# Tom94/practical-path-guiding

Hardware: AMD Instinct MI355X
Metric: Msamples/s (higher is better)
Workload: dtype f32; 1 GPU; room-720p (kitchen-class STAND-IN for the KITCHEN scene, 1397784 Lambertian triangles), 1280x720, 1 spp/pass, 614 passes, improved preset; headline_scene=False, parallelism=tiles1

## Files before the change

### include/ppg.h

```cpp
#ifndef PPG_H
#define PPG_H

#include <stddef.h>
#include <stdint.h>

#ifdef __cplusplus
extern "C" {
#endif

#define PPG_OK 0
#define PPG_ERR_INVALID (-1)
#define PPG_ERR_DEVICE (-2)
#define PPG_ERR_STATE (-3)
#define PPG_ERR_CANCELLED (-4)
#define PPG_ERR_NOMEM (-5)

typedef struct ppg_ctx ppg_ctx;

typedef struct ppg_config {
    const char *nee;
    const char *sampleCombination;
    const char *spatialFilter;
    const char *directionalFilter;
    const char *bsdfSamplingFractionLoss;
// ... 223 lines not shown
    uint32_t weight_texture;
    int32_t ensure_energy_conservation;
    uint32_t _reserved[4];
} ppg_blend;
int ppg_set_blends(ppg_ctx *ctx, const ppg_blend *b, uint32_t n_materials);

int ppg_render(ppg_ctx *ctx);

int ppg_begin_render(ppg_ctx *ctx);
int ppg_begin_iteration(ppg_ctx *ctx, int32_t is_final);
int ppg_set_final(ppg_ctx *ctx, int32_t is_final);
int ppg_set_do_nee(ppg_ctx *ctx, int32_t do_nee);
int ppg_render_passes(ppg_ctx *ctx, int32_t n_passes, ppg_pass_stats *stats);
int ppg_build_sdtree(ppg_ctx *ctx, ppg_tree_stats *stats);
int ppg_end_iteration(ppg_ctx *ctx);
int ppg_end_render(ppg_ctx *ctx);

int ppg_cancel(ppg_ctx *ctx);
int ppg_release_cached_memory(int32_t device);

int ppg_read_film(ppg_ctx *ctx, float *rgb);
int ppg_read_variance(ppg_ctx *ctx, float *rgb);

int ppg_dump_sdtree(ppg_ctx *ctx, const char *path);

typedef struct ppg_sdtree_info {
    uint32_t n_stree_nodes;
    uint32_t n_leaves;
    uint64_t n_sampling_nodes;
    uint64_t n_building_nodes;
    float aabb_min[3], aabb_max[3];
    int32_t iter;
    int32_t is_built;
} ppg_sdtree_info;

int ppg_sdtree_info_get(ppg_ctx *ctx, ppg_sdtree_info *info);

int ppg_sdtree_read_stree(ppg_ctx *ctx, int32_t *axis, uint32_t *children );

int ppg_sdtree_read_dtree_headers(ppg_ctx *ctx, int32_t which, uint64_t *offset, uint32_t *num_nodes,
                                  int32_t *max_depth, float *sum, double *stat_weight);

int ppg_sdtree_read_dtree_nodes(ppg_ctx *ctx, int32_t which, float *sums, uint16_t *children, uint64_t *fixed_sums);

int ppg_sdtree_read_adam(ppg_ctx *ctx, float *theta);

int ppg_sdtree_stat_buffers(ppg_ctx *ctx, void **dev_sums, uint64_t *n_sums, void **dev_weights, uint64_t *n_weights);
int ppg_film_buffers(ppg_ctx *ctx, void **dev_rgb_sum , void **dev_weight );
int ppg_image_buffers(ppg_ctx *ctx, void **dev_image , void **dev_sq_image ,
                      void **dev_weight );
int ppg_render_passes_nostat(ppg_ctx *ctx, int32_t n_passes);
int ppg_finish_passes(ppg_ctx *ctx, ppg_pass_stats *stats);

#define PPG_STOP_CANCELLED 2
typedef int (*ppg_stop_hook)(void *user, int local_stop);
int ppg_set_stop_hook(ppg_ctx *ctx, ppg_stop_hook hook, void *user);
int ppg_exchange_stream(ppg_ctx *ctx, void **hip_stream);
int32_t ppg_final_group_passes(int32_t n_passes);
int ppg_final_partials(ppg_ctx *ctx, void **dev , uint64_t *n_floats);
int ppg_final_partials_commit(ppg_ctx *ctx);

typedef int (*ppg_footprint_hook)(void *user, void *dev_halo , uint64_t n_floats, int32_t local_status);
int ppg_set_footprint_hook(ppg_ctx *ctx, ppg_footprint_hook hook, void *user);
uint64_t ppg_footprint_halo_floats(int32_t width, int32_t height, int32_t tile_size, int32_t world, int32_t border);

#define PPG_ADAM_ROUND_MAX_PASSES 16
#define PPG_ADAM_ROUND_MAX_PATHS (1u << 24)
#define PPG_ADAM_CODE_BITS 13
#define PPG_ADAM_PATH_BITS 27
#define PPG_ADAM_LEAF_SHIFT (PPG_ADAM_CODE_BITS + PPG_ADAM_PATH_BITS)
#define PPG_ADAM_CODE_VERTEX 4096
#define PPG_ADAM_DEFER_DEPTH 64
#define PPG_ADAM_DEFER_PATH_BIT (1u << (PPG_ADAM_PATH_BITS - 1))
int32_t ppg_adam_round_passes(int32_t spp_per_pass, int32_t width, int32_t height, int32_t n_passes);

#define PPG_ADAM_REGION_MAX_PASSES 16
int ppg_set_adam_regions(ppg_ctx *ctx, int32_t regions);

typedef struct ppg_adam_record {
    uint64_t key;
    float product, wo_pdf, bsdf_pdf, dtree_pdf, statistical_weight, _pad;
} ppg_adam_record;

typedef int (*ppg_pass_hook)(void *user);
int ppg_set_pass_hook(ppg_ctx *ctx, ppg_pass_hook hook, void *user);
int ppg_adam_records(ppg_ctx *ctx, void **dev_records , uint64_t *n);
int ppg_adam_records_replace(ppg_ctx *ctx, const void *dev_records, uint64_t n);

int ppg_hook_phase(ppg_ctx *ctx, int32_t *phase);
int ppg_adam_records_by_owner(ppg_ctx *ctx, int32_t world, void **dev_records , uint64_t *counts );
int ppg_adam_state(ppg_ctx *ctx, int32_t world, void **dev_state, uint64_t *segment);
int ppg_adam_state_commit(ppg_ctx *ctx);

int ppg_query_pdf(ppg_ctx *ctx, uint32_t n, const float *positions, const float *dirs, float *pdf_out);
int ppg_query_sample(ppg_ctx *ctx, uint32_t n, const float *positions, uint64_t seed, float *dirs_out);

typedef struct ppg_kernel_time { const char *name; double ms; uint64_t launches; uint64_t units; } ppg_kernel_time;
int ppg_kernel_times(ppg_ctx *ctx, ppg_kernel_time *out, uint32_t cap, uint32_t *n);
int ppg_enable_kernel_timing(ppg_ctx *ctx, int32_t enable);

#define PPG_FIXED_SHIFT 24

#ifdef __cplusplus
}
#endif
#endif
// ... 1 lines not shown
```

### include/ppg_testhooks.h

```cpp
#ifndef PPG_TESTHOOKS_H
#define PPG_TESTHOOKS_H

#include <stdint.h>

#ifdef __cplusplus
extern "C" {
#endif

int ppg_debug_build_bvh(const float *positions, const uint32_t *indices, uint32_t n_triangles, float pad_abs, int32_t max_leaf,
                        void *nodes_out, uint32_t nodes_cap, uint32_t *n_nodes, uint32_t *order_out);

struct ppg_bvh_stats {
    uint32_t n_nodes, n_leaves, depth, n_binary_nodes;
    uint32_t leaf_hist[9];
    uint32_t stack_need;
    double sa_interior, sa_leaf, sa_tris;
    double build_seconds;
};
int ppg_debug_bvh_stats(const float *positions, const uint32_t *indices, uint32_t n_triangles, float pad_abs, int32_t max_leaf,
                        struct ppg_bvh_stats *out);

int ppg_debug_bvh_trace(const float *positions, const uint32_t *indices, uint32_t n_triangles, float pad_abs, int32_t max_leaf,
                        const float *rays, uint32_t n_rays, float *t_out, int32_t *orig_out, uint32_t *steps_out, uint32_t *tests_out,
                        uint32_t *max_stack);

struct ppg_rfilter;
int ppg_debug_rfilter_table(const struct ppg_rfilter *f, float table[32], float *radius, int32_t *border);

struct ppg_ctx;
int ppg_debug_set_defer_depth(struct ppg_ctx *ctx, int32_t depth);

struct ppg_debug_hit {
    int32_t prim;
    float t;
    float p[3], geo_n[3], n[3], s[3], wi[3];
    int32_t material, emitter;
    int32_t _pad;
};
int ppg_debug_intersect(struct ppg_ctx *ctx, uint32_t n, const float *rays, struct ppg_debug_hit *out, int32_t any_hit);

enum {
    PPG_DEBUG_TRACE_LANE = 0, PPG_DEBUG_TRACE_LANE_ANY = 1, PPG_DEBUG_TRACE_LANE_VOTE = 2, PPG_DEBUG_TRACE_RESUME = 3, PPG_DEBUG_TRACE_WAVE = 4,
    PPG_DEBUG_TRACE_KTRACE = 5
};
int ppg_debug_intersect_mode(struct ppg_ctx *ctx, uint32_t n, const float *rays, struct ppg_debug_hit *out, int32_t mode, int32_t param, uint32_t *stats_out);

struct ppg_debug_direct {
    int32_t emitter;
    float d[3];
    float dist;
    float n[3];
    float pdf, em_pdf;
    float value[3];
    float _pad[3];
};
int ppg_debug_sample_direct(struct ppg_ctx *ctx, uint32_t n, const float *ref, const float *ref_n, const float *u, struct ppg_debug_direct *out);

struct ppg_debug_bsdf_item {
    int32_t material;
    float wi[3], wo[3];
    float sample[2];
    uint32_t key;
    float uv[2];
};
struct ppg_debug_bsdf_out {
    float eval[3];
    float pdf;
    float wo[3];
    float sampled_pdf;
    float weight[3];
    float eta;
    int32_t delta, is_null;
    int32_t _pad[2];
};
int ppg_debug_bsdf(struct ppg_ctx *ctx, uint32_t n, const struct ppg_debug_bsdf_item *items, struct ppg_debug_bsdf_out *out);

#ifdef __cplusplus
}
#endif
#endif
```

### practical-path-guiding_amd/csrc/ppg_batch_plan.h

```cpp
#pragma once

#include <algorithm>
#include <cstddef>
#include <cstdint>

namespace ppg_plan {

constexpr int kSpatialFilterBox = 2;
constexpr int kNeeKickstart = 1;
constexpr unsigned int kBlock = 256;
constexpr unsigned int kDenseChunk = 256;
constexpr unsigned int kAdamLeafShift = 40;

inline bool recordPositionsKnown(int spatialFilter, bool doNee, int nee) { return spatialFilter != kSpatialFilterBox && !(doNee && nee == kNeeKickstart); }

inline bool sideStreamsAllowed(bool timerOn, bool tuneNoOverlap) { return !timerOn && !tuneNoOverlap; }

inline unsigned int adamFlagShift(size_t streeNodes) {
    unsigned int leafBits = 1;
    while ((1u << leafBits) <= (unsigned int)streeNodes) ++leafBits;
    return kAdamLeafShift + leafBits;
}

struct BatchFacts {
// ... 58 lines not shown
    if (maxDepth >= 0) return maxDepth;
    int maxBounces;
    if (tuneBulkBounces >= 0) maxBounces = std::min(64, tuneBulkBounces);
    else {
        int need = 8;
        if (c.bounces > 0 && c.paths > 0) {
            const double scale = (double)paths / (double)c.paths;
            need = -1;
            for (int b = 0; b < c.bounces; ++b) if (c.live[b] * scale < stopBelow) { need = b + 1; break; }
            if (need < 0) {
                double live = c.live[c.bounces - 1] * scale;
                const double before = c.bounces > 1 ? c.live[c.bounces - 2] : (double)c.paths;
                const double ratio = std::min(0.97, std::max(0.5, before > 0 ? c.live[c.bounces - 1] / before : 0.9));
                need = c.bounces;
                while (live >= stopBelow && need < 64) { live *= ratio; ++need; }
            }
        }
        maxBounces = std::max(1, std::min(64, need + margin));
        if (paths < stopBelow) maxBounces = 1;
    }
    if (adamFast) maxBounces = std::min(maxBounces, std::max(1, deferDepthAdam));
    return maxBounces;
}

inline int observeBounces(SurvivalCurve &c, const unsigned int *live, int bouncesRun, unsigned int paths, unsigned int stopBelow) {
    int ran = bouncesRun;
    for (int b = 0; b < bouncesRun; ++b) if (live[b] < stopBelow) { ran = b + 1; break; }
    c.bounces = ran; c.paths = paths;
    for (int b = 0; b < ran; ++b) c.live[b] = live[b];
    return ran;
}

inline int wavefrontGrid(int nBlocks, int tuneBlocksSmall, size_t tuneSmallPaths, unsigned int paths, unsigned int queueCap) {
    if (tuneBlocksSmall > 0 && tuneBlocksSmall < nBlocks && (size_t)paths <= tuneSmallPaths) {
        const size_t chunks = ((size_t)paths + kDenseChunk - 1) / kDenseChunk;
        if (((chunks + (size_t)tuneBlocksSmall - 1) / (size_t)tuneBlocksSmall) * kDenseChunk <= (size_t)queueCap) return tuneBlocksSmall;
    }
    return nBlocks;
}

struct TailShape { int grid; unsigned int laneLimit; };

inline TailShape tailShape(int wavefrontGrid, int tuneTailBlocks, size_t handedPaths) {
    const int grid = std::min(wavefrontGrid, tuneTailBlocks ? tuneTailBlocks : 1024);
    const size_t waves = (size_t)grid * (kBlock / 64);
    return {grid, handedPaths ? (unsigned int)std::max<size_t>(1, std::min<size_t>(64, (handedPaths + waves - 1) / waves)) : 64u};
}
inline TailShape stragglerShape(unsigned int n) {
    const unsigned int waves = 1024u * (kBlock / 64u);
    const unsigned int laneLimit = std::max(1u, std::min(64u, (n + waves - 1u) / waves));
    return {(int)std::max(1u, std::min(1024u, (n + laneLimit * (kBlock / 64u) - 1u) / (laneLimit * (kBlock / 64u)))), laneLimit};
}

struct RoundReadback {
    unsigned int live[64];
    unsigned int slowCount, slowOverflow;
    unsigned int sumBase, lastNv;
    unsigned long long handed;
    unsigned long long stragglers;
};
static_assert(offsetof(RoundReadback, slowOverflow) == offsetof(RoundReadback, slowCount) + 4, "one 8-byte copy fills both");

enum class CommitSet {
    All,
    Ended,
    List
};

}
```

### practical-path-guiding_amd/csrc/ppg_hip.hip

```cpp
#include <hip/hip_runtime.h>

#include <cstring>
#include <map>
#include <mutex>
#include <set>

#include <rocprim/rocprim.hpp>

#include <algorithm>
#include <atomic>
#include <chrono>
#include <cmath>
#include <cstdio>
#include <cstdlib>
#include <cstring>
#include <functional>
#include <limits>
#include <map>
#include <memory>
#include <string>
#include <vector>

#include "../../include/ppg.h"
#include "../../include/ppg_testhooks.h"
// ... 138 lines not shown
        if (keep && p && cap && !g_ctxStream) (void)hipStreamSynchronize(nullptr);
        if (p) g_blockCache.give(p, bytes);
        p = np; bytes = got; cap = got / sizeof(T);
        return e;
    }
};

struct HostSNode {
    int axis = 0;
    uint32_t child[2] = {0, 0};
    bool isLeaf() const { return child[0] == 0; }
};

int parseEnum(const char *s, const char *dflt, std::initializer_list<const char *> names) {
    std::string v = s ? s : dflt;
    int i = 0;
    for (const char *n : names) {
        if (v == n) return i;
        ++i;
    }
    return -1;
}

struct KernelTimer {
    struct Rec { hipEvent_t a, b; int id; uint64_t units; };
    std::vector<std::string> names;
    std::vector<double> ms;
    std::vector<uint64_t> launches, units;
    std::vector<Rec> pending;
    std::vector<hipEvent_t> pool;
    bool enabled = false;
    int idOf(const char *n) {
        for (size_t i = 0; i < names.size(); ++i) if (names[i] == n) return (int)i;
        names.push_back(n); ms.push_back(0); launches.push_back(0); units.push_back(0);
        return (int)names.size() - 1;
    }
    hipEvent_t ev() { if (!pool.empty()) { hipEvent_t e = pool.back(); pool.pop_back(); return e; } hipEvent_t e; (void)hipEventCreate(&e); return e; }
    void resolve() {
        for (auto &r : pending) {
            (void)hipEventSynchronize(r.b);
            float t = 0; (void)hipEventElapsedTime(&t, r.a, r.b);
            ms[r.id] += t; launches[r.id]++; units[r.id] += r.units;
            pool.push_back(r.a); pool.push_back(r.b);
        }
        pending.clear();
    }
    void reset() { resolve(); for (size_t i = 0; i < ms.size(); ++i) { ms[i] = 0; launches[i] = 0; units[i] = 0; } }
};

}

struct GroupLaunch { unsigned int firstPass, groupPasses, stridePasses, slot0, slotStride; bool wholeFilm; unsigned int addCount; bool groupsDone = true; bool exchange = false; };

struct ppg_ctx {
    int nee = 0, sampleCombination = 1, spatialFilter = 0, directionalFilter = 0, loss = 0, budgetType = 1;
    int sdTreeMaxMemory = -1, sTreeThreshold = 12000, sppPerPass = 4, rrDepth = 5, maxDepth = -1;
    float dTreeThreshold = 0.01f, bsdfSamplingFraction = 0.5f, budget = 300.0f;
    bool dumpSDTree = false, strictNormals = false, hideEmitters = false;
    uint64_t seed = 0;
    int device = 0;
    std::string dumpPrefix, error;
    hipStream_t stream = nullptr;
    hipStream_t stream2 = nullptr;
    hipEvent_t evFork = nullptr, evJoin = nullptr;
    hipStream_t stream3 = nullptr;
    hipEvent_t evTreeFork = nullptr, evSplatDone = nullptr, evAdamDone = nullptr;
    bool treePending = false;
    void joinTree() {
        if (!treePending) return;
        (void)hipStreamWaitEvent(stream, evSplatDone, 0);
        (void)hipStreamWaitEvent(stream, evAdamDone, 0);
        treePending = false;
    }
    void quiesce() {
        joinTree();
        if (stream2) (void)hipStreamSynchronize(stream2);
        if (stream3) (void)hipStreamSynchronize(stream3);
        if (stream4) (void)hipStreamSynchronize(stream4);
        if (stream) (void)hipStreamSynchronize(stream);
        for (Stragglers &g : strag) { g.pending = false; g.aside = false; g.film = nullptr; }
    }
    hipStream_t stream4 = nullptr;
    hipEvent_t evStragFork = nullptr, evStragDone = nullptr;
    struct Stragglers {
        DevBuf<float4> rec, vert;
        DevBuf<unsigned int> orig, iota, ticket, base, origSorted, perm;
        DevBuf<unsigned long long> count;
        DevBuf<unsigned char> nv8;
        DevBuf<float> neeCos, theta;
        size_t iotaN = 0;
        PathState P{};
        unsigned int n = 0;
        bool pending = false;
        bool aside = false;
        bool commit = false, adam = false;
        std::function<void()> film;
    } strag[2];
    int stragCur = 0;
    DevBuf<float4> d_liKeep;
    Stragglers &stragPrev() { return strag[stragCur ^ 1]; }
    int tuneSplitDepth = PPG_ADAM_DEFER_DEPTH;
    bool tuneFinalHalves = false;
    int adamRegions = 0;
    DevBuf<unsigned int> d_regionPixels;
    std::vector<unsigned int> regionOffset;
    int regionsBuilt = 0;
    int deferDepthAdam = PPG_ADAM_DEFER_DEPTH;
    int joinStragglers() {
        int rc = 0;
        for (Stragglers &g : strag) if (g.pending && g.aside) { g.aside = false; rc = (int)hipStreamWaitEvent(stream, evStragDone, 0); }
        return rc;
    }
    DevBuf<unsigned char> d_straggler;
    DevBuf<unsigned char> d_nv8;

    bool haveScene = false;
    bool fullMaterials = false;
    DevBuf<float4> d_tris, d_accel, d_accelSmall, d_normals, d_materials, d_emitters, d_emTris, d_emNrm;
    DevBuf<float> d_rtrans;
    DevBuf<float4> d_spheres;
    DevBuf<float2> d_uvs;
    std::vector<DevBuf<float4>> d_texTexels;
    DevBuf<DevTex> d_textures;
    DevBuf<float4> d_emTexels;
    DevBuf<float> d_emCdfRows, d_emCdfCols, d_emRowWeights;
    DevBuf<float> d_emSel, d_emArea, d_neeCos;
    DevBuf<int4> d_emInfo;
    DevBuf<BvhNode> d_bvh;
    DevBuf<Bvh4QNode> d_bvh4;
    DevBuf<float4> d_bvhTop;
    DevScene scene{};
    float aabbMin[3], aabbMax[3];
// ... 80 lines not shown
    DevBuf<unsigned long long> d_adamKeys[2];
    DevBuf<unsigned int> d_adamIdx[2], d_adamNv, d_adamBase, d_adamCount;
    DevBuf<AdamRec> d_adamRecs, d_adamRecsOut;
    DevBuf<float4> d_splat;
    bool sortedCommit = false;
    unsigned int adamFlagShift = 0;
    DevBuf<unsigned char> d_sortTemp, d_orderTemp;
    DevBuf<unsigned int> d_adamLeafCount[2], d_adamLeafOrder[2];
    size_t adamIota = 0;
    bool adamFast = false;
    bool adamActive = false;
    bool inHook = false, hookReplaced = false;
    uint64_t hookCount = 0;
    int hookPhase = 0;
    bool ownerMode = false;
    DevBuf<unsigned int> d_adamState;
    DevBuf<unsigned long long> d_ownerBounds;
    DevBuf<unsigned int> d_bounceCounts, d_ticket;
    RoundReadback *h_round = nullptr;
    SurvivalCurve survival;
    int bounceMargin = 3;
    unsigned int tailThreshold = 0;
    unsigned int tailMin = 2097152, tailDiv = 12;
    size_t tuneBatchPaths = 0;
    int tuneBlocks = 0;
    bool tuneForceBvh = false;
    bool tuneNoSort = false;
    bool tuneNoSortFirst = false;
    bool tuneNoSplit = false;
    bool tuneNoOverlap = false;
    bool tuneNoSortedCommit = false;
    unsigned int tuneSplatLdsNodes = PPG_SPLAT_NODES;
    bool tuneNoAside = false;
    bool tuneAdamUnordered = false;
    int tuneBulkBounces = -1;
    bool debugBatch = false;
    int tuneFinalBatch = 0;
    int tuneTailBlocks = 0;
    int tunePathLayout = 0;
    int tuneBlocksSmall = 2048;
    size_t tuneSmallPaths = 13000000;
    int tuneBvhLeaf = 4;
    float tuneBvhPad = 2e-6f;
    bool tuneNoTopCut = false;
    DevBuf<unsigned int> d_leaves, d_counts, d_offsets, d_grid;
    DevBuf<unsigned int> d_dfs[2], d_refEv, d_refLv, d_refEvOff, d_refLvOff;
    int dfsCur = 0;
    unsigned int dfsCount = 0;
    int ldsNodes = 0, ldsTris = 0;
    float treeMin[3], treeMax[3], treeExt[3];
    bool isBuilt = false, isFinalIter = false, doNee = false;
    int iter = 0, passesRendered = 0, passesRenderedThisIter = 0, passesLocal = 0;
    std::chrono::steady_clock::time_point startTime, passStart;
    std::atomic<bool> cancelled{false};
    bool cancelSeen = false;
    bool seesCancel() { if (!cancelled.load()) return false; cancelSeen = true; return true; }
    float lastVariance = 0;
    ppg_pass_stats lastStats{};
    KernelTimer timer;
#define PPG_TAIL_LOG 256
    DevBuf<unsigned int> d_tailLongest;
    unsigned int tailLaunches = 0;
    uint64_t tailLongestSum = 0;
    uint64_t shadeCommonRays = 0;
    uint64_t bvhNodesVisited = 0, bvhTrisTested = 0;
    ppg_pass_hook passHook = nullptr;
    void *passHookUser = nullptr;
    ppg_stop_hook stopHook = nullptr;
    void *stopHookUser = nullptr;
#ifdef PPG_PROBE
    DevBuf<unsigned long long> d_probe;
#endif

    DevTree devTree() {
        DevTree T{};
        T.stree = d_stree.p; T.hdr = d_hdr.p; T.snodes = d_snodes[cur].p; T.bchild = d_bchild.p; T.bacc = d_bacc.p;
        T.bweight = d_bweight.p;
        T.bweight_rep = d_bweightRep.p;
        T.adam_keys = adamActive ? d_adamKeys[0].p : nullptr; T.adam_recs = adamActive ? d_adamRecs.p : nullptr;
        T.adam_count = d_adamCount.p; T.adam_base = (adamActive && adamFast) ? d_adamBase.p : nullptr;
        T.adam_cap = adamActive ? (unsigned int)std::min<size_t>(std::min(d_adamRecs.cap, d_adamKeys[0].cap), 0xfffffff0u) : 0u;
        for (int a = 0; a < 3; ++a) { T.aabb_min[a] = treeMin[a]; T.aabb_ext[a] = treeExt[a]; T.aabb_max[a] = treeMax[a]; }
        T.is_built = isBuilt ? 1 : 0;
        T.grid = d_grid.p;
        return T;
    }
    RenderParams params() const {
        RenderParams R{};
        R.nee = nee; R.spatial_filter = spatialFilter; R.directional_filter = directionalFilter; R.loss = loss;
        R.bsdf_sampling_fraction = bsdfSamplingFraction; R.rr_depth = rrDepth; R.max_depth = maxDepth;
        R.strict_normals = strictNormals; R.hide_emitters = hideEmitters; R.spp = sppPerPass;
        R.is_final_iter = isFinalIter; R.do_nee = doNee; R.seed = seed; R.pass_index = (unsigned int)passesRendered;
        R.max_vertices = maxVertices; R.img_pixels = (unsigned int)W * (unsigned int)H;
#ifdef PPG_PROBE
        R.probe = d_probe.p;
#endif
        return R;
    }
};

PathKernels ppg_path_kernels[PPG_FAMILIES];

static int sceneFamily(const DevScene &S) {
    if (S.blend) return PPG_FAMILY_BLEND;
    if (S.coat) return PPG_FAMILY_COAT;
    if (S.mfd) return PPG_FAMILY_EXT;
    if (S.n_shapes) return PPG_FAMILY_SHAPES;
    return PPG_FAMILY_BASE;
}
template <typename F> static F launcher(F f) {
    if (!f) { fprintf(stderr, "libppg_hip: no unit of this library holds the kernel asked for\n"); abort(); }
    return f;
}
static void ppg_launch_shade(int variant, const ShadeLaunch &a) { launcher(ppg_path_kernels[sceneFamily(a.S)].shade[variant >> 1])(variant, a); }
static void ppg_launch_tail(int variant, const TailLaunch &a) { launcher(ppg_path_kernels[sceneFamily(a.S)].tail[variant >> 1])(variant, a); }
static bool isSmallScene(const ppg_ctx *ctx) {
    return ctx->scene.n_tris <= 64 && ctx->ldsTris == ctx->scene.n_tris && ctx->scene.n_spheres == 0 && sceneFamily(ctx->scene) == PPG_FAMILY_BASE && !ctx->tuneForceBvh;
}
namespace {

template <typename F> void timedLaunch(ppg_ctx *ctx, const char *name, uint64_t units, F &&launch) {
    if (!ctx->timer.enabled) { launch(); return; }
    KernelTimer::Rec r; r.a = ctx->timer.ev(); r.b = ctx->timer.ev(); r.id = ctx->timer.idOf(name); r.units = units;
    (void)hipEventRecord(r.a, ctx->stream);
    launch();
    (void)hipEventRecord(r.b, ctx->stream);
    ctx->timer.pending.push_back(r);
}

bool sideStreamsAllowed(const ppg_ctx *ctx) { return ppg_plan::sideStreamsAllowed(ctx->timer.enabled, ctx->tuneNoOverlap); }

int gridFor(size_t n, int block = PPG_BLOCK, int maxBlocks = 256 * 8) {
    size_t b = (n + block - 1) / block;
    return (int)std::max<size_t>(1, std::min<size_t>(b, (size_t)maxBlocks));
}

float elapsedSeconds(std::chrono::steady_clock::time_point start) {
    auto ms = std::chrono::duration_cast<std::chrono::milliseconds>(std::chrono::steady_clock::now() - start);
    return (float)ms.count() / 1000;
}

int uploadTree(ppg_ctx *ctx, bool nodes) {
    size_t n = ctx->snodes.size();
    std::vector<int4> st(nodes ? n : 0);
    if (nodes) {
        for (size_t i = 0; i < n; ++i) st[i] = make_int4(ctx->snodes[i].axis, (int)ctx->snodes[i].child[0], (int)ctx->snodes[i].child[1], 0);
        HIP_CHECK(ctx->d_stree.reserve(n));
        HIP_CHECK(ctx->d_hdr.reserve(n));
        HIP_CHECK(hipMemcpyAsync(ctx->d_stree.p, st.data(), n * sizeof(int4), hipMemcpyHostToDevice, ctx->stream));
        HIP_CHECK(hipMemcpyAsync(ctx->d_hdr.p, ctx->hdr.data(), n * sizeof(LeafHdr), hipMemcpyHostToDevice, ctx->stream));
    }
    ctx->leaves.clear();
    for (size_t i = 0; i < n; ++i) if (ctx->snodes[i].isLeaf()) ctx->leaves.push_back((unsigned int)i);
    HIP_CHECK(ctx->d_leaves.reserve(ctx->leaves.size()));
    HIP_CHECK(ctx->d_counts.reserve(ctx->leaves.size()));
    HIP_CHECK(ctx->d_offsets.reserve(ctx->leaves.size()));
    HIP_CHECK(hipMemcpyAsync(ctx->d_leaves.p, ctx->leaves.data(), ctx->leaves.size() * 4, hipMemcpyHostToDevice, ctx->stream));
    HIP_CHECK(ctx->d_bweight.reserve(n));
    HIP_CHECK(hipMemsetAsync(ctx->d_bweight.p, 0, n * 8, ctx->stream));
    HIP_CHECK(ctx->d_bweightRep.reserve(n * PPG_REPLICAS));
    HIP_CHECK(hipMemsetAsync(ctx->d_bweightRep.p, 0, n * PPG_REPLICAS * 8, ctx->stream));
    if (n >= (1u << 27)) { ctx->error = "S-tree exceeds 2^27 nodes"; return PPG_ERR_NOMEM; }
    const unsigned int cells = PPG_GRID_DIM * PPG_GRID_DIM * PPG_GRID_DIM;
    HIP_CHECK(ctx->d_grid.reserve(cells));
    hipLaunchKernelGGL(k_build_grid, dim3((cells + 255) / 256), dim3(256), 0, ctx->stream, ctx->d_stree.p, ctx->d_grid.p);
    HIP_CHECK(hipStreamSynchronize(ctx->stream));
    return PPG_OK;
}

int refineDevice(ppg_ctx *ctx, size_t sTreeThreshold, int maxMB) {
    auto &nodes = ctx->snodes;
    auto &hdr = ctx->hdr;
    if (maxMB >= 0) {
        size_t foot = 0;
        for (size_t i = 0; i < nodes.size(); ++i) foot += nodes[i].isLeaf() ? ((size_t)hdr[i].b_num * 24 + 40) + ((size_t)hdr[i].s_num * 24 + 40) : 2 * (24 + 40);
        if (foot / 1000000 >= (size_t)maxMB) return PPG_OK;
    }
    const unsigned int nl = ctx->dfsCount, nOld = (unsigned int)nodes.size();
    hipStream_t s = ctx->stream;
    HIP_CHECK(ctx->d_refEv.reserve(nl)); HIP_CHECK(ctx->d_refLv.reserve(nl)); HIP_CHECK(ctx->d_refEvOff.reserve(nl)); HIP_CHECK(ctx->d_refLvOff.reserve(nl));
    HIP_CHECK(ctx->d_total.reserve(2));
    hipLaunchKernelGGL(k_refine_count, dim3((nl + 255) / 256), dim3(256), 0, s, ctx->d_hdr.p, ctx->d_dfs[ctx->dfsCur].p, nl, (float)sTreeThreshold,
                       ctx->d_refEv.p, ctx->d_refLv.p);
// ... 114 lines not shown
        st->min_stat_weight = minSW; st->avg_stat_weight = avgSW; st->max_stat_weight = maxSW;
        st->n_leaves = (uint32_t)nPoints; st->n_stree_nodes = (uint32_t)ctx->snodes.size(); st->n_dtree_nodes = totalNodes;
    }
    ctx->isBuilt = true;
    return PPG_OK;
}

int allocPaths(ppg_ctx *ctx) {
    std::vector<unsigned int> pix;
    int tilesX = (ctx->W + ctx->tileSize - 1) / ctx->tileSize;
    for (int y = 0; y < ctx->H; ++y)
        for (int x = 0; x < ctx->W; ++x) {
            int t = (y / ctx->tileSize) * tilesX + (x / ctx->tileSize);
            if (ctx->shardWorld <= 1 || t % ctx->shardWorld == ctx->shardRank) pix.push_back((unsigned int)(y * ctx->W + x));
        }
    ctx->nPix = (unsigned int)pix.size();
    ctx->regionsBuilt = 0;
    HIP_CHECK(ctx->d_pixels.reserve(std::max<size_t>(1, pix.size())));
    if (!pix.empty()) HIP_CHECK(hipMemcpy(ctx->d_pixels.p, pix.data(), pix.size() * 4, hipMemcpyHostToDevice));
    ctx->nPixAll = (unsigned int)((size_t)ctx->W * ctx->H);
    if (ctx->shardWorld > 1) {
        std::vector<unsigned int> all(ctx->nPixAll);
        for (unsigned int k = 0; k < ctx->nPixAll; ++k) all[k] = k;
        HIP_CHECK(ctx->d_pixelsAll.reserve(std::max<size_t>(1, all.size())));
        if (!all.empty()) HIP_CHECK(hipMemcpy(ctx->d_pixelsAll.p, all.data(), all.size() * 4, hipMemcpyHostToDevice));
    }
    {
        const size_t perPass = std::max<size_t>(1, (size_t)ctx->nPix * ctx->sppPerPass);
        size_t target = 16u << 20;
        {
            int slots = PPG_MAX_VERTICES;
            if (ctx->maxDepth > 0) slots = std::max(1, std::min(PPG_MAX_VERTICES, ctx->maxDepth - 1));
            const size_t perPath = (size_t)slots * (ctx->spatialFilter != SF_NEAREST ? 96 : 64) + 96;
            target = std::min<size_t>(target, (size_t)24e9 / perPath);
        }
        if (ctx->tuneBatchPaths) target = ctx->tuneBatchPaths;
        ctx->maxBatch = ctx->budgetType == 1 ? 1 : (int)std::max<size_t>(1, std::min<size_t>(64, target / perPass));
        if (ctx->loss != LOSS_NONE) {
            if ((uint64_t)ctx->W * ctx->H * ctx->sppPerPass > (uint64_t)PPG_ADAM_DEFER_PATH_BIT) { ctx->error = "width * height * sppPerPass exceeds 2^26 = 67108864 with a bsdfSamplingFractionLoss"; return PPG_ERR_INVALID; }
            ctx->maxBatch = std::max(ctx->maxBatch, (int)ppg_adam_round_passes(ctx->sppPerPass, ctx->W, ctx->H, 1 << 30));
        }
    }
    {
        const size_t perPass = std::max<size_t>(1, (size_t)(ctx->shardWorld > 1 ? ctx->nPixAll : ctx->nPix) * ctx->sppPerPass);
        const size_t capPasses = ctx->tuneFinalBatch ? (size_t)ctx->tuneFinalBatch : 64, capPaths = (size_t)1 << (capPasses > 64 ? 28 : 26);
        ctx->maxBatchFinal = ctx->budgetType == 1 ? 1 : (int)std::max<size_t>((size_t)ctx->maxBatch, std::min<size_t>(capPasses, capPaths / perPass));
        if (ctx->tuneBatchPaths) ctx->maxBatchFinal = ctx->maxBatch;
    }
    size_t n = (size_t)ctx->nPix * ctx->sppPerPass * (size_t)ctx->maxBatch;
    const size_t nFinal = (size_t)(ctx->shardWorld > 1 ? ctx->nPixAll : ctx->nPix) * ctx->sppPerPass * (size_t)ctx->maxBatchFinal;
    if (n > 0xfffffff0ull || nFinal > 0xfffffff0ull) { ctx->error = "too many paths per pass"; return PPG_ERR_INVALID; }
    const size_t nTrain = std::max<size_t>(1, n);
    size_t nn = std::max<size_t>(1, std::max(n, nFinal));
    ctx->maxVertices = PPG_MAX_VERTICES;
    if (ctx->maxDepth > 0) ctx->maxVertices = std::max(1, std::min(PPG_MAX_VERTICES, ctx->maxDepth - 1));
    ctx->aosPaths = ctx->tunePathLayout ? ctx->tunePathLayout == 2 : (ctx->maxDepth < 0 && ctx->scene.n_tris > 64);
    if (ctx->aosPaths) { HIP_CHECK(ctx->d_pathRec.reserve(nn * 8)); HIP_CHECK(ctx->d_miscCompact.reserve(nn)); }
    else {
        HIP_CHECK(ctx->d_ray_o.reserve(nn)); HIP_CHECK(ctx->d_ray_d.reserve(nn)); HIP_CHECK(ctx->d_thr.reserve(nn));
        HIP_CHECK(ctx->d_li.reserve(nn)); HIP_CHECK(ctx->d_hit.reserve(nn)); HIP_CHECK(ctx->d_misc.reserve(nn));
    }
    if (ctx->tuneBlocks) ctx->nBlocks = ctx->tuneBlocks;
    const size_t nb = (size_t)ctx->nBlocks;
    const size_t chunks = (nn + PPG_DCHUNK - 1) / PPG_DCHUNK;
    const size_t cap = ((chunks + nb - 1) / nb) * PPG_DCHUNK;
    for (int k = 0; k < 2; ++k) { HIP_CHECK(ctx->d_queue[k].reserve(cap * nb)); HIP_CHECK(ctx->d_qcount[k].reserve(nb)); }
    HIP_CHECK(ctx->d_stats.reserve(nb)); HIP_CHECK(ctx->d_qtotal.reserve(1));
    HIP_CHECK(ctx->d_offsets.reserve(nb)); HIP_CHECK(ctx->d_total.reserve(2));
    HIP_CHECK(ctx->d_bounceCounts.reserve(72)); HIP_CHECK(ctx->d_ticket.reserve(1));
    HIP_CHECK(ctx->d_adamCount.reserve(2));
    if (!ctx->h_round) HIP_CHECK(hipHostMalloc((void **)&ctx->h_round, sizeof(RoundReadback), hipHostMallocDefault));
    ctx->queues.items[0] = ctx->d_queue[0].p; ctx->queues.items[1] = ctx->d_queue[1].p;
    ctx->queues.count[0] = ctx->d_qcount[0].p; ctx->queues.count[1] = ctx->d_qcount[1].p;
    ctx->queues.cap = (unsigned int)cap; ctx->queues.stats = ctx->d_stats.p; ctx->queues.n_blocks = (unsigned int)nb;
    ctx->queues.n_common = nullptr;
    if (ctx->fullMaterials && !ctx->tuneNoSort) {
        HIP_CHECK(ctx->d_queueSorted.reserve(cap * nb)); HIP_CHECK(ctx->d_sortKeys.reserve(cap * nb));
        if (!ctx->tuneNoSplit) { HIP_CHECK(ctx->d_qcommon.reserve(nb)); ctx->queues.n_common = ctx->d_qcommon.p; }
    }
    size_t nv = nTrain * (size_t)ctx->maxVertices;
    const bool filtered = ctx->spatialFilter != SF_NEAREST;
    PathState &P = ctx->paths;
    P.n_paths = (unsigned int)n; P.n_pix = ctx->nPix; P.pixels = ctx->d_pixels.p;
    if (ctx->aosPaths) {
        const unsigned int vs = filtered ? 6u : 4u;
        HIP_CHECK(ctx->d_vertexRec.reserve(nv * vs));
        float4 *r = ctx->d_pathRec.p, *v = ctx->d_vertexRec.p;
        P.ray_o = {r, 8}; P.ray_d = {r + 1, 8}; P.thr = {r + 2, 8}; P.li = {r + 3, 8}; P.hit = {r + 4, 8}; P.misc = {reinterpret_cast<uint4 *>(r + 5), 8};
        P.v_d = {v, vs}; P.v_thr = {v + 1, vs}; P.v_bsdf = {v + 2, vs}; P.v_rad = {v + 3, vs};
        P.v_o = {filtered ? v + 4 : nullptr, vs}; P.v_vox = {filtered ? v + 5 : nullptr, vs};
    } else {
        HIP_CHECK(ctx->d_vd.reserve(nv)); HIP_CHECK(ctx->d_vthr.reserve(nv)); HIP_CHECK(ctx->d_vbsdf.reserve(nv)); HIP_CHECK(ctx->d_vrad.reserve(nv));
        if (filtered) { HIP_CHECK(ctx->d_vo.reserve(nv)); HIP_CHECK(ctx->d_vvox.reserve(nv)); }
        P.ray_o = {ctx->d_ray_o.p, 1}; P.ray_d = {ctx->d_ray_d.p, 1}; P.thr = {ctx->d_thr.p, 1}; P.li = {ctx->d_li.p, 1}; P.hit = {ctx->d_hit.p, 1};
        P.misc = {ctx->d_misc.p, 1};
        P.v_d = {ctx->d_vd.p, 1}; P.v_thr = {ctx->d_vthr.p, 1}; P.v_bsdf = {ctx->d_vbsdf.p, 1}; P.v_rad = {ctx->d_vrad.p, 1};
        P.v_o = {filtered ? ctx->d_vo.p : nullptr, 1}; P.v_vox = {filtered ? ctx->d_vvox.p : nullptr, 1};
    }
    P.nee_cos = nullptr;
    if (ctx->scene.env.w != 0 && ctx->nee != NEE_NEVER) { HIP_CHECK(ctx->d_neeCos.reserve(nn)); P.nee_cos = ctx->d_neeCos.p; }
    return PPG_OK;
}

int presizeRounds(ppg_ctx *ctx) {
    g_blockCache.prewarm();
    if (ctx->loss == LOSS_NONE || ctx->budgetType != 0 || !recordPositionsKnown(ctx->spatialFilter, false, ctx->nee)) return PPG_OK;
    const int nPasses = (int)std::ceil((size_t)ctx->budget / (float)ctx->sppPerPass);
    int rendered = 0, largest = 0;
    for (int it = 0; rendered < nPasses; ++it) {
        const int remaining = nPasses - rendered;
        int n = std::min(remaining, 1 << std::min(it, 30));
        if (remaining - n < 2 * n) n = remaining;
        if (n < remaining && it > 0) largest = std::max(largest, n);
        rendered += n;
    }
    if (largest == 0) return PPG_OK;
    const size_t roundPaths = (size_t)ppg_adam_round_passes(ctx->sppPerPass, ctx->W, ctx->H, largest) * ctx->nPix * ctx->sppPerPass;
    const size_t handed = ctx->maxDepth < 0 ? std::min(roundPaths, std::max<size_t>(ctx->tailMin, roundPaths / ctx->tailDiv)) : 0;
    const size_t positions = std::min<size_t>(roundPaths * 7 + handed * (size_t)ctx->maxVertices, 0xfffffff0u);
    for (int k = 0; k < 2; ++k) { HIP_CHECK(ctx->d_adamKeys[k].reserve(positions)); HIP_CHECK(ctx->d_adamIdx[k].reserve(positions)); }
// ... 406 lines not shown
                           ctx->d_foot.p, ctx->d_halo.p);
    });
    { int rc = callFootprintHook(ctx, 0); if (rc) return rc; }
    if (ctx->haloUnpackN) timedLaunch(ctx, "k_halo_unpack", ctx->haloUnpackN, [&] {
        hipLaunchKernelGGL(k_halo_unpack, dim3((ctx->haloUnpackN + 255) / 256), dim3(256), 0, s, ctx->d_haloUnpack.p, ctx->haloUnpackN, ctx->d_haloSrc.p, ctx->d_haloTap.p, M, n,
                           ctx->d_foot.p, ctx->d_halo.p);
    });
    launchFilmResolveOwned(ctx, im, sq, w, film, film_w);
    HIP_CHECK(hipGetLastError());
    return PPG_OK;
}


int prepareBatch(ppg_ctx *ctx, Batch &B, int batch, bool adamRound, const GroupLaunch *gl, bool last) {
    const PathState &P = B.P;
    hipStream_t s = ctx->stream;
    const ppg_ctx::Stragglers &prev = ctx->stragPrev();
    BatchFacts f;
    f.paths = P.n_paths; f.maxDepth = ctx->maxDepth; f.isFinalIter = ctx->isFinalIter; f.adamRound = adamRound; f.last = last;
    f.spatialFilter = ctx->spatialFilter; f.nee = ctx->nee; f.doNee = ctx->doNee;
    f.timerOn = ctx->timer.enabled; f.tuneNoOverlap = ctx->tuneNoOverlap; f.tuneNoSortedCommit = ctx->tuneNoSortedCommit; f.tuneSplitDepth = ctx->tuneSplitDepth;
    f.tailThreshold = ctx->tailThreshold; f.tailMin = ctx->tailMin; f.tailDiv = ctx->tailDiv;
    f.deferDepthAdam = ctx->deferDepthAdam; f.streeNodes = ctx->snodes.size();
    f.prevPendingWithRecords = prev.pending && prev.adam; f.prevStragglers = prev.n; f.maxVertices = ctx->maxVertices;
    B.plan = planBatch(f);
    ctx->adamActive = adamRound; ctx->adamFast = B.plan.adamFast; ctx->sortedCommit = B.plan.sortedCommit; ctx->adamFlagShift = B.plan.adamFlagShift;
    if (adamRound && !B.plan.adamFast) {
        const size_t cap = std::max<size_t>((size_t)1 << 16, std::min<size_t>((size_t)48 * P.n_paths, 0xfffffff0u));
        HIP_CHECK(ctx->d_adamKeys[0].reserve(cap)); HIP_CHECK(ctx->d_adamRecs.reserve(cap));
        HIP_CHECK(hipMemsetAsync(ctx->d_adamCount.p, 0, 8, s));
    }
    B.S = ctx->scene;
    B.T = ctx->devTree();
    RenderParams &R = B.R;
    R = ctx->params();
    R.spp = ctx->sppPerPass * batch;
    R.pass_index_spp = (unsigned int)ctx->passesRendered * (unsigned int)ctx->sppPerPass;
    if (gl) {
        R.pass_index_spp = gl->firstPass * (unsigned int)ctx->sppPerPass;
        R.group_samples = gl->groupPasses * (unsigned int)ctx->sppPerPass;
        R.group_stride = gl->stridePasses * (unsigned int)ctx->sppPerPass;
    }
    B.Q = ctx->queues;
    B.dense = B.Q.items[1];
    B.grid = wavefrontGrid(ctx->nBlocks, ctx->tuneBlocksSmall, ctx->tuneSmallPaths, P.n_paths, ctx->queues.cap);
    B.gridAll = gridFor(P.n_paths);
    B.smallScene = isSmallScene(ctx);
    B.ldsBytes = B.smallScene ? (size_t)ctx->ldsTris * 48 : (size_t)PPG_LDS_STACK * PPG_BLOCK * 4;
    B.hostCount = P.n_paths;
    B.Pc = P;
    return PPG_OK;
}

int runWavefront(ppg_ctx *ctx, Batch &B) {
    const PathState &P = B.P;
    const DevScene &S = B.S;
    Queues &Q = B.Q;
    hipStream_t s = ctx->stream;
    const int grid = B.grid;
    const bool smallScene = B.smallScene;
    const bool neeOn = ctx->doNee;
    const bool fullMats = ctx->fullMaterials;
    const size_t triBytes = (size_t)ctx->scene.n_tris * 48;
    const size_t traceLds = smallScene ? B.ldsBytes : (size_t)PPG_TRACE_STACK * PPG_BLOCK * 4 + (PPG_BLOCK / 64) * sizeof(PairLds);
    const unsigned int stopBelow = B.plan.stopBelow;
    int qin = QIN_FIRST;
    timedLaunch(ctx, "k_generate", P.n_paths, [&] { hipLaunchKernelGGL(k_generate, dim3(B.gridAll), dim3(PPG_BLOCK), 0, s, P, S, B.R, Q); });
    const int maxBounces = planBounces(ctx->survival, P.n_paths, stopBelow, ctx->maxDepth, ctx->tuneBulkBounces, ctx->bounceMargin, B.plan.adamFast, ctx->deferDepthAdam);
    const bool liveCount = ctx->timer.enabled;
    unsigned int *counts = ctx->d_bounceCounts.p;
    HIP_CHECK(hipMemsetAsync(counts, 0, 72 * 4, s));
    Q.stop = counts + 64;
    Q.dense_n = ctx->d_total.p;
    for (int b = 0; b < maxBounces; ++b) {
        const bool sortSlices = fullMats && (qin == QIN_DENSE || (Q.n_common && !neeOn && !ctx->tuneNoSortFirst)) && ctx->d_queueSorted.p;
        unsigned int *const trSorted = sortSlices ? ctx->d_queueSorted.p : nullptr;
        unsigned char *const trKeys = sortSlices ? ctx->d_sortKeys.p : nullptr;
        timedLaunch(ctx, "k_trace", B.hostCount, [&] {
            TraceLaunch a{grid, traceLds, s, P, S, Q, qin, smallScene ? 0 : ctx->ldsNodes, ctx->ldsTris, trSorted, trKeys, smallScene, ctx->timer.enabled};
            launcher(ppg_path_kernels[sceneFamily(S)].trace)(a);
        });
        int shadeIn = sortSlices ? QIN_SORTED : qin;
        ctx->joinTree();
        const bool split = shadeIn == QIN_SORTED && Q.n_common && !neeOn;
        if (split) {
            timedLaunch(ctx, "k_shade<common>", B.hostCount, [&] {
                ShadeLaunch a{grid, 0, s, P, S, B.T, B.R, Q, QIN_SORTED_COMMON, smallScene ? 1 : 0, ctx->d_queueSorted.p};
                ppg_launch_shade_common(a);
            });
            shadeIn = QIN_SORTED_REST;
        }
        timedLaunch(ctx, neeOn ? "k_shade<nee>" : (fullMats ? (split ? "k_shade<rest>" : "k_shade<full>") : "k_shade"), B.hostCount, [&] {
            const int small = smallScene ? 1 : 0;
            const size_t neeBytes = smallScene ? triBytes : (size_t)PPG_LDS_STACK * PPG_BLOCK * 4;
            const size_t lds = (neeOn || ctx->scene.has_null) ? neeBytes : 0;
            const int variant = (neeOn ? 2 : 0) | (fullMats ? 1 : 0);
            ShadeLaunch a{grid, lds, s, P, S, B.T, B.R, Q, shadeIn, small, ctx->d_queueSorted.p};
            ppg_launch_shade(variant, a);
        });
        qin = QIN_DENSE;
        ++B.bouncesRun;
        hipLaunchKernelGGL(k_scan_counts, dim3(1), dim3(1024), 0, s, Q.count[0], ctx->d_offsets.p, (unsigned int)grid, ctx->d_total.p,
                           counts + std::min(b, 63), counts + 64, stopBelow);
        hipLaunchKernelGGL(k_gather_slices, dim3(grid), dim3(PPG_BLOCK), 0, s, Q.items[0], Q.count[0], ctx->d_offsets.p, Q.cap, Q.items[1]);
        if (liveCount) {
            HIP_CHECK(hipMemcpyAsync(&B.hostCount, ctx->d_total.p, 4, hipMemcpyDeviceToHost, s));
            HIP_CHECK(hipStreamSynchronize(s));
            if (B.hostCount == 0 || (ctx->maxDepth < 0 && B.hostCount < stopBelow)) break;
        }
    }
    return PPG_OK;
}

int launchTail(ppg_ctx *ctx, Batch &B, unsigned int depth, size_t handedPaths) {
    hipStream_t s = ctx->stream;
    ppg_ctx::Stragglers &G = ctx->strag[ctx->stragCur];
    HIP_CHECK(hipMemsetAsync(ctx->d_ticket.p, 0, 4, s));
    const TailShape shape = tailShape(B.grid, ctx->tuneTailBlocks, handedPaths);
    timedLaunch(ctx, "k_tail", B.hostCount, [&] {
        RenderParams Rt = B.R;
        Rt.defer_depth = depth;
        TailLaunch a{shape.grid, B.ldsBytes, s, B.P, B.S, B.T, Rt, B.dense, ctx->d_total.p, ctx->d_ticket.p, B.Q.stats, ctx->ldsTris,
                     ctx->d_tailLongest.p + (depth ? PPG_TAIL_LOG : (ctx->tailLaunches++ % PPG_TAIL_LOG)), StragOut{G.rec.p, G.orig.p, G.count.p}, shape.laneLimit};
        ppg_launch_tail(tailVariant(ctx), a);
    });
    return PPG_OK;
}

int copyMisc(ppg_ctx *ctx, Batch &B) {
    const PathState &P = B.P;
    if (B.miscCopied || P.n_paths == 0) return PPG_OK;
    HIP_CHECK(ctx->d_nv8.reserve(P.n_paths));
    hipLaunchKernelGGL(k_commit_prepare, dim3((P.n_paths + 255) / 256), dim3(256), 0, ctx->stream, P, ctx->aosPaths ? ctx->d_miscCompact.p : (uint4 *)nullptr, ctx->d_nv8.p,
                       B.plan.overlap ? (const unsigned char *)ctx->d_straggler.p : (const unsigned char *)nullptr);
// ... 8 lines not shown
    CommitLaunch a{B.grid, st, list ? B.P : B.Pc, B.T, B.R, B.Q, ctx->d_nv8.p, list ? B.dense : nullptr, list ? ctx->d_total.p : nullptr, ctx->d_splat.p, ctx->adamFlagShift};
    launchCommitKernels(ctx, a, ctx->sortedCommit);
}
void launchCommitTimed(ppg_ctx *ctx, const Batch &B, CommitSet set, uint64_t units) {
    timedLaunch(ctx, commitName(ctx->sortedCommit), units, [&] { launchCommit(ctx, B, ctx->stream, set); });
}

int launchTailAndEndedCommit(ppg_ctx *ctx, Batch &B, unsigned int depth, size_t handedPaths) {
    hipStream_t s = ctx->stream;
    if (B.plan.overlap) HIP_CHECK(hipEventRecord(ctx->evFork, s));
    { int rc = launchTail(ctx, B, depth, handedPaths); if (rc) return rc; }
    if (!B.plan.overlap) return PPG_OK;
    if (B.plan.beside) {
        HIP_CHECK(hipStreamWaitEvent(ctx->stream2, ctx->evFork, 0));
        launchCommit(ctx, B, ctx->stream2, CommitSet::Ended);
        HIP_CHECK(hipEventRecord(ctx->evJoin, ctx->stream2));
        HIP_CHECK(hipStreamWaitEvent(s, ctx->evJoin, 0));
    } else launchCommitTimed(ctx, B, CommitSet::Ended, B.P.n_paths);
    return PPG_OK;
}

int finishPaths(ppg_ctx *ctx, Batch &B) {
    const PathState &P = B.P;
    const BatchPlan &plan = B.plan;
    hipStream_t s = ctx->stream;
    RoundReadback *const h = ctx->h_round;
    ctx->joinTree();
    if (plan.tail) {
        if (B.bouncesRun == 0)
            hipLaunchKernelGGL(k_iota_total, dim3(B.gridAll), dim3(PPG_BLOCK), 0, s, B.dense, P.n_paths, ctx->d_total.p);
        if (plan.overlap) {
            HIP_CHECK(ctx->d_straggler.reserve(P.n_paths));
            HIP_CHECK(hipMemsetAsync(ctx->d_straggler.p, 0, P.n_paths, s));
            hipLaunchKernelGGL(k_mark_list, dim3(B.grid), dim3(PPG_BLOCK), 0, s, B.dense, ctx->d_total.p, ctx->d_straggler.p);
        } else if (!plan.splitTail) {
            int rc = launchTail(ctx, B, 0u, 0);
            if (rc) return rc;
        }
    }
    if (plan.fastRound) {
        HIP_CHECK(ctx->d_adamNv.reserve(P.n_paths)); HIP_CHECK(ctx->d_adamBase.reserve(P.n_paths));
        { int rc = copyMisc(ctx, B); if (rc) return rc; }
        hipLaunchKernelGGL(k_path_nv, dim3((P.n_paths + 255) / 256), dim3(256), 0, s, B.Pc, ctx->d_adamNv.p, plan.overlap ? ctx->d_straggler.p : nullptr, (unsigned int)ctx->maxVertices);
        size_t bytes = 0;
        HIP_CHECK(rocprim::exclusive_scan(nullptr, bytes, ctx->d_adamNv.p, ctx->d_adamBase.p, 0u, (size_t)P.n_paths, rocprim::plus<unsigned int>(), s));
        HIP_CHECK(ctx->d_sortTemp.reserve(std::max<size_t>(bytes, 16)));
        HIP_CHECK(rocprim::exclusive_scan((void *)ctx->d_sortTemp.p, bytes, ctx->d_adamNv.p, ctx->d_adamBase.p, 0u, (size_t)P.n_paths, rocprim::plus<unsigned int>(), s));
        HIP_CHECK(hipMemcpyAsync(&h->sumBase, ctx->d_adamBase.p + (P.n_paths - 1), 4, hipMemcpyDeviceToHost, s));
        HIP_CHECK(hipMemcpyAsync(&h->lastNv, ctx->d_adamNv.p + (P.n_paths - 1), 4, hipMemcpyDeviceToHost, s));
    }
    if (plan.tail || plan.fastRound) {
        if (plan.tail) HIP_CHECK(hipMemcpyAsync(h->live, ctx->d_bounceCounts.p, sizeof h->live, hipMemcpyDeviceToHost, s));
        if (plan.splitTail) HIP_CHECK(hipMemcpyAsync(&h->handed, ctx->d_total.p, 8, hipMemcpyDeviceToHost, s));
        HIP_CHECK(hipStreamSynchronize(s));
        if (plan.tail) {
            const int ran = observeBounces(ctx->survival, h->live, B.bouncesRun, P.n_paths, plan.stopBelow);
            if (ctx->debugBatch) {
                fprintf(stderr, "[ppg batch] iter %d paths %u built %d final %d launched %d ran %d stop<%u live:", ctx->iter, P.n_paths, (int)ctx->isBuilt, (int)ctx->isFinalIter, B.bouncesRun, ran, plan.stopBelow);
                for (int b = 0; b < ran; ++b) fprintf(stderr, " %u", h->live[b]);
                fprintf(stderr, "\n");
            }
        }
        if (plan.fastRound) {
            B.nRecordsOwn = (size_t)h->sumBase + h->lastNv;
            if (B.nRecordsOwn + plan.nDeferredIn > 0xfffffff0ull) { ctx->error = "too many Adam records in one round"; return PPG_ERR_NOMEM; }
        }
    }
    if (plan.fastRound || (plan.adamFast && plan.nDeferredIn)) {
        B.nRecords = B.nRecordsOwn + plan.nDeferredIn;
        int rc = reserveRoundRecords(ctx, B.nRecords);
        if (rc) return rc;
        B.T = ctx->devTree();
    }
    if (plan.commit) { int rc = copyMisc(ctx, B); if (rc) return rc; }
    if (plan.splitTail) {
        ppg_ctx::Stragglers &G = ctx->strag[ctx->stragCur];
        const size_t handed = (size_t)h->handed;
        HIP_CHECK(G.rec.reserve(std::max<size_t>(1, handed) * 8)); HIP_CHECK(G.orig.reserve(std::max<size_t>(1, handed)));
        HIP_CHECK(G.count.reserve(2)); HIP_CHECK(G.ticket.reserve(1));
        HIP_CHECK(hipMemsetAsync(G.count.p, 0, 16, s));
        { int rc = launchTailAndEndedCommit(ctx, B, plan.deferDepth, handed); if (rc) return rc; }
        HIP_CHECK(hipMemcpyAsync(&h->stragglers, G.count.p, 8, hipMemcpyDeviceToHost, s));
        HIP_CHECK(hipStreamSynchronize(s));
        B.nStrag = (unsigned int)h->stragglers;
        if (ctx->debugBatch) fprintf(stderr, "[ppg batch] iter %d stragglers %u of %zu handed over at depth %u\n", ctx->iter, B.nStrag, handed, plan.deferDepth);
        if (B.nStrag) {
            int rc = drainStragglers(ctx, B.nRecordsOwn);
            if (!rc) rc = launchStragglers(ctx, B);
            if (rc) return rc;
        }
        if (plan.overlap) launchCommitTimed(ctx, B, CommitSet::List, 0);
    } else if (plan.overlap) {
        int rc = launchTailAndEndedCommit(ctx, B, 0u, 0);
        if (rc) return rc;
        launchCommitTimed(ctx, B, CommitSet::List, 0);
    } else if (plan.commit) launchCommitTimed(ctx, B, CommitSet::All, P.n_paths);
    if (!B.nStrag) return drainStragglers(ctx, B.nRecordsOwn);
    return PPG_OK;
}

int optimiserRound(ppg_ctx *ctx, Batch &B) {
    if (!ctx->adamFast) {
        RoundReadback *const h = ctx->h_round;
        HIP_CHECK(hipMemcpyAsync(&h->slowCount, ctx->d_adamCount.p, 8, hipMemcpyDeviceToHost, ctx->stream));
        HIP_CHECK(hipStreamSynchronize(ctx->stream));
        if (h->slowOverflow) { ctx->error = "Adam record buffer overflow (box spatial filter / next-event estimation with a bsdfSamplingFractionLoss)"; return PPG_ERR_NOMEM; }
        B.nRecords = h->slowCount;
    }
    const int rc = applyAdamRound(ctx, B.nRecords);
    ctx->adamActive = false;
    return rc;
}

void filmOrDefer(ppg_ctx *ctx, const Batch &B, int batch, const GroupLaunch *gl) {
    PathState Pf = B.P;
    const bool defer = B.nStrag > 0;
    if (defer) Pf.li = {ctx->d_liKeep.p, 1};
    const int sppBatch = ctx->sppPerPass * batch;
    const bool hasGl = gl != nullptr;
    const GroupLaunch glv = gl ? *gl : GroupLaunch{};
    const unsigned long long seed = B.R.seed;
    const unsigned int base = B.R.pass_index_spp, gs = B.R.group_samples, gstride = B.R.group_stride;
    auto film = [ctx, Pf, sppBatch, hasGl, glv, seed, base, gs, gstride] {
        hipStream_t st = ctx->stream;
        if (ctx->filtered) {
            if (!hasGl) launchFilmFilter(ctx, Pf, seed, base, 0u, 0u, 0, sppBatch);
            else {
                const size_t n = ctx->nPixAll;
                for (int j0 = 0, k = 0; j0 < sppBatch; j0 += (int)gs, ++k) {
                    launchFilmFilter(ctx, Pf, seed, base, gs, gstride, j0, std::min(sppBatch, j0 + (int)gs));
                    if (!glv.groupsDone || glv.exchange) continue;
                    float *slot = ctx->d_partials.p + (ctx->shardWorld > 1 ? 4 * n : 0) + (size_t)(glv.slot0 + (unsigned int)k * glv.slotStride) * 7u * n;
                    launchFilmResolve(ctx, slot, slot + 3 * n, slot + 6 * n, nullptr, nullptr);
                }
            }
            if (hasGl && glv.addCount) (void)addGroups(ctx, 0, glv.addCount);
            return;
        }
        timedLaunch(ctx, "k_film", Pf.n_pix, [&] {
            if (hasGl) hipLaunchKernelGGL(k_film_groups, dim3((Pf.n_pix + 255) / 256), dim3(256), 0, st, Pf, sppBatch, glv.groupPasses * (unsigned int)ctx->sppPerPass,
                                          ctx->d_partials.p + (ctx->shardWorld > 1 ? 4 * (size_t)ctx->nPixAll : 0), glv.slot0, glv.slotStride, ctx->nPixAll);
            else hipLaunchKernelGGL(k_film, dim3((Pf.n_pix + 255) / 256), dim3(256), 0, st, Pf, sppBatch, ctx->d_image.p, ctx->d_sq.p, ctx->d_imageW.p,
                                    ctx->d_film.p, ctx->d_filmW.p);
        });
        if (hasGl && glv.addCount) (void)addGroups(ctx, 0, glv.addCount);
    };
    if (defer) ctx->stragPrev().film = film; else film();
}


int renderBatch(ppg_ctx *ctx, int batch, bool adamRound, const GroupLaunch *gl = nullptr, bool last = true, const unsigned int *regionPixels = nullptr,
                unsigned int regionCount = 0) {
    Batch B{};
    PathState &P = B.P;
    P = ctx->paths;
    if (regionPixels) { P.n_pix = regionCount; P.pixels = regionPixels; }
    if (gl && gl->wholeFilm && ctx->shardWorld > 1) { P.n_pix = ctx->nPixAll; P.pixels = ctx->d_pixelsAll.p; }
    P.n_paths = (unsigned int)((size_t)P.n_pix * ctx->sppPerPass * (size_t)batch);
    if (P.n_paths == 0 && !(adamRound && ctx->passHook)) return PPG_OK;
    int rc = prepareBatch(ctx, B, batch, adamRound, gl, last);
    if (!rc && P.n_paths > 0) rc = runWavefront(ctx, B);
    if (!rc) rc = finishPaths(ctx, B);
    if (!rc && adamRound) rc = optimiserRound(ctx, B);
    if (rc) return rc;
    if (P.n_paths > 0) filmOrDefer(ctx, B, batch, gl);
    HIP_CHECK(hipGetLastError());
    return PPG_OK;
}


int addGroups(ppg_ctx *ctx, unsigned int first, unsigned int count) {
    const unsigned int n = ctx->nPixAll;
    hipLaunchKernelGGL(k_add_groups, dim3((n + 255) / 256), dim3(256), 0, ctx->stream, n, ctx->d_partials.p + (ctx->shardWorld > 1 ? 4 * (size_t)n : 0), first, count,
                       ctx->d_image.p, ctx->d_sq.p, ctx->d_imageW.p, ctx->d_film.p, ctx->d_filmW.p);
    return PPG_OK;
}
static bool finalGroupsByRank(unsigned int nGroups, unsigned int world) { return world > 1 && nGroups >= 2u * world; }

int renderFinalGroups(ppg_ctx *ctx, int numPasses) {
    const unsigned int G = (unsigned int)ppg_final_group_passes(numPasses), nGroups = ((unsigned int)numPasses + G - 1) / G;
    const unsigned int world = (unsigned int)ctx->shardWorld, rank = (unsigned int)ctx->shardRank;
    const bool byRank = finalGroupsByRank(nGroups, world);
    const size_t n = ctx->nPixAll;
    std::vector<unsigned int> mine;
    for (unsigned int g = byRank ? rank : 0u; g < nGroups; g += byRank ? world : 1u) mine.push_back(g);
    auto passesOf = [&](unsigned int g) { return std::min(G, (unsigned int)numPasses - g * G); };
    unsigned int launchPasses = (unsigned int)ctx->maxBatchFinal;
    {
        unsigned int minePasses = 0;
        for (unsigned int g : mine) minePasses += passesOf(g);
        const size_t pixels = byRank || world == 1 ? n : (size_t)ctx->nPix;
        if (ctx->tuneFinalHalves && ctx->maxDepth < 0 && ctx->tuneSplitDepth > 0 && sideStreamsAllowed(ctx) && minePasses >= 2 && minePasses <= launchPasses &&
            pixels * (size_t)ctx->sppPerPass * (size_t)(minePasses / 2) >= ((size_t)1 << 21)) {
            launchPasses = (minePasses + 1) / 2;
            if (G < launchPasses) launchPasses = std::max(G, launchPasses / G * G);
        }
    }
    const bool exch = ctx->exchangesFootprints() && !byRank;
    auto exchangeGroup = [&](unsigned int g) -> int {
        int rc = flushStragglers(ctx, false);
        if (rc) return rc;
        float *slot = ctx->d_partials.p + 4 * n + (size_t)g * 7u * n;
        return exchangeFootprint(ctx, slot, slot + 3 * n, slot + 6 * n, nullptr, nullptr);
    };
    const unsigned int perLaunch = exch ? 1u : std::max(1u, launchPasses / G);
    const unsigned int slots = world > 1 ? nGroups : std::max(perLaunch, std::max(1u, (unsigned int)ctx->maxBatchFinal / G));
    const size_t floats = (world > 1 ? 4 * n : 0) + (size_t)slots * 7 * n;
    if (ctx->d_partials.cap < floats || ctx->partialSlots != slots) {
        HIP_CHECK(ctx->d_partials.reserve(floats));
        ctx->partialSlots = slots;
    }
    HIP_CHECK(hipMemsetAsync(ctx->d_partials.p, 0, floats * 4, ctx->stream));
    const unsigned int firstPassAbs = (unsigned int)ctx->passesRendered;
    const unsigned int step = byRank ? world : 1u;
    const uint64_t pixelsMine = byRank || world == 1 ? (uint64_t)n : (uint64_t)ctx->nPix;
    bool stop = false;
    for (size_t m = 0; m < mine.size() && !stop;) {
        if (ctx->seesCancel()) break;
        if (G <= launchPasses) {
            const size_t cnt = std::min<size_t>(perLaunch, mine.size() - m);
            unsigned int batch = 0;
            for (size_t q = 0; q < cnt; ++q) batch += passesOf(mine[m + q]);
            GroupLaunch gl{firstPassAbs + mine[m] * G, G, step * G, world > 1 ? mine[m] : 0u, world > 1 ? step : 1u, byRank, world == 1 ? (unsigned int)cnt : 0u};
            gl.exchange = exch;
            int rc = renderBatch(ctx, (int)batch, false, &gl, m + cnt >= mine.size());
            if (rc) return rc;
            ctx->samplesLocal += pixelsMine * batch * ctx->sppPerPass;
            if (exch && (rc = exchangeGroup(mine[m]))) return rc;
            m += cnt;
        } else {
            const unsigned int g = mine[m], total = passesOf(g);
            for (unsigned int done = 0; done < total;) {
                if (ctx->seesCancel()) { stop = true; break; }
                const unsigned int batch = std::min(launchPasses, total - done);
                const bool lastPart = done + batch >= total;
                GroupLaunch gl{firstPassAbs + g * G + done, batch, batch, world > 1 ? g : 0u, 1u, byRank, (world == 1 && lastPart) ? 1u : 0u, lastPart};
                gl.exchange = exch;
                int rc = renderBatch(ctx, (int)batch, false, &gl, lastPart && m + 1 >= mine.size());
                if (rc) return rc;
                ctx->samplesLocal += pixelsMine * batch * ctx->sppPerPass;
                done += batch;
            }
            if (exch && !stop) { int rc = exchangeGroup(g); if (rc) return rc; }
            ++m;
        }
        HIP_CHECK(hipStreamSynchronize(ctx->stream));
    }
    { int rc = flushStragglers(ctx, false); if (rc) return rc; }
    ctx->passesRendered += numPasses; ctx->passesRenderedThisIter += numPasses; ctx->passesLocal += numPasses;
    if (world > 1) { ctx->partialsPending = true; ctx->pendingGroups = nGroups; }
    return ctx->seesCancel() ? PPG_ERR_CANCELLED : PPG_OK;
}

int buildRegionLists(ppg_ctx *ctx, int regions) {
    if (ctx->regionsBuilt == regions) return PPG_OK;
    const int bs = 32, bx = (ctx->W + bs - 1) / bs, by = (ctx->H + bs - 1) / bs;
    std::vector<int> rank((size_t)bx * by);
    ppg_spiral_block_ranks(bx, by, rank.data());
    std::vector<unsigned int> own(ctx->nPix);
    if (ctx->nPix) HIP_CHECK(hipMemcpy(own.data(), ctx->d_pixels.p, (size_t)ctx->nPix * 4, hipMemcpyDeviceToHost));
    std::vector<std::vector<unsigned int>> lists((size_t)regions);
    for (unsigned int p : own) {
        const int x = (int)(p % (unsigned int)ctx->W), y = (int)(p / (unsigned int)ctx->W);
        const int r = (int)((long long)rank[(size_t)(y / bs) * bx + (x / bs)] * regions / (bx * by));
        lists[(size_t)r].push_back(p);
    }
    ctx->regionOffset.assign((size_t)regions + 1, 0u);
    std::vector<unsigned int> flat;
    flat.reserve(own.size());
    for (int r = 0; r < regions; ++r) { ctx->regionOffset[(size_t)r] = (unsigned int)flat.size(); flat.insert(flat.end(), lists[(size_t)r].begin(), lists[(size_t)r].end()); }
    ctx->regionOffset[(size_t)regions] = (unsigned int)flat.size();
    HIP_CHECK(ctx->d_regionPixels.reserve(std::max<size_t>(1, flat.size())));
    if (!flat.empty()) HIP_CHECK(hipMemcpyAsync(ctx->d_regionPixels.p, flat.data(), flat.size() * 4, hipMemcpyHostToDevice, ctx->stream));
    HIP_CHECK(hipStreamSynchronize(ctx->stream));
    ctx->regionsBuilt = regions;
    return PPG_OK;
}

int renderPassesBody(ppg_ctx *ctx, int numPasses) {
    size_t n = (size_t)ctx->W * ctx->H;
    HIP_CHECK(hipMemsetAsync(ctx->d_image.p, 0, 3 * n * 4, ctx->stream));
    HIP_CHECK(hipMemsetAsync(ctx->d_sq.p, 0, 3 * n * 4, ctx->stream));
    HIP_CHECK(hipMemsetAsync(ctx->d_imageW.p, 0, n * 4, ctx->stream));
    HIP_CHECK(hipMemsetAsync(ctx->d_stats.p, 0, sizeof(BlockStats) * (size_t)ctx->nBlocks, ctx->stream));
    HIP_CHECK(ctx->d_tailLongest.reserve(PPG_TAIL_LOG + 1));
    HIP_CHECK(hipMemsetAsync(ctx->d_tailLongest.p, 0, (PPG_TAIL_LOG + 1) * 4, ctx->stream));
    ctx->tailLaunches = 0;
    ctx->passStart = std::chrono::steady_clock::now();
    ctx->passesLocal = 0;
    const bool rounds = ctx->loss != LOSS_NONE && ctx->isBuilt && !ctx->isFinalIter;
    const int roundPasses = rounds ? (int)ppg_adam_round_passes(ctx->sppPerPass, ctx->W, ctx->H, numPasses) : (ctx->isFinalIter ? ctx->maxBatchFinal : ctx->maxBatch);
    ctx->samplesLocal = 0;
    ctx->partialsPending = false; ctx->partialsExported = false;
    if (ctx->filtered) { int rc = prepareFootprint(ctx); if (rc) return rc; }
    if (ctx->isFinalIter && ctx->budgetType == 0 && numPasses > 0) return renderFinalGroups(ctx, numPasses);
    int regions = 0;
    if (rounds && ctx->adamRegions > 1 && numPasses <= PPG_ADAM_REGION_MAX_PASSES) {
        regions = std::min(ctx->adamRegions, ((ctx->W + 31) / 32) * ((ctx->H + 31) / 32));
        int rc = buildRegionLists(ctx, regions);
        if (rc) return rc;
    }
    bool drain = false;
    for (int i = 0; i < numPasses;) {
        if (ctx->seesCancel()) {
            if (rounds && ctx->passHook) drain = true;
            else {
                if (ctx->budgetType == 1 && ctx->stopHook) (void)ctx->stopHook(ctx->stopHookUser, PPG_STOP_CANCELLED);
                break;
            }
        }
        const int batch = regions ? 1 : std::min(roundPasses, numPasses - i);
        int rc = PPG_OK;
        if (regions) {
            for (int r = 0; r < regions && !rc; ++r) {
                const unsigned int first = ctx->regionOffset[(size_t)r], count = ctx->regionOffset[(size_t)r + 1] - first;
                rc = renderBatch(ctx, drain ? 0 : 1, true, nullptr, i + 1 >= numPasses && r + 1 == regions, ctx->d_regionPixels.p + first, drain ? 0u : count);
            }
        } else rc = renderBatch(ctx, drain ? 0 : batch, rounds, nullptr, i + batch >= numPasses);
        if (rc) return rc;
        ctx->passesRendered += batch; ctx->passesRenderedThisIter += batch; ctx->passesLocal += batch;
        ctx->samplesLocal += (uint64_t)ctx->nPix * batch * ctx->sppPerPass;
        i += batch;
        if (ctx->budgetType == 1) {
            HIP_CHECK(hipStreamSynchronize(ctx->stream));
            int stop = (int)elapsedSeconds(ctx->startTime) > ctx->budget ? 1 : 0;
            if (ctx->stopHook) stop = ctx->stopHook(ctx->stopHookUser, stop);
            if (stop) break;
        } else if ((i & 63) < batch) {
            HIP_CHECK(hipStreamSynchronize(ctx->stream));
        }
    }
    {
        const bool deferRounds = rounds && ctx->maxDepth < 0 && recordPositionsKnown(ctx->spatialFilter, ctx->doNee, ctx->nee);
        int rc = flushStragglers(ctx, deferRounds && ctx->passHook != nullptr);
        if (rc) return rc;
    }
    if (ctx->exchangesFootprints()) { int rc = exchangeFootprint(ctx, ctx->d_image.p, ctx->d_sq.p, ctx->d_imageW.p, ctx->d_film.p, ctx->d_filmW.p); if (rc) return rc; }
    else if (ctx->filtered) launchFilmResolve(ctx, ctx->d_image.p, ctx->d_sq.p, ctx->d_imageW.p, ctx->d_film.p, ctx->d_filmW.p);
    return ctx->seesCancel() ? PPG_ERR_CANCELLED : PPG_OK;
}

int renderPassesNoStat(ppg_ctx *ctx, int numPasses) {
    ctx->footDue = 0; ctx->footDone = 0; ctx->footFailed = false;
    if (ctx->exchangesFootprints()) {
        if (!ctx->footHook) { ctx->error = kShardedFilter; return PPG_ERR_STATE; }
        if (ctx->isFinalIter && ctx->budgetType == 0 && numPasses > 0) {
            const unsigned int G = (unsigned int)ppg_final_group_passes(numPasses), nGroups = ((unsigned int)numPasses + G - 1) / G;
            ctx->footDue = finalGroupsByRank(nGroups, (unsigned int)ctx->shardWorld) ? 0u : nGroups;
        } else ctx->footDue = 1;
    }
    int rc = renderPassesBody(ctx, numPasses);
    if (ctx->footDone < ctx->footDue && !ctx->footFailed) {
        const std::string why = ctx->error;
        const uint64_t floats = ppg_footprint_halo_floats(ctx->W, ctx->H, ctx->tileSize, ctx->shardWorld, ctx->rfBorder);
        void *buf = nullptr;
        if (ctx->d_halo.reserve(std::max<size_t>(1, (size_t)floats)) == hipSuccess && hipMemsetAsync(ctx->d_halo.p, 0, std::max<size_t>(1, (size_t)floats) * 4, ctx->stream) == hipSuccess &&
            hipStreamSynchronize(ctx->stream) == hipSuccess) buf = ctx->d_halo.p;
        else (void)hipGetLastError();
        ++ctx->footDone;
        (void)ctx->footHook(ctx->footHookUser, buf, floats, 1);
        ctx->footFailed = true;
        ctx->error = why.empty() ? "footprint hook failed" : why;
        if (rc == PPG_OK) rc = PPG_ERR_INVALID;
    }
    return rc;
}

int finishPasses(ppg_ctx *ctx, ppg_pass_stats *st) {
    if (ctx->partialsPending) { ctx->error = "the groups of this final iteration were not exchanged: ppg_final_partials / ppg_final_partials_commit before ppg_finish_passes"; return PPG_ERR_STATE; }
    const int n = ctx->W * ctx->H;
    const int N = ctx->passesLocal * ctx->sppPerPass;
    if (ctx->sampleCombination == 2) {
        ctx->images.emplace_back();
        HIP_CHECK(ctx->images.back().reserve(3 * (size_t)n));
        hipLaunchKernelGGL(k_normalise, dim3((n + 255) / 256), dim3(256), 0, ctx->stream, n, ctx->d_image.p, ctx->d_imageW.p, ctx->images.back().p);
    }
    hipLaunchKernelGGL(k_variance, dim3((n + 255) / 256), dim3(256), 0, ctx->stream, n, ctx->W, N, ctx->d_image.p, ctx->d_sq.p, ctx->d_imageW.p, ctx->d_var.p, ctx->d_lum.p);
    float *lum = ctx->h_lum;
    if (ctx->h_statsCap < (size_t)ctx->nBlocks) {
        if (ctx->h_stats) (void)hipHostFree(ctx->h_stats);
        ctx->h_stats = nullptr; ctx->h_statsCap = 0;
        HIP_CHECK(hipHostMalloc((void **)&ctx->h_stats, (size_t)ctx->nBlocks * sizeof(BlockStats), hipHostMallocDefault));
        ctx->h_statsCap = (size_t)ctx->nBlocks;
    }
    BlockStats *bs = ctx->h_stats;
    HIP_CHECK(hipMemcpyAsync(lum, ctx->d_lum.p, (size_t)n * 4, hipMemcpyDeviceToHost, ctx->stream));
    HIP_CHECK(hipMemcpyAsync(bs, ctx->d_stats.p, (size_t)ctx->nBlocks * sizeof(BlockStats), hipMemcpyDeviceToHost, ctx->stream));
    unsigned int tailLongest[PPG_TAIL_LOG];
    const unsigned int nTails = std::min<unsigned int>(ctx->tailLaunches, PPG_TAIL_LOG);
    if (nTails) HIP_CHECK(hipMemcpyAsync(tailLongest, ctx->d_tailLongest.p, nTails * 4, hipMemcpyDeviceToHost, ctx->stream));
    HIP_CHECK(hipStreamSynchronize(ctx->stream));
    BlockStats c{};
    for (int k = 0; k < ctx->nBlocks; ++k) { const BlockStats &x = bs[k]; c.rays += x.rays; c.path_len += x.path_len; c.committed += x.committed; c.bvh_nodes += x.bvh_nodes; c.bvh_tris += x.bvh_tris; c.max_len = std::max(c.max_len, x.max_len); c.shade_common += x.shade_common; }
    if (ctx->debugBatch) fprintf(stderr, "[ppg passes] iter %d passes %d rays %llu path_len_sum %llu longest path finished by k_tail %llu\n", ctx->iter, ctx->passesLocal, (unsigned long long)c.rays, (unsigned long long)c.path_len, (unsigned long long)c.max_len);
    ctx->bvhNodesVisited += c.bvh_nodes; ctx->bvhTrisTested += c.bvh_tris; ctx->shadeCommonRays += c.shade_common;
    for (unsigned int k = 0; k < nTails; ++k) ctx->tailLongestSum += tailLongest[k];
    float variance = 0;
    for (int k = 0; k < n; ++k) variance += lum[k];
    variance /= (float)ctx->W * ctx->H * (N - 1);
    if (ctx->sampleCombination == 2) ctx->variances.push_back(variance);
    ctx->lastVariance = variance;
    ppg_pass_stats s{};
    s.seconds = elapsedSeconds(ctx->passStart);
    s.passes_rendered_total = ctx->passesRendered; s.passes_rendered_local = ctx->passesLocal; s.variance = variance;
    s.samples = ctx->samplesLocal;
    s.rays = c.rays; s.path_length_sum = c.path_len; s.vertices_committed = c.committed;
    ctx->lastStats = s;
    if (st) *st = s;
    ctx->timer.resolve();
    return PPG_OK;
}

int allocFilm(ppg_ctx *ctx) {
    size_t n = (size_t)ctx->W * ctx->H;
    HIP_CHECK(ctx->d_image.reserve(3 * n)); HIP_CHECK(ctx->d_sq.reserve(3 * n)); HIP_CHECK(ctx->d_imageW.reserve(n));
    HIP_CHECK(ctx->d_film.reserve(3 * n)); HIP_CHECK(ctx->d_filmW.reserve(n)); HIP_CHECK(ctx->d_var.reserve(3 * n));
    HIP_CHECK(ctx->d_lum.reserve(n)); HIP_CHECK(ctx->d_tmp.reserve(3 * n));
    if (ctx->h_lumCap < n) {
        if (ctx->h_lum) (void)hipHostFree(ctx->h_lum);
        ctx->h_lum = nullptr; ctx->h_lumCap = 0;
        HIP_CHECK(hipHostMalloc((void **)&ctx->h_lum, n * sizeof(float), hipHostMallocDefault));
        ctx->h_lumCap = n;
    }
    return PPG_OK;
}

int beginRender(ppg_ctx *ctx) {
    HIP_CHECK(hipSetDevice(ctx->device));
    ctx->quiesce();
    if (!ctx->pathsReady) {
        int rc = allocPaths(ctx);
        if (rc) return rc;
        if ((rc = allocFilm(ctx))) return rc;
        ctx->pathsReady = true;
    }
    float maxSize = 0;
    for (int a = 0; a < 3; ++a) maxSize = ppg_max(maxSize, ctx->aabbMax[a] - ctx->aabbMin[a]);
    {
        float sx = ctx->aabbMax[0] - ctx->aabbMin[0], sy = ctx->aabbMax[1] - ctx->aabbMin[1], sz = ctx->aabbMax[2] - ctx->aabbMin[2];
        maxSize = ppg_max(ppg_max(sx, sy), sz);
    }
    for (int a = 0; a < 3; ++a) {
        ctx->treeMin[a] = ctx->aabbMin[a];
        ctx->treeMax[a] = ctx->aabbMin[a] + maxSize;
        ctx->treeExt[a] = ctx->treeMax[a] - ctx->treeMin[a];
    }
    ctx->snodes.assign(1, HostSNode());
    ctx->hdr.assign(1, LeafHdr{});
    HIP_CHECK(ctx->d_snodes[0].reserve(1));
    HIP_CHECK(hipMemsetAsync(ctx->d_snodes[0].p, 0, sizeof(SNode), ctx->stream));
    ctx->cur = 0;
    ctx->hdr[0].s_base = 0; ctx->hdr[0].s_num = 1;
    {
        int rc = uploadTree(ctx, true);
        if (rc) return rc;
        const unsigned int root = 0;
        HIP_CHECK(ctx->d_dfs[0].reserve(1));
        HIP_CHECK(hipMemcpy(ctx->d_dfs[0].p, &root, 4, hipMemcpyHostToDevice));
        ctx->dfsCur = 0; ctx->dfsCount = 1;
    }
    ctx->nSamplingNodes = 1; ctx->nBuildingNodes = 0;
    ctx->iter = 0; ctx->isFinalIter = false; ctx->isBuilt = false;
    size_t n = (size_t)ctx->W * ctx->H;
    HIP_CHECK(hipMemsetAsync(ctx->d_film.p, 0, 3 * n * 4, ctx->stream));
    HIP_CHECK(hipMemsetAsync(ctx->d_filmW.p, 0, n * 4, ctx->stream));
    HIP_CHECK(hipMemsetAsync(ctx->d_var.p, 0, 3 * n * 4, ctx->stream));
    HIP_CHECK(hipMemsetAsync(ctx->d_image.p, 0, 3 * n * 4, ctx->stream));
    HIP_CHECK(hipMemsetAsync(ctx->d_sq.p, 0, 3 * n * 4, ctx->stream));
    HIP_CHECK(hipMemsetAsync(ctx->d_imageW.p, 0, n * 4, ctx->stream));
    ctx->images.clear(); ctx->variances.clear();
#ifdef PPG_PROBE
    HIP_CHECK(ctx->d_probe.reserve(PPG_PROBE_SLOTS));
    HIP_CHECK(hipMemsetAsync(ctx->d_probe.p, 0, PPG_PROBE_SLOTS * 8, ctx->stream));
#endif
    ctx->startTime = std::chrono::steady_clock::now();
    ctx->passesRendered = 0; ctx->passesRenderedThisIter = 0;
    ctx->treeAlive = true;
    ctx->renderOpen = true;
    {
        const bool pending = ctx->cancelled.exchange(false), spent = ctx->cancelSeen;
        ctx->cancelSeen = false;
        if (pending && !spent) { ctx->error = "cancelled before the render began"; return PPG_ERR_CANCELLED; }
    }
    return PPG_OK;
}

int beginIteration(ppg_ctx *ctx, bool isFinal) {
    ctx->isFinalIter = isFinal;
    size_t n = (size_t)ctx->W * ctx->H;
    HIP_CHECK(hipMemsetAsync(ctx->d_film.p, 0, 3 * n * 4, ctx->stream));
    HIP_CHECK(hipMemsetAsync(ctx->d_filmW.p, 0, n * 4, ctx->stream));
    return resetSDTree(ctx);
}

int dumpSDTreeFile(ppg_ctx *ctx, const char *path);

int endIteration(ppg_ctx *ctx) {
    if (ctx->dumpSDTree && !ctx->isFinalIter && !ctx->dumpPrefix.empty()) {
        char buf[1024];
        snprintf(buf, sizeof buf, "%s-%02d.sdt", ctx->dumpPrefix.c_str(), ctx->iter);
        int rc = dumpSDTreeFile(ctx, buf);
        if (rc) return rc;
    }
    ++ctx->iter;
    ctx->passesRenderedThisIter = 0;
    return PPG_OK;
}

int endRender(ppg_ctx *ctx) {
    ctx->joinTree();
    ctx->renderOpen = false;
#ifdef PPG_PROBE
    if (ctx->d_probe.p) {
        unsigned long long h[PPG_PROBE_SLOTS];
        HIP_CHECK(hipStreamSynchronize(ctx->stream));
        HIP_CHECK(hipMemcpy(h, ctx->d_probe.p, sizeof h, hipMemcpyDeviceToHost));
        fprintf(stderr, "[ppg probe] lone_bounces %llu coop_rays %llu coop_steps %llu cycles:", h[20], h[22], h[21]);
        for (int k = 0; k <= 11; ++k) fprintf(stderr, " s%d=%llu", k, h[k]);
        fprintf(stderr, "\n");
    }
#endif
    if (ctx->sampleCombination == 2 && !ctx->images.empty()) {
        const int n = ctx->W * ctx->H;
        HIP_CHECK(hipMemsetAsync(ctx->d_film.p, 0, 3 * (size_t)n * 4, ctx->stream));
        std::vector<float> ones((size_t)n, 1.0f);
        HIP_CHECK(hipMemcpyAsync(ctx->d_filmW.p, ones.data(), (size_t)n * 4, hipMemcpyHostToDevice, ctx->stream));
        size_t begin = ctx->images.size() - std::min(ctx->images.size(), (size_t)4);
        float totalWeight = 0;
        for (size_t i = begin; i < ctx->variances.size(); ++i) totalWeight += 1.0f / ctx->variances[i];
        for (size_t i = begin; i < ctx->images.size(); ++i) {
            float mult = 1.0f / ctx->variances[i] / totalWeight;
            hipLaunchKernelGGL(k_axpy, dim3((3 * n + 255) / 256), dim3(256), 0, ctx->stream, 3 * n, mult, ctx->images[i].p, ctx->d_film.p);
        }
        HIP_CHECK(hipStreamSynchronize(ctx->stream));
    }
    return PPG_OK;
}

bool doNeeWithSpp(const ppg_ctx *ctx, int spp) {
    switch (ctx->nee) {
        case NEE_NEVER: return false;
        case NEE_KICKSTART: return spp < 128;
        default: return true;
    }
}

int renderSPP(ppg_ctx *ctx) {
    size_t sampleCount = (size_t)ctx->budget;
    int nPasses = (int)std::ceil(sampleCount / (float)ctx->sppPerPass);
    float currentVarAtEnd = std::numeric_limits<float>::infinity();
    while (ctx->passesRendered < nPasses) {
        const int sppRendered = ctx->passesRendered * ctx->sppPerPass;
        ctx->doNee = doNeeWithSpp(ctx, sppRendered);
        int remainingPasses = nPasses - ctx->passesRendered;
        int passesThisIteration = std::min(remainingPasses, 1 << ctx->iter);
        if (remainingPasses - passesThisIteration < 2 * passesThisIteration) passesThisIteration = remainingPasses;
        int rc = beginIteration(ctx, passesThisIteration >= remainingPasses);
        if (rc) return rc;
        ppg_pass_stats st;
        if ((rc = renderPassesNoStat(ctx, passesThisIteration))) return rc;
        if ((rc = finishPasses(ctx, &st))) return rc;
        float variance = st.variance;
        const float lastVarAtEnd = currentVarAtEnd;
        currentVarAtEnd = passesThisIteration * variance / remainingPasses;
        remainingPasses -= passesThisIteration;
        if (ctx->sampleCombination == 1 && remainingPasses > 0 &&
            (remainingPasses < passesThisIteration || (sppRendered > 256 && currentVarAtEnd > lastVarAtEnd))) {
            ctx->isFinalIter = true;
            if ((rc = renderPassesNoStat(ctx, remainingPasses))) return rc;
            if ((rc = finishPasses(ctx, &st))) return rc;
        }
        if ((rc = buildSDTree(ctx, nullptr))) return rc;
        if ((rc = endIteration(ctx))) return rc;
    }
    return PPG_OK;
}

int renderTime(ppg_ctx *ctx) {
    float nSeconds = ctx->budget;
    float currentVarAtEnd = std::numeric_limits<float>::infinity();
    float elapsed = 0;
    while (elapsed < nSeconds) {
        const int sppRendered = ctx->passesRendered * ctx->sppPerPass;
        ctx->doNee = doNeeWithSpp(ctx, sppRendered);
        float remainingTime = nSeconds - elapsed;
        const int passesThisIteration = 1 << ctx->iter;
        const auto startIter = std::chrono::steady_clock::now();
        int rc = beginIteration(ctx, false);
        if (rc) return rc;
        ppg_pass_stats st;
        if ((rc = renderPassesNoStat(ctx, passesThisIteration))) return rc;
        if ((rc = finishPasses(ctx, &st))) return rc;
        float variance = st.variance;
        const float secondsIter = elapsedSeconds(startIter);
        const float lastVarAtEnd = currentVarAtEnd;
        currentVarAtEnd = secondsIter * variance / remainingTime;
        remainingTime -= secondsIter;
        if (ctx->sampleCombination == 1 && remainingTime > 0 &&
            (remainingTime < secondsIter || (sppRendered > 256 && currentVarAtEnd > lastVarAtEnd))) {
            ctx->isFinalIter = true;
            do {
                if ((rc = renderPassesNoStat(ctx, passesThisIteration))) return rc;
                if ((rc = finishPasses(ctx, &st))) return rc;
                elapsed = elapsedSeconds(ctx->startTime);
            } while (elapsed < nSeconds);
        }
        if ((rc = buildSDTree(ctx, nullptr))) return rc;
        if ((rc = endIteration(ctx))) return rc;
        elapsed = elapsedSeconds(ctx->startTime);
    }
    return PPG_OK;
}

int gatherDTrees(ppg_ctx *ctx, int which, std::vector<float> &sums, std::vector<uint16_t> &children, std::vector<uint64_t> *fixed) {
// ... 142 lines not shown
int32_t ppg_adam_round_passes(int32_t spp_per_pass, int32_t width, int32_t height, int32_t n_passes) {
    const uint64_t perPass = (uint64_t)std::max(1, spp_per_pass) * (uint64_t)std::max(1, width) * (uint64_t)std::max(1, height);
    int32_t r = 1;
    while (r * 2 <= PPG_ADAM_ROUND_MAX_PASSES && r * 4 <= n_passes && (uint64_t)(r * 2) * perPass <= PPG_ADAM_ROUND_MAX_PATHS) r *= 2;
    return r;
}

int ppg_create(const ppg_config *cfg, ppg_ctx **out) {
    if (!cfg || !out) { g_createError = "null argument"; return PPG_ERR_INVALID; }
    std::unique_ptr<ppg_ctx> c(new ppg_ctx());
#define PARSE(field, dflt, target, ...)                                                                                  \
    c->target = parseEnum(cfg->field, dflt, {__VA_ARGS__});                                                              \
    if (c->target < 0) { g_createError = std::string("invalid value for '" #field "': ") + (cfg->field ? cfg->field : ""); return PPG_ERR_INVALID; }
    PARSE(nee, "never", nee, "never", "kickstart", "always")
    PARSE(sampleCombination, "automatic", sampleCombination, "discard", "automatic", "inversevar")
    PARSE(spatialFilter, "nearest", spatialFilter, "nearest", "stochastic", "box")
    PARSE(directionalFilter, "nearest", directionalFilter, "nearest", "box")
    PARSE(bsdfSamplingFractionLoss, "none", loss, "none", "kl", "var")
    PARSE(budgetType, "seconds", budgetType, "spp", "seconds")
#undef PARSE
    c->sdTreeMaxMemory = cfg->sdTreeMaxMemory; c->sTreeThreshold = cfg->sTreeThreshold; c->dTreeThreshold = cfg->dTreeThreshold;
    c->bsdfSamplingFraction = cfg->bsdfSamplingFraction; c->sppPerPass = cfg->sppPerPass; c->budget = cfg->budget;
    c->dumpSDTree = cfg->dumpSDTree != 0; c->rrDepth = cfg->rrDepth; c->maxDepth = cfg->maxDepth;
    c->strictNormals = cfg->strictNormals != 0; c->hideEmitters = cfg->hideEmitters != 0; c->seed = cfg->seed; c->device = cfg->device;
    if (cfg->dumpPrefix) c->dumpPrefix = cfg->dumpPrefix;
    {
        if (const char *e = getenv("PPG_TAIL_THRESHOLD")) c->tailThreshold = (unsigned int)std::max(0ll, atoll(e));
        if (const char *e = getenv("PPG_TAIL_MIN")) c->tailMin = (unsigned int)std::max(1ll, atoll(e));
        if (const char *e = getenv("PPG_TAIL_DIV")) c->tailDiv = (unsigned int)std::max(1ll, atoll(e));
        if (const char *e = getenv("PPG_BATCH_PATHS")) c->tuneBatchPaths = (size_t)std::max(1ll, atoll(e));
        if (const char *e = getenv("PPG_BLOCKS")) c->tuneBlocks = std::max(1, atoi(e));
        c->tuneForceBvh = getenv("PPG_FORCE_BVH") != nullptr;
        c->tuneNoSort = getenv("PPG_NO_SORT") != nullptr;
        c->tuneNoSplit = getenv("PPG_NO_SPLIT") != nullptr;
        c->tuneNoSortFirst = getenv("PPG_NO_SORT_FIRST") != nullptr;
        c->tuneNoOverlap = getenv("PPG_NO_OVERLAP") != nullptr;
        c->tuneNoSortedCommit = getenv("PPG_NO_SORTED_COMMIT") != nullptr;
        c->tuneAdamUnordered = getenv("PPG_ADAM_UNORDERED") != nullptr;
        c->tuneNoAside = getenv("PPG_NO_ASIDE") != nullptr;
        if (const char *e = getenv("PPG_SPLAT_LDS_NODES")) c->tuneSplatLdsNodes = (unsigned int)std::max(0, std::min((int)PPG_SPLAT_NODES, atoi(e)));
        if (const char *e = getenv("PPG_BULK_BOUNCES")) c->tuneBulkBounces = std::max(0, atoi(e));
        if (const char *e = getenv("PPG_BOUNCE_MARGIN")) c->bounceMargin = std::max(0, atoi(e));
        c->debugBatch = getenv("PPG_DEBUG_BATCH") != nullptr;
        if (const char *e = getenv("PPG_TAIL_BLOCKS")) c->tuneTailBlocks = std::max(1, atoi(e));
        if (const char *e = getenv("PPG_FINAL_BATCH")) c->tuneFinalBatch = std::max(1, atoi(e));
        if (const char *e = getenv("PPG_PATH_LAYOUT")) c->tunePathLayout = !strcmp(e, "aos") ? 2 : (!strcmp(e, "soa") ? 1 : 0);
        if (const char *e = getenv("PPG_BLOCKS_SMALL")) c->tuneBlocksSmall = std::max(0, atoi(e));
        if (const char *e = getenv("PPG_SMALL_PATHS")) c->tuneSmallPaths = (size_t)std::max(0ll, atoll(e));
        if (const char *e = getenv("PPG_BVH_LEAF")) c->tuneBvhLeaf = std::max(1, std::min(8, atoi(e)));
        if (const char *e = getenv("PPG_BVH_PAD")) c->tuneBvhPad = (float)atof(e);
        if (const char *e = getenv("PPG_SPLIT_DEPTH")) c->tuneSplitDepth = std::max(0, atoi(e));
        c->tuneFinalHalves = getenv("PPG_FINAL_HALVES") != nullptr;
        c->tuneNoTopCut = getenv("PPG_NO_TOPCUT") != nullptr;
    }
    if (c->sppPerPass <= 0) { g_createError = "sppPerPass must be > 0"; return PPG_ERR_INVALID; }
    int ndev = 0;
    hipError_t e = hipGetDeviceCount(&ndev);
    if (e != hipSuccess || ndev <= 0) { g_createError = std::string("no HIP device available: ") + hipGetErrorString(e); return PPG_ERR_DEVICE; }
    if (c->device < 0 || c->device >= ndev) { g_createError = "device ordinal out of range"; return PPG_ERR_INVALID; }
    if ((e = hipSetDevice(c->device)) != hipSuccess || (e = hipStreamCreate(&c->stream)) != hipSuccess || (e = hipStreamCreate(&c->stream2)) != hipSuccess ||
        (e = hipEventCreateWithFlags(&c->evFork, hipEventDisableTiming)) != hipSuccess || (e = hipEventCreateWithFlags(&c->evJoin, hipEventDisableTiming)) != hipSuccess ||
        (e = hipStreamCreate(&c->stream3)) != hipSuccess || (e = hipEventCreateWithFlags(&c->evTreeFork, hipEventDisableTiming)) != hipSuccess ||
        (e = hipStreamCreate(&c->stream4)) != hipSuccess || (e = hipEventCreateWithFlags(&c->evStragFork, hipEventDisableTiming)) != hipSuccess ||
        (e = hipEventCreateWithFlags(&c->evStragDone, hipEventDisableTiming)) != hipSuccess ||
        (e = hipEventCreateWithFlags(&c->evSplatDone, hipEventDisableTiming)) != hipSuccess || (e = hipEventCreateWithFlags(&c->evAdamDone, hipEventDisableTiming)) != hipSuccess) {
        g_createError = std::string("HIP init failed: ") + hipGetErrorString(e);
        return PPG_ERR_DEVICE;
    }
    *out = c.release();
    return PPG_OK;
}

void ppg_destroy(ppg_ctx *ctx) {
    if (!ctx) return;
    (void)hipSetDevice(ctx->device);
    if (ctx->stream) { (void)hipStreamSynchronize(ctx->stream); }
    g_blockCache.settle();
    if (ctx->stream2) (void)hipStreamSynchronize(ctx->stream2);
    if (ctx->stream3) (void)hipStreamSynchronize(ctx->stream3);
    if (ctx->stream4) (void)hipStreamSynchronize(ctx->stream4);
    g_blockCache.settle();
    if (ctx->stream2) (void)hipStreamDestroy(ctx->stream2);
    if (ctx->stream3) (void)hipStreamDestroy(ctx->stream3);
    if (ctx->stream4) (void)hipStreamDestroy(ctx->stream4);
    for (hipEvent_t ev : {ctx->evStragFork, ctx->evStragDone}) if (ev) (void)hipEventDestroy(ev);
    for (hipEvent_t ev : {ctx->evTreeFork, ctx->evSplatDone, ctx->evAdamDone}) if (ev) (void)hipEventDestroy(ev);
    if (ctx->evFork) (void)hipEventDestroy(ctx->evFork);
    if (ctx->evJoin) (void)hipEventDestroy(ctx->evJoin);
    ctx->timer.resolve();
    for (auto e : ctx->timer.pool) (void)hipEventDestroy(e);
    if (ctx->h_lum) (void)hipHostFree(ctx->h_lum);
    if (ctx->h_stats) (void)hipHostFree(ctx->h_stats);
    if (ctx->h_round) (void)hipHostFree(ctx->h_round);
    hipStream_t s = ctx->stream;
    delete ctx;
    if (s) (void)hipStreamDestroy(s);
}

const char *ppg_last_error(const ppg_ctx *ctx) { return ctx ? ctx->error.c_str() : g_createError.c_str(); }

int ppg_set_scene(ppg_ctx *ctx, const ppg_scene *s) {
    const SceneInputs in{s, ctx->materialTextures, ctx->microfacet, ctx->coatings, ctx->blends, ctx->deltaEmitters, ctx->shapes,
                         ctx->lensOn ? &ctx->lens : nullptr, ctx->tuneBvhPad, ctx->tuneBvhLeaf, ctx->tuneNoTopCut};
    if (!sceneComplete(in)) { ctx->error = "incomplete scene"; return PPG_ERR_INVALID; }
    HIP_CHECK(hipSetDevice(ctx->device));
    ctx->quiesce();
    HostScene H;
    if (int rc = buildScene(in, H, ctx->error)) return rc;
    ctx->haveScene = false; ctx->treeAlive = false; ctx->renderOpen = false; ctx->pathsReady = false;
    DevScene S;
    if (int rc = uploadScene(ctx, H, S)) return rc;
    ctx->scene = S;
    for (int a = 0; a < 3; ++a) { ctx->geomMin[a] = H.geomMin[a]; ctx->geomMax[a] = H.geomMax[a]; ctx->aabbMin[a] = H.aabbMin[a]; ctx->aabbMax[a] = H.aabbMax[a]; }
    ctx->sceneDelta = std::move(H.deltaEmitters);
    ctx->fullMaterials = H.fullMaterials; ctx->nMaterials = H.nMaterials;
    ctx->ldsNodes = H.ldsNodes; ctx->ldsTris = H.ldsTris;
    ctx->W = H.W; ctx->H = H.H;
    ctx->haveScene = true;
    return sizeBuffers(ctx);
}

int ppg_set_shard(ppg_ctx *ctx, int32_t rank, int32_t world, int32_t tile_size) {
    (void)hipSetDevice(ctx->device);
    ctx->quiesce();
    if (world < 1 || rank < 0 || rank >= world || tile_size < 1) { ctx->error = "bad shard"; return PPG_ERR_INVALID; }
    if (world > 1 && ctx->filtered && !ctx->footHook) { ctx->error = kShardedFilter; return PPG_ERR_INVALID; }
    ctx->shardRank = rank; ctx->shardWorld = world; ctx->tileSize = tile_size;
    return sizeBuffers(ctx);
}

#define NEED_SCENE (void)hipSetDevice(ctx->device); StreamScope scope_(ctx->stream); if (!ctx->haveScene) { ctx->error = "no scene"; return PPG_ERR_STATE; }
#define NEED_TREE (void)hipSetDevice(ctx->device); StreamScope scope_(ctx->stream); if (!ctx->treeAlive) { ctx->error = "render not begun"; return PPG_ERR_STATE; } ctx->joinTree();

int ppg_begin_render(ppg_ctx *ctx) { NEED_SCENE return beginRender(ctx); }
int ppg_begin_iteration(ppg_ctx *ctx, int32_t is_final) { NEED_TREE return beginIteration(ctx, is_final != 0); }
int ppg_set_final(ppg_ctx *ctx, int32_t is_final) { ctx->isFinalIter = is_final != 0; return PPG_OK; }
int ppg_set_do_nee(ppg_ctx *ctx, int32_t do_nee) { ctx->doNee = do_nee != 0; return PPG_OK; }
int ppg_render_passes_nostat(ppg_ctx *ctx, int32_t n) { NEED_TREE return renderPassesNoStat(ctx, n); }
int ppg_finish_passes(ppg_ctx *ctx, ppg_pass_stats *st) { NEED_TREE return finishPasses(ctx, st); }
int ppg_render_passes(ppg_ctx *ctx, int32_t n, ppg_pass_stats *st) {
    NEED_TREE
    int rc = renderPassesNoStat(ctx, n);
    if (rc && rc != PPG_ERR_CANCELLED) return rc;
    int rc2 = finishPasses(ctx, st);
    return rc ? rc : rc2;
}
int ppg_build_sdtree(ppg_ctx *ctx, ppg_tree_stats *st) { NEED_TREE return buildSDTree(ctx, st); }
int ppg_end_iteration(ppg_ctx *ctx) { NEED_TREE return endIteration(ctx); }
int ppg_end_render(ppg_ctx *ctx) { NEED_TREE return endRender(ctx); }
int ppg_cancel(ppg_ctx *ctx) { ctx->cancelled.store(true); return PPG_OK; }
int ppg_debug_build_bvh(const float *positions, const uint32_t *indices, uint32_t n_triangles, float pad_abs, int32_t max_leaf,
                        void *nodes_out, uint32_t nodes_cap, uint32_t *n_nodes, uint32_t *order_out) {
    if (!positions || !indices || !n_nodes || n_triangles == 0) return PPG_ERR_INVALID;
    BvhBuilder bb;
    bb.maxLeaf = std::max(1, std::min(8, (int)max_leaf));
    bb.run(positions, indices, n_triangles, pad_abs);
    *n_nodes = (uint32_t)bb.nodes4q.size();
    if (nodes_out) memcpy(nodes_out, bb.nodes4q.data(), std::min<size_t>(nodes_cap, bb.nodes4q.size()) * sizeof(Bvh4QNode));
    if (order_out) memcpy(order_out, bb.order.data(), (size_t)n_triangles * sizeof(uint32_t));
    return PPG_OK;
}
static void decodeChildBox(const Bvh4QNode &q, int k, float lo[3], float hi[3]) {
    const float s[3] = {BvhBuilder::scaleOf(q.exps & 255u), BvhBuilder::scaleOf((q.exps >> 8) & 255u), BvhBuilder::scaleOf((q.exps >> 16) & 255u)};
    const float org[3] = {q.ox, q.oy, q.oz};
    const unsigned int ql[3] = {q.qlox, q.qloy, q.qloz}, qh[3] = {q.qhix, q.qhiy, q.qhiz};
    for (int a = 0; a < 3; ++a) {
        lo[a] = org[a] + (float)((ql[a] >> (8 * k)) & 255u) * s[a];
        hi[a] = org[a] + (float)((qh[a] >> (8 * k)) & 255u) * s[a];
    }
}
int ppg_debug_bvh_stats(const float *positions, const uint32_t *indices, uint32_t n_triangles, float pad_abs, int32_t max_leaf, ppg_bvh_stats *out) {
    if (!positions || !indices || !out || n_triangles == 0) return PPG_ERR_INVALID;
    BvhBuilder bb;
    bb.maxLeaf = std::max(1, std::min(8, (int)max_leaf));
    const auto t0 = std::chrono::steady_clock::now();
    bb.run(positions, indices, n_triangles, pad_abs);
    const auto t1 = std::chrono::steady_clock::now();
    memset(out, 0, sizeof(*out));
    out->build_seconds = std::chrono::duration<double>(t1 - t0).count();
    out->n_nodes = (uint32_t)bb.nodes4q.size();
    out->n_binary_nodes = (uint32_t)bb.nodes.size();
    out->stack_need = (uint32_t)BvhBuilder::stackNeedOf(bb.nodes4);
    auto areaOf = [](const float lo[3], const float hi[3]) {
        const double d[3] = {(double)hi[0] - lo[0], (double)hi[1] - lo[1], (double)hi[2] - lo[2]};
        return d[0] < 0 || d[1] < 0 || d[2] < 0 ? 0.0 : 2 * (d[0] * d[1] + d[1] * d[2] + d[2] * d[0]);
    };
    double rootArea = 0;
    {
        float lo[3] = {INFINITY, INFINITY, INFINITY}, hi[3] = {-INFINITY, -INFINITY, -INFINITY};
        for (int k = 0; k < 4; ++k) {
            if (bb.nodes4q[0].child[k] == PPG_BVH4_EMPTY) continue;
            float l[3], h[3];
// ... 353 lines not shown
    for (uint32_t i = 0; i < n; ++i)
        if (items[i].material < 0 || (uint32_t)items[i].material >= ctx->nMaterials) { ctx->error = "ppg_debug_bsdf: item " + std::to_string(i) + ": material out of range"; return PPG_ERR_INVALID; }
    if (n == 0) return PPG_OK;
    HIP_CHECK(hipSetDevice(ctx->device));
    ctx->quiesce();
    DebugBuf dItems, dOut;
    HIP_CHECK(dItems.fill(items, (size_t)n * sizeof(ppg_debug_bsdf_item)));
    HIP_CHECK(dOut.fill(nullptr, (size_t)n * sizeof(ppg_debug_bsdf_out)));
    const unsigned int block = 64;
    const int family = std::max(sceneFamily(ctx->scene), PPG_FAMILY_EXT);
    launcher(ppg_path_kernels[family].debug_bsdf)((int)((n + block - 1) / block), (int)block, ctx->stream, ctx->scene, n, (const ppg_debug_bsdf_item *)dItems.p, (ppg_debug_bsdf_out *)dOut.p);
    HIP_CHECK(hipGetLastError());
    HIP_CHECK(hipStreamSynchronize(ctx->stream));
    HIP_CHECK(hipMemcpy(out, dOut.p, (size_t)n * sizeof(ppg_debug_bsdf_out), hipMemcpyDeviceToHost));
    return PPG_OK;
}

int ppg_debug_rfilter_table(const ppg_rfilter *f, float table[32], float *radius, int32_t *border) {
    if (!f || !table || !radius || !border) return PPG_ERR_INVALID;
    std::string err;
    return rfilterTable(f, table, radius, border, err);
}

int ppg_release_cached_memory(int32_t device) {
    int prev = 0;
    (void)hipGetDevice(&prev);
    if (hipSetDevice(device) != hipSuccess) return PPG_ERR_DEVICE;
    g_blockCache.trim();
    (void)hipSetDevice(prev);
    return PPG_OK;
}

int ppg_render(ppg_ctx *ctx) {
    NEED_SCENE
    int rc = beginRender(ctx);
    if (rc) return rc;
    rc = ctx->budgetType == 0 ? renderSPP(ctx) : renderTime(ctx);
    if (rc) { ctx->renderOpen = false; return rc; }
    return endRender(ctx);
}

int ppg_read_film(ppg_ctx *ctx, float *rgb) {
    NEED_SCENE
    const int n = ctx->W * ctx->H;
    if (!ctx->d_film.p || !ctx->d_tmp.p) { ctx->error = "nothing rendered"; return PPG_ERR_STATE; }
    hipLaunchKernelGGL(k_normalise, dim3((n + 255) / 256), dim3(256), 0, ctx->stream, n, ctx->d_film.p, ctx->d_filmW.p, ctx->d_tmp.p);
    HIP_CHECK(hipMemcpyAsync(rgb, ctx->d_tmp.p, 3 * (size_t)n * 4, hipMemcpyDeviceToHost, ctx->stream));
    HIP_CHECK(hipStreamSynchronize(ctx->stream));
    return PPG_OK;
}
int ppg_read_variance(ppg_ctx *ctx, float *rgb) {
    NEED_SCENE
    if (!ctx->d_var.p) { ctx->error = "nothing rendered"; return PPG_ERR_STATE; }
    HIP_CHECK(hipMemcpy(rgb, ctx->d_var.p, 3 * (size_t)ctx->W * ctx->H * 4, hipMemcpyDeviceToHost));
    return PPG_OK;
}
int ppg_dump_sdtree(ppg_ctx *ctx, const char *path) { NEED_TREE return dumpSDTreeFile(ctx, path); }

int ppg_sdtree_info_get(ppg_ctx *ctx, ppg_sdtree_info *info) {
    NEED_TREE
    memset(info, 0, sizeof *info);
    info->n_stree_nodes = (uint32_t)ctx->snodes.size();
    std::vector<LeafHdr> dh(ctx->hdr);
    if (ctx->d_hdr.p && ctx->d_hdr.cap >= dh.size()) HIP_CHECK(hipMemcpy(dh.data(), ctx->d_hdr.p, dh.size() * sizeof(LeafHdr), hipMemcpyDeviceToHost));
    for (size_t i = 0; i < ctx->snodes.size(); ++i)
        if (ctx->snodes[i].isLeaf()) { info->n_leaves++; info->n_sampling_nodes += ctx->hdr[i].s_num; info->n_building_nodes += dh[i].b_num; }
    for (int a = 0; a < 3; ++a) { info->aabb_min[a] = ctx->treeMin[a]; info->aabb_max[a] = ctx->treeMax[a]; }
    info->iter = ctx->iter; info->is_built = ctx->isBuilt;
    return PPG_OK;
}

int ppg_sdtree_read_stree(ppg_ctx *ctx, int32_t *axis, uint32_t *children) {
    NEED_TREE
    for (size_t i = 0; i < ctx->snodes.size(); ++i) { axis[i] = ctx->snodes[i].axis; children[2 * i] = ctx->snodes[i].child[0]; children[2 * i + 1] = ctx->snodes[i].child[1]; }
    return PPG_OK;
}

int ppg_sdtree_read_dtree_headers(ppg_ctx *ctx, int32_t which, uint64_t *offset, uint32_t *num_nodes, int32_t *max_depth, float *sum, double *stat_weight) {
    NEED_TREE
    std::vector<LeafHdr> dh(ctx->hdr.size());
    std::vector<unsigned long long> bw(ctx->hdr.size(), 0);
    { int rc = foldWeights(ctx); if (rc) return rc; }
    if (ctx->d_hdr.p) {
        HIP_CHECK(hipMemcpy(dh.data(), ctx->d_hdr.p, dh.size() * sizeof(LeafHdr), hipMemcpyDeviceToHost));
        HIP_CHECK(hipMemcpy(bw.data(), ctx->d_bweight.p, bw.size() * 8, hipMemcpyDeviceToHost));
    } else dh = ctx->hdr;
    uint64_t off = 0;
    for (size_t i = 0; i < ctx->snodes.size(); ++i) {
        if (!ctx->snodes[i].isLeaf()) { offset[i] = 0; num_nodes[i] = 0; max_depth[i] = 0; sum[i] = 0; stat_weight[i] = 0; continue; }
        const LeafHdr &h = dh[i];
        offset[i] = off;
        if (which == 0) { num_nodes[i] = h.s_num; max_depth[i] = h.s_depth; sum[i] = h.s_sum; stat_weight[i] = h.s_statw; off += h.s_num; }
        else {
            num_nodes[i] = h.b_num; max_depth[i] = h.b_depth; sum[i] = 0.0f;
            stat_weight[i] = (double)bw[i] / 16777216.0;
            off += h.b_num;
        }
    }
    return PPG_OK;
}

int ppg_sdtree_read_dtree_nodes(ppg_ctx *ctx, int32_t which, float *sums, uint16_t *children, uint64_t *fixed_sums) {
    NEED_TREE
    std::vector<float> s; std::vector<uint16_t> c; std::vector<uint64_t> f;
    int rc = gatherDTrees(ctx, which, s, c, fixed_sums ? &f : nullptr);
    if (rc) return rc;
// ... 132 lines not shown
    hipLaunchKernelGGL((k_adam_state<true>), dim3((nNodes + 255u) / 256u), dim3(256), 0, ctx->stream, ctx->d_hdr.p, nNodes, ctx->d_adamState.p);
    HIP_CHECK(hipStreamSynchronize(ctx->stream));
    return PPG_OK;
}
int ppg_adam_records_replace(ppg_ctx *ctx, const void *dev_records, uint64_t n) {
    NEED_TREE
    if (!ctx->inHook) { ctx->error = "ppg_adam_records_replace: only valid inside the round hook"; return PPG_ERR_STATE; }
    if (n > 0xfffffff0ull) { ctx->error = "too many Adam records in one round"; return PPG_ERR_NOMEM; }
    if (n && dev_records == (const void *)ctx->d_adamRecs.p) { ctx->error = "ppg_adam_records_replace: source aliases the destination"; return PPG_ERR_INVALID; }
    HIP_CHECK(ctx->d_adamRecs.reserve(std::max<size_t>(1, (size_t)n)));
    if (n) HIP_CHECK(hipMemcpyAsync(ctx->d_adamRecs.p, dev_records, (size_t)n * sizeof(AdamRec), hipMemcpyDeviceToDevice, ctx->stream));
    HIP_CHECK(hipStreamSynchronize(ctx->stream));
    ctx->hookReplaced = true; ctx->hookCount = n;
    return PPG_OK;
}

int ppg_query_pdf(ppg_ctx *ctx, uint32_t n, const float *positions, const float *dirs, float *pdf_out) {
    NEED_TREE
    if (n == 0) return PPG_OK;
    DevBuf<float> dp, dd, dout;
    HIP_CHECK(dp.reserve(3 * (size_t)n)); HIP_CHECK(dd.reserve(3 * (size_t)n)); HIP_CHECK(dout.reserve(n));
    HIP_CHECK(hipMemcpy(dp.p, positions, 12 * (size_t)n, hipMemcpyHostToDevice));
    HIP_CHECK(hipMemcpy(dd.p, dirs, 12 * (size_t)n, hipMemcpyHostToDevice));
    hipLaunchKernelGGL(k_query_pdf, dim3((n + 255) / 256), dim3(256), 0, ctx->stream, ctx->devTree(), n, dp.p, dd.p, dout.p);
    HIP_CHECK(hipStreamSynchronize(ctx->stream));
    HIP_CHECK(hipMemcpy(pdf_out, dout.p, 4 * (size_t)n, hipMemcpyDeviceToHost));
    return PPG_OK;
}
int ppg_query_sample(ppg_ctx *ctx, uint32_t n, const float *positions, uint64_t seed, float *dirs_out) {
    NEED_TREE
    if (n == 0) return PPG_OK;
    DevBuf<float> dp, dout;
    HIP_CHECK(dp.reserve(3 * (size_t)n)); HIP_CHECK(dout.reserve(3 * (size_t)n));
    HIP_CHECK(hipMemcpy(dp.p, positions, 12 * (size_t)n, hipMemcpyHostToDevice));
    hipLaunchKernelGGL(k_query_sample, dim3((n + 255) / 256), dim3(256), 0, ctx->stream, ctx->devTree(), n, dp.p, (unsigned long long)seed, dout.p);
    HIP_CHECK(hipStreamSynchronize(ctx->stream));
    HIP_CHECK(hipMemcpy(dirs_out, dout.p, 12 * (size_t)n, hipMemcpyDeviceToHost));
    return PPG_OK;
}

int ppg_set_adam_regions(ppg_ctx *ctx, int32_t regions) {
    if (!ctx || regions < 0 || regions > 4096) { if (ctx) ctx->error = "ppg_set_adam_regions: 0 .. 4096"; return PPG_ERR_INVALID; }
    ctx->adamRegions = regions >= 2 ? regions : 0;
    return PPG_OK;
}

int ppg_debug_set_defer_depth(ppg_ctx *ctx, int32_t depth) {
    if (!ctx || depth < 1 || depth > 64) return PPG_ERR_INVALID;
    ctx->deferDepthAdam = depth;
    return PPG_OK;
}

int ppg_enable_kernel_timing(ppg_ctx *ctx, int32_t enable) {
    ctx->timer.reset();
    ctx->bvhNodesVisited = ctx->bvhTrisTested = 0; ctx->tailLongestSum = 0; ctx->shadeCommonRays = 0;
    ctx->timer.enabled = enable != 0;
    return PPG_OK;
}
int ppg_kernel_times(ppg_ctx *ctx, ppg_kernel_time *out, uint32_t cap, uint32_t *n) {
    ctx->timer.resolve();
    uint32_t k = 0;
    for (size_t i = 0; i < ctx->timer.names.size() && k < cap; ++i, ++k) {
        out[k].name = ctx->timer.names[i].c_str(); out[k].ms = ctx->timer.ms[i]; out[k].launches = ctx->timer.launches[i]; out[k].units = ctx->timer.units[i];
        if (ctx->timer.names[i] == "k_shade<common>") out[k].units = ctx->shadeCommonRays;
        else if (ctx->timer.names[i] == "k_shade<rest>") out[k].units = ctx->timer.units[i] > ctx->shadeCommonRays ? ctx->timer.units[i] - ctx->shadeCommonRays : 0;
    }
    if (k + 2 <= cap && ctx->bvhNodesVisited) {
        out[k].name = "bvh_nodes_visited"; out[k].ms = 0; out[k].launches = 0; out[k].units = ctx->bvhNodesVisited; ++k;
        out[k].name = "bvh_triangles_tested"; out[k].ms = 0; out[k].launches = 0; out[k].units = ctx->bvhTrisTested; ++k;
    }
    if (k + 1 <= cap && ctx->tailLongestSum) { out[k].name = "tail_longest_paths_sum"; out[k].ms = 0; out[k].launches = 0; out[k].units = ctx->tailLongestSum; ++k; }
    *n = k;
    return PPG_OK;
}

}
```

### practical-path-guiding_amd/csrc/ppg_host_kernels.h

```cpp
#ifndef PPG_HOST_KERNELS_H
#define PPG_HOST_KERNELS_H

#include "ppg_kernels.h"

static __global__ __launch_bounds__(PPG_BLOCK) void k_generate(PathState P, DevScene S, RenderParams R, Queues Q) {
    for (unsigned int i = blockIdx.x * blockDim.x + threadIdx.x; i < P.n_paths; i += gridDim.x * blockDim.x) {
        unsigned int k = i % P.n_pix, j = i / P.n_pix;
        unsigned int pixel = P.pixels[k];
        const unsigned int sample = R.group_samples ? R.pass_index_spp + (j / R.group_samples) * R.group_stride + (j % R.group_samples) : R.pass_index_spp + j;
        unsigned int key = ppg_path_key(R.seed, pixel, sample);
        unsigned int dim = 0;
        float u1 = ppg_rand(key, dim++);
        float u2 = ppg_rand(key, dim++);
        int px = (int)(pixel % (unsigned int)S.cam.width), py = (int)(pixel / (unsigned int)S.cam.width);
        float sx = (float)px + u1, sy = (float)py + u2;
        F3 nearP = xf_point(S.cam.s2c, f3(sx * S.cam.inv_w, sy * S.cam.inv_h, 0.0f));
        F3 dl, o;
        if (S.cam.lens) {
            const float u3 = ppg_rand(key, dim++);
            const float u4 = ppg_rand(key, dim++);
            float ax, ay;
            disk_concentric(u3, u4, ax, ay);
            ax = ax * S.cam.aperture; ay = ay * S.cam.aperture;
            const float fDist = S.cam.focus / nearP.z;
// ... 17 lines not shown

static __global__ void k_build_grid(const int4 *stree, unsigned int *grid) {
    unsigned int c = blockIdx.x * blockDim.x + threadIdx.x;
    if (c >= PPG_GRID_DIM * PPG_GRID_DIM * PPG_GRID_DIM) return;
    unsigned int coord[3] = {c % PPG_GRID_DIM, (c / PPG_GRID_DIM) % PPG_GRID_DIM, c / (PPG_GRID_DIM * PPG_GRID_DIM)};
    int used[3] = {0, 0, 0};
    int idx = 0, depth = 0;
    for (; depth < PPG_GRID_LEVELS; ++depth) {
        int4 n = stree[idx];
        if (n.y == 0) break;
        int a = n.x;
        unsigned int bit = (coord[a] >> (PPG_GRID_BITS - 1 - used[a])) & 1u;
        ++used[a];
        idx = bit ? n.z : n.y;
    }
    grid[c] = (unsigned int)idx | ((unsigned int)depth << 27);
}

static __global__ void k_gather_slices(const unsigned int *items, const unsigned int *count, const unsigned int *offsets, unsigned int cap,
                                unsigned int *dense) {
    const unsigned int b = blockIdx.x, n = count[b], off = offsets[b];
    for (unsigned int k = threadIdx.x; k < n; k += blockDim.x) dense[off + k] = items[(size_t)b * cap + k];
}

static __global__ __launch_bounds__(1024) void k_scan_counts(const unsigned int *counts, unsigned int *offsets, unsigned int n, unsigned long long *total_out,
                                                      unsigned int *bounce_count, unsigned int *stop, unsigned int stop_below) {
    __shared__ unsigned long long part[1024];
    __shared__ unsigned long long carry;
    const bool stopped = stop && *stop;
    if (threadIdx.x == 0) carry = 0;
    __syncthreads();
    if (stopped) return;
    for (unsigned int start = 0; start < n; start += 1024) {
        unsigned int i = start + threadIdx.x;
        unsigned long long v = i < n ? counts[i] : 0;
        part[threadIdx.x] = v;
        __syncthreads();
        for (unsigned int off = 1; off < 1024; off <<= 1) {
            unsigned long long t = threadIdx.x >= off ? part[threadIdx.x - off] : 0;
            __syncthreads();
            part[threadIdx.x] += t;
            __syncthreads();
        }
        if (i < n) offsets[i] = (unsigned int)(carry + part[threadIdx.x] - v);
        __syncthreads();
        if (threadIdx.x == 1023) carry += part[1023];
        __syncthreads();
    }
    if (threadIdx.x == 0) {
        *total_out = carry;
        if (bounce_count) *bounce_count = (unsigned int)carry;
        if (stop && carry < (unsigned long long)stop_below) *stop = 1u;
    }
}

static __global__ void k_fold_replicas(unsigned long long *compact, unsigned long long *rep, unsigned int n_nodes) {
    unsigned int i = blockIdx.x * blockDim.x + threadIdx.x;
    if (i >= n_nodes) return;
    unsigned long long s = 0;
    for (int r = 0; r < PPG_REPLICAS; ++r) {
        unsigned long long v = rep[(size_t)i * PPG_REPLICAS + r];
        if (v) { s += v; rep[(size_t)i * PPG_REPLICAS + r] = 0; }
    }
    if (s) compact[i] += s;
}

static __global__ void k_path_nv(PathState P, unsigned int *nv, const unsigned char *straggler, unsigned int max_vertices) {
    unsigned int i = blockIdx.x * blockDim.x + threadIdx.x;
    if (i < P.n_paths) nv[i] = (straggler && straggler[i]) ? max_vertices : (P.misc[i].z & FL_NV_MASK) >> FL_NV_SHIFT;
}
static __global__ void k_commit_prepare(PathState P, uint4 *misc_out, unsigned char *nv8, const unsigned char *straggler) {
    unsigned int i = blockIdx.x * blockDim.x + threadIdx.x;
    if (i >= P.n_paths) return;
    const uint4 m = P.misc[i];
    if (misc_out) misc_out[i] = m;
    nv8[i] = (straggler && straggler[i]) ? (unsigned char)0 : (unsigned char)((m.z & FL_NV_MASK) >> FL_NV_SHIFT);
}
static __global__ void k_commit_prepare_list(PathState P, const unsigned int *list, const unsigned long long *list_n, unsigned char *nv8) {
    const unsigned int n = (unsigned int)*list_n;
    for (unsigned int k = blockIdx.x * blockDim.x + threadIdx.x; k < n; k += gridDim.x * blockDim.x)
        nv8[k] = (unsigned char)((P.misc[list[k]].z & FL_NV_MASK) >> FL_NV_SHIFT);
}
static __global__ void k_mark_list(const unsigned int *list, const unsigned long long *list_n, unsigned char *flag) {
    const unsigned int n = (unsigned int)*list_n;
    for (unsigned int k = blockIdx.x * blockDim.x + threadIdx.x; k < n; k += gridDim.x * blockDim.x) flag[list[k]] = 1;
}
static __global__ void k_iota_total(unsigned int *a, unsigned int n, unsigned long long *total) {
    for (unsigned int i = blockIdx.x * blockDim.x + threadIdx.x; i < n; i += gridDim.x * blockDim.x) a[i] = i;
    if (blockIdx.x == 0 && threadIdx.x == 0) *total = n;
}
static __global__ void k_iota(unsigned int *a, unsigned int n) {
    unsigned int i = blockIdx.x * blockDim.x + threadIdx.x;
    if (i < n) a[i] = i;
}
static __global__ void k_extract_vertices(PathState P, PathState Ps, unsigned int n, unsigned int max_vertices) {
    const unsigned int q = threadIdx.x & 3u;
    for (unsigned int j = (blockIdx.x * blockDim.x + threadIdx.x) >> 2; j < n; j += (gridDim.x * blockDim.x) >> 2) {
        const unsigned int i = Ps.orig[j];
        unsigned int nv = ((Ps.misc[j].z & FL_NV_MASK) >> FL_NV_SHIFT) + 1u;
        if (nv > max_vertices) nv = max_vertices;
        for (unsigned int v = q; v < nv; v += 4u) {
            const size_t a = (size_t)v * P.n_paths + i, b = (size_t)v * Ps.n_paths + j;
            Ps.v_d[b] = P.v_d[a]; Ps.v_thr[b] = P.v_thr[a]; Ps.v_bsdf[b] = P.v_bsdf[a]; Ps.v_rad[b] = P.v_rad[a];
            if (P.v_o) { Ps.v_o[b] = P.v_o[a]; Ps.v_vox[b] = P.v_vox[a]; }
        }
        if (q == 0 && P.nee_cos) Ps.nee_cos[j] = P.nee_cos[i];
// ... 573 lines not shown
```

### practical-path-guiding_amd/host/guided_path_hip.h

```cpp
#ifndef GUIDED_PATH_HIP_H
#define GUIDED_PATH_HIP_H

#include <algorithm>
#include <atomic>
#include <chrono>
#include <cstdarg>
#include <cmath>
#include <cstdio>
#include <functional>
#include <limits>
#include <map>
#include <stdexcept>
#include <string>
#include <vector>

#include "../../include/ppg.h"

namespace ppg {

struct SceneData {
    std::vector<float> positions, normals;
    std::vector<uint32_t> indices, triMaterial;
    std::vector<int32_t> triEmitter;
    std::vector<ppg_material> materials;
// ... 120 lines not shown
        check(ppg_set_shapes(m_ctx, scene.shapes.data(), (uint32_t)scene.shapes.size()), "ppg_set_shapes");
        check(ppg_set_microfacet(m_ctx, scene.microfacet.data(), (uint32_t)scene.microfacet.size()), "ppg_set_microfacet");
        check(ppg_set_coatings(m_ctx, scene.coatings.data(), (uint32_t)scene.coatings.size()), "ppg_set_coatings");
        check(ppg_set_blends(m_ctx, scene.blends.data(), (uint32_t)scene.blends.size()), "ppg_set_blends");
        check(ppg_set_scene(m_ctx, &sv), "ppg_set_scene");
        check(ppg_set_rfilter(m_ctx, scene.hasRFilter ? &scene.rfilter : nullptr), "ppg_set_rfilter");
        check(ppg_set_lens(m_ctx, scene.hasLens ? &scene.lens : nullptr), "ppg_set_lens");
        if (reducer) check(ppg_set_shard(m_ctx, reducer->rank(), reducer->world(), 32), "ppg_set_shard");
        m_w = scene.camera.width; m_h = scene.camera.height;
        {
            const int rc = ppg_begin_render(m_ctx);
            if (reducer) {
                if (rc != PPG_OK) reducer->setLocalStatus(1);
                const int bad = reducer->stopDecision(0);
                if (rc == PPG_ERR_CANCELLED) return false;
                check(rc, "ppg_begin_render");
                if (bad) throw std::runtime_error("render aborted: a rank could not start (cancelled or failed before its first exchange)");
            } else {
                if (rc == PPG_ERR_CANCELLED) return false;
                check(rc, "ppg_begin_render");
            }
        }
        if (reducer && std::string(m_cfg.bsdfSamplingFractionLoss) != "none") check(ppg_set_pass_hook(m_ctx, &GuidedPathTracerHIP::roundHook, this), "ppg_set_pass_hook");
        check(ppg_set_stop_hook(m_ctx, (reducer && !spp) ? &GuidedPathTracerHIP::stopHook : nullptr, this), "ppg_set_stop_hook");
        say(log, fmt("Starting render job (%ix%i, MI355X%s) ..", m_w, m_h, reducer ? fmt(", rank %d of %d", reducer->rank(), reducer->world()).c_str() : ""));
        bool ok = spp ? renderSPP(log) : renderTime(log);
        if (ok && reducer && !m_filmComplete && std::string(m_cfg.sampleCombination) != "inversevar") reducer->reduceFilm(m_ctx, m_w, m_h);
        if (ok) check(ppg_end_render(m_ctx), "ppg_end_render");
        return ok;
    }

    std::vector<float> film() {
        std::vector<float> rgb((size_t)m_w * m_h * 3);
        check(ppg_read_film(m_ctx, rgb.data()), "ppg_read_film");
        return rgb;
    }
    ppg_ctx *context() { return m_ctx; }

private:
    static std::string fmt(const char *f, ...) __attribute__((format(printf, 1, 2))) {
        char buf[1024];
        va_list ap; va_start(ap, f); vsnprintf(buf, sizeof buf, f, ap); va_end(ap);
        return buf;
    }
    static void say(const LogFn &log, const std::string &s) { if (log) log(s); }
    void check(int rc, const char *what) {
        rethrowHookError();
        if (rc != PPG_OK && rc != PPG_ERR_CANCELLED) throw std::runtime_error(std::string(what) + ": " + ppg_last_error(m_ctx));
    }

    bool passes(int n, ppg_pass_stats &st, const LogFn &log, bool finalGroups = false) {
        say(log, fmt("Rendering %d render passes.", n));
        int rc;
        if (!m_reducer) {
            rc = ppg_render_passes(m_ctx, n, &st);
            check(rc, "ppg_render_passes");
        } else {
            rc = ppg_render_passes_nostat(m_ctx, n);
            if (rc != PPG_OK || m_hookError) m_reducer->setLocalStatus(1);
            try {
                if (finalGroups && m_reducer->world() > 1) {
                    const uint64_t px = (uint64_t)m_w * m_h, G = (uint64_t)ppg_final_group_passes(n);
                    const uint64_t expect = 4 * px + (((uint64_t)n + G - 1) / G) * 7 * px;
                    void *dev = nullptr;
                    uint64_t nFloats = 0;
                    if (ppg_final_partials(m_ctx, &dev, &nFloats) != PPG_OK || nFloats != expect) { m_reducer->setLocalStatus(1); dev = nullptr; }
                    m_reducer->reduceFinalPartials(m_ctx, dev, expect);
                    m_filmComplete = true;
                } else m_reducer->reduceImages(m_ctx, m_w, m_h);
            } catch (...) { if (!m_hookError) m_hookError = std::current_exception(); }
            if (rc == PPG_ERR_CANCELLED || m_cancelled.load()) { m_hookError = nullptr; return false; }
            check(rc, "ppg_render_passes_nostat");
            rethrowHookError();
            check(ppg_finish_passes(m_ctx, &st), "ppg_finish_passes");
        }
        const float ttuv = (float)st.seconds * st.variance, stuv = st.passes_rendered_local * m_cfg.sppPerPass * st.variance;
        say(log, fmt("%.2f seconds, Total passes: %d, Var: %f, TTUV: %f, STUV: %f.", st.seconds, st.passes_rendered_total, st.variance, ttuv, stuv));
        m_passesRendered = st.passes_rendered_total;
        return rc == PPG_OK;
    }
    void build(const LogFn &log, bool nothingRecorded = false) {
        if (m_reducer && !nothingRecorded) m_reducer->reduceSDTree(m_ctx);
        say(log, "Building distributions for sampling.");
        ppg_tree_stats t;
        check(ppg_build_sdtree(m_ctx, &t), "ppg_build_sdtree");
        say(log, fmt("Distribution statistics:\n  Depth         = [%d, %f, %d]\n  Mean radiance = [%f, %f, %f]\n  Node count    = [%llu, %f, %llu]\n"
                     "  Stat. weight  = [%f, %f, %f]\n",
                     t.min_depth, t.avg_depth, t.max_depth, t.min_mean_radiance, t.avg_mean_radiance, t.max_mean_radiance,
                     (unsigned long long)t.min_nodes, t.avg_nodes, (unsigned long long)t.max_nodes, t.min_stat_weight, t.avg_stat_weight,
                     t.max_stat_weight));
    }
    bool doNeeWithSpp(int spp) const {
        const std::string nee = m_cfg.nee;
        return nee == "never" ? false : (nee == "kickstart" ? spp < 128 : true);
    }

    bool renderSPP(const LogFn &log) {
        const size_t sampleCount = (size_t)m_cfg.budget;
        const int nPasses = (int)std::ceil(sampleCount / (float)m_cfg.sppPerPass);
        float currentVarAtEnd = std::numeric_limits<float>::infinity();
        const bool automatic = std::string(m_cfg.sampleCombination) == "automatic";
        int iter = 0;
        m_passesRendered = 0;
        while (m_passesRendered < nPasses) {
            const int sppRendered = m_passesRendered * m_cfg.sppPerPass;
            ppg_set_do_nee(m_ctx, doNeeWithSpp(sppRendered));
            int remainingPasses = nPasses - m_passesRendered;
            int passesThisIteration = std::min(remainingPasses, 1 << iter);
            if (remainingPasses - passesThisIteration < 2 * passesThisIteration) passesThisIteration = remainingPasses;
            say(log, fmt("ITERATION %d, %d passes", iter, passesThisIteration));
            say(log, "Resetting distributions for sampling.");
            bool isFinal = passesThisIteration >= remainingPasses;
            const bool recorded = !isFinal;
            check(ppg_begin_iteration(m_ctx, isFinal), "ppg_begin_iteration");
            m_filmComplete = false;
            ppg_pass_stats st;
            if (!passes(passesThisIteration, st, log, isFinal)) return false;
            const float lastVarAtEnd = currentVarAtEnd;
            currentVarAtEnd = passesThisIteration * st.variance / remainingPasses;
            say(log, fmt("Extrapolated var:\n  Last:    %f\n  Current: %f\n", lastVarAtEnd, currentVarAtEnd));
            remainingPasses -= passesThisIteration;
            if (automatic && remainingPasses > 0 && (remainingPasses < passesThisIteration || (sppRendered > 256 && currentVarAtEnd > lastVarAtEnd))) {
                say(log, fmt("FINAL %d passes", remainingPasses));
                ppg_set_final(m_ctx, 1);
                isFinal = true;
                if (!passes(remainingPasses, st, log, true)) return false;
            }
            build(log, !recorded);
            check(ppg_end_iteration(m_ctx), "ppg_end_iteration");
            ++iter;
        }
        return true;
    }

    bool renderTime(const LogFn &log) {
        const float nSeconds = m_cfg.budget;
        float currentVarAtEnd = std::numeric_limits<float>::infinity();
        const bool automatic = std::string(m_cfg.sampleCombination) == "automatic";
        const auto start = std::chrono::steady_clock::now();
        auto elapsed = [&](std::chrono::steady_clock::time_point t0) {
            const float local = (float)std::chrono::duration_cast<std::chrono::milliseconds>(std::chrono::steady_clock::now() - t0).count() / 1000;
            return m_reducer ? (float)m_reducer->broadcast(local) : local;
        };
        float elapsedSeconds = 0;
        int iter = 0;
        m_passesRendered = 0;
        while (elapsedSeconds < nSeconds) {
            const int sppRendered = m_passesRendered * m_cfg.sppPerPass;
            ppg_set_do_nee(m_ctx, doNeeWithSpp(sppRendered));
            float remainingTime = nSeconds - elapsedSeconds;
            const int passesThisIteration = 1 << iter;
            say(log, fmt("ITERATION %d, %d passes", iter, passesThisIteration));
            const auto startIter = std::chrono::steady_clock::now();
            check(ppg_begin_iteration(m_ctx, 0), "ppg_begin_iteration");
            ppg_pass_stats st;
            if (!passes(passesThisIteration, st, log)) return false;
            const float secondsIter = elapsed(startIter);
            const float lastVarAtEnd = currentVarAtEnd;
            currentVarAtEnd = secondsIter * st.variance / remainingTime;
            remainingTime -= secondsIter;
            if (automatic && remainingTime > 0 && (remainingTime < secondsIter || (sppRendered > 256 && currentVarAtEnd > lastVarAtEnd))) {
                say(log, fmt("FINAL %f seconds", remainingTime));
                ppg_set_final(m_ctx, 1);
                do {
                    if (!passes(passesThisIteration, st, log)) return false;
                    elapsedSeconds = elapsed(start);
                } while (elapsedSeconds < nSeconds);
            }
            build(log);
            check(ppg_end_iteration(m_ctx), "ppg_end_iteration");
            ++iter;
            elapsedSeconds = elapsed(start);
        }
        return true;
    }

    static int stopHook(void *self, int localStop) {
        GuidedPathTracerHIP *g = static_cast<GuidedPathTracerHIP *>(self);
        if (g->m_cancelled.load() || localStop == PPG_STOP_CANCELLED) g->m_reducer->setLocalStatus(1);
        try { return g->m_reducer->stopDecision(localStop); } catch (...) { if (!g->m_hookError) g->m_hookError = std::current_exception(); return 1; }
    }
    static int footprintHook(void *self, void *dev, uint64_t nFloats, int32_t localStatus) {
        GuidedPathTracerHIP *g = static_cast<GuidedPathTracerHIP *>(self);
        if (!g->m_reducer) return 1;
        if (localStatus != 0 || g->m_cancelled.load()) g->m_reducer->setLocalStatus(1);
        try { g->m_reducer->reduceFootprint(dev, nFloats); return 0; } catch (...) { if (!g->m_hookError) g->m_hookError = std::current_exception(); return 1; }
    }
    static int roundHook(void *self) {
        GuidedPathTracerHIP *g = static_cast<GuidedPathTracerHIP *>(self);
        if (g->m_cancelled.load()) g->m_reducer->setLocalStatus(1);
        try { g->m_reducer->reduceAdamRecords(g->m_ctx); return 0; } catch (...) { if (!g->m_hookError) g->m_hookError = std::current_exception(); return 1; }
    }
    void rethrowHookError() { if (m_hookError) { std::exception_ptr e = m_hookError; m_hookError = nullptr; std::rethrow_exception(e); } }

    Reducer *m_reducer = nullptr;
    std::atomic<bool> m_cancelled{false};
    bool m_filmComplete = false;
    std::exception_ptr m_hookError;
    ppg_config m_cfg;
    ppg_ctx *m_ctx = nullptr;
    std::string m_str[7];
    int m_w = 0, m_h = 0, m_passesRendered = 0;
};

}
#endif
```

### practical-path-guiding_amd/ppg_host/bindings.py

```python
import ctypes as C
import os

import numpy as np

_HERE = os.path.dirname(os.path.abspath(__file__))
_PKG = os.path.dirname(_HERE)


def hip_library_path():
    return os.environ.get("PPG_HIP_LIB") or os.path.join(_PKG, "lib", "libppg_hip.so")


class PPGError(RuntimeError):
    def __init__(self, code, msg):
        super().__init__("ppg error %d: %s" % (code, msg))
        self.code = code


class Config(C.Structure):
    _fields_ = [
        ("nee", C.c_char_p), ("sampleCombination", C.c_char_p), ("spatialFilter", C.c_char_p),
        ("directionalFilter", C.c_char_p), ("bsdfSamplingFractionLoss", C.c_char_p),
        ("sdTreeMaxMemory", C.c_int32), ("sTreeThreshold", C.c_int32), ("dTreeThreshold", C.c_float),
        ("bsdfSamplingFraction", C.c_float), ("sppPerPass", C.c_int32), ("budgetType", C.c_char_p),
# ... 701 lines not shown
        items["material"] = material
        items["wi"] = np.broadcast_to(np.asarray(wi, np.float32), (n, 3))
        items["wo"] = wo
        items["sample"] = np.broadcast_to(np.asarray(sample, np.float32), (n, 2))
        items["key"] = 0 if key is None else key
        items["uv"] = 0.0 if uv is None else np.broadcast_to(np.asarray(uv, np.float32), (n, 2))
        out = np.zeros(n, DEBUG_BSDF_OUT_DTYPE)
        assert items.itemsize == C.sizeof(DebugBsdfItem) and out.itemsize == C.sizeof(DebugBsdfOut)
        self._call("debug_bsdf", C.c_uint32(n), items.ctypes.data_as(C.POINTER(DebugBsdfItem)), out.ctypes.data_as(C.POINTER(DebugBsdfOut)))
        return out

    def set_lens(self, lens):
        self._lens = None if lens is None else Lens.from_dict(lens)
        self._call("set_lens", None if self._lens is None else C.byref(self._lens))

    def set_rfilter(self, rfilter):
        self._rfilter = RFilter.from_dict(rfilter)
        self._call("set_rfilter", C.byref(self._rfilter))

    def set_shard(self, rank, world, tile_size=32):
        self._call("set_shard", C.c_int32(rank), C.c_int32(world), C.c_int32(tile_size))

    def render(self):
        self._call("render")

    def begin_render(self):
        self._call("begin_render")

    def begin_iteration(self, is_final):
        self._call("begin_iteration", C.c_int32(int(is_final)))

    def set_final(self, is_final):
        self._call("set_final", C.c_int32(int(is_final)))

    def set_adam_regions(self, regions):
        self._call("set_adam_regions", C.c_int32(int(regions)))

    def set_do_nee(self, v):
        self._call("set_do_nee", C.c_int32(int(v)))

    def render_passes(self, n):
        st = PassStats()
        self._call("render_passes", C.c_int32(n), C.byref(st))
        return st

    def render_passes_nostat(self, n):
        self._call("render_passes_nostat", C.c_int32(n))

    def finish_passes(self):
        st = PassStats()
        self._call("finish_passes", C.byref(st))
        return st

    def build_sdtree(self):
        st = TreeStats()
        self._call("build_sdtree", C.byref(st))
        return st

    def end_iteration(self):
        self._call("end_iteration")

    def end_render(self):
        self._call("end_render")

    def cancel(self):
        self._call("cancel")

    def read_film(self):
        out = np.empty((self.height, self.width, 3), np.float32)
        self._call("read_film", _fp(out))
        return out

    def read_variance(self):
        out = np.empty((self.height, self.width, 3), np.float32)
        self._call("read_variance", _fp(out))
        return out

    def dump_sdtree(self, path):
        self._call("dump_sdtree", path.encode())

    def sdtree_info(self):
        info = SDTreeInfo()
        self._call("sdtree_info_get", C.byref(info))
        return info

    def read_sdtree(self):
        info = self.sdtree_info()
        n = info.n_stree_nodes
        axis = np.zeros(n, np.int32)
        children = np.zeros((n, 2), np.uint32)
        self._call("sdtree_read_stree", _p(axis, C.c_int32), _p(children, C.c_uint32))
        out = {"axis": axis, "children": children, "n_leaves": info.n_leaves, "iter": info.iter,
               "aabb_min": np.array(info.aabb_min[:], np.float32), "aabb_max": np.array(info.aabb_max[:], np.float32)}
        for which, name, total in ((0, "sampling", info.n_sampling_nodes), (1, "building", info.n_building_nodes)):
            off = np.zeros(n, np.uint64)
            nn = np.zeros(n, np.uint32)
            md = np.zeros(n, np.int32)
            sm = np.zeros(n, np.float32)
            sw = np.zeros(n, np.float64)
            self._call("sdtree_read_dtree_headers", C.c_int32(which), _p(off, C.c_uint64), _p(nn, C.c_uint32),
                       _p(md, C.c_int32), _fp(sm), _p(sw, C.c_double))
            total = int(total)
            sums = np.zeros((total, 4), np.float32)
            ch = np.zeros((total, 4), np.uint16)
            fx = np.zeros((total, 4), np.uint64)
            self._call("sdtree_read_dtree_nodes", C.c_int32(which), _fp(sums), _p(ch, C.c_uint16), _p(fx, C.c_uint64))
# ... 139 lines not shown
```

### practical-path-guiding_amd/ppg_host/integrator.py

```python
import math
import time

from .bindings import Engine


class GuidedPathTracer:
    def __init__(self, engine=None, reducer=None, log=None, **props):
        self.engine = engine if engine is not None else Engine.hip(**props)
        self.props = self.engine.props
        self.reducer = reducer
        self.log = log
        self.iterations = []

    def _passes(self, n):
        e = self.engine
        if self.reducer is None:
            return e.render_passes(n)
        failure = None
        try:
            e.render_passes_nostat(n)
        except Exception as ex:
            failure = ex
            self.reducer.status = 1
        try:
            if self._final and self.props["budgetType"] == "spp" and self.reducer.world > 1:
                expect = e.final_partials_expected(n)
                ptr, count = None, 0
                if failure is None:
                    try:
                        ptr, count = e.final_partials()
                    except Exception as ex:
                        failure = ex
                if count != expect:
                    self.reducer.status, ptr = 1, None
                self.reducer.reduce_final_partials(e, ptr, expect)
                self._film_complete = True
            else:
                self.reducer.reduce_images(e)
        except Exception:
            if failure is None:
                raise
        if failure is not None:
            raise failure
        return e.finish_passes()

    def _build(self):
        if self.reducer is not None and self._recorded:
            self.reducer.reduce_sdtree(self.engine)
        return self.engine.build_sdtree()

    def cancel(self):
        self._cancelled = True
        self.engine.cancel()

    def _do_nee(self, spp):
        nee = self.props["nee"]
        return False if nee == "never" else (spp < 128 if nee == "kickstart" else True)

    def render(self, scene=None):
        e, p = self.engine, self.props
        if scene is not None:
            if self.reducer is not None:
                from .distributed import check_shardable
                check_shardable(scene, self.reducer)
                self.reducer.install(e)
            e.set_scene(scene)
        self._cancelled = False
        if self.reducer is not None:
            self.reducer.begin_render()
        try:
            e.begin_render()
        except Exception:
            if self.reducer is None:
                raise
            self.reducer.status = 1
            self.reducer.stop_decision(0)
            raise
        if self.reducer is not None and self.reducer.stop_decision(0):
            from .distributed import RenderAborted
            raise RenderAborted("render aborted: a rank could not start (cancelled or failed before its first exchange)")
        clock = (lambda v: self.reducer.broadcast(v)) if self.reducer is not None else (lambda v: v)
        def stop_hook(local):
            if self._cancelled or local == 2:
                self.reducer.status = 1
            return self.reducer.stop_decision(local)
        e.set_stop_hook(stop_hook if (self.reducer is not None and p["budgetType"] != "spp") else None)
        e.set_pass_hook(None)
        if self.reducer is not None and p["bsdfSamplingFractionLoss"] != "none":
            def round_hook():
                if self._cancelled:
                    self.reducer.status = 1
                self.reducer.reduce_adam(e)
            e.set_pass_hook(round_hook)
        self.iterations = []
        self._film_complete = False
        spp = p["sppPerPass"]
        automatic = p["sampleCombination"] == "automatic"
        it, passes_rendered = 0, 0
        current_var_at_end = float("inf")
        t_start = time.monotonic()
        if p["budgetType"] == "spp":
            n_passes = int(math.ceil(int(p["budget"]) / float(spp)))
            while passes_rendered < n_passes:
                spp_rendered = passes_rendered * spp
                e.set_do_nee(self._do_nee(spp_rendered))
                remaining = n_passes - passes_rendered
                this_iter = min(remaining, 1 << it)
                if remaining - this_iter < 2 * this_iter:
                    this_iter = remaining
                self._final = this_iter >= remaining
                self._recorded = not self._final
                self._film_complete = False
                e.begin_iteration(self._final)
                st = self._passes(this_iter)
                rec = dict(iter=it, passes=this_iter, stats=[st.as_dict()])
                passes_rendered += st.passes_rendered_local
                last_var_at_end = current_var_at_end
                current_var_at_end = this_iter * st.variance / remaining
                remaining -= this_iter
                if automatic and remaining > 0 and (remaining < this_iter or (spp_rendered > 256 and current_var_at_end > last_var_at_end)):
                    self._final = True
                    e.set_final(True)
                    st = self._passes(remaining)
                    rec["final_passes"] = remaining
                    rec["stats"].append(st.as_dict())
                    passes_rendered += st.passes_rendered_local
                rec["tree"] = self._build().as_dict()
                e.end_iteration()
                self.iterations.append(rec)
                if self.log:
                    self.log(rec)
                it += 1
        else:
            n_seconds = float(p["budget"])
            elapsed = 0.0
            while elapsed < n_seconds:
                spp_rendered = passes_rendered * spp
                e.set_do_nee(self._do_nee(spp_rendered))
                remaining_time = n_seconds - elapsed
                this_iter = 1 << it
                t_iter = time.monotonic()
                self._final = False
                self._recorded = True
                e.begin_iteration(False)
                st = self._passes(this_iter)
                rec = dict(iter=it, passes=this_iter, stats=[st.as_dict()])
                passes_rendered += st.passes_rendered_local
                seconds_iter = clock(time.monotonic() - t_iter)
                last_var_at_end = current_var_at_end
                current_var_at_end = seconds_iter * st.variance / remaining_time
                remaining_time -= seconds_iter
                if automatic and remaining_time > 0 and (remaining_time < seconds_iter or (spp_rendered > 256 and current_var_at_end > last_var_at_end)):
                    self._final = True
                    e.set_final(True)
                    while True:
                        st = self._passes(this_iter)
                        rec["stats"].append(st.as_dict())
                        passes_rendered += st.passes_rendered_local
                        elapsed = clock(time.monotonic() - t_start)
                        if elapsed >= n_seconds:
                            break
                rec["tree"] = self._build().as_dict()
                e.end_iteration()
                self.iterations.append(rec)
                if self.log:
                    self.log(rec)
                it += 1
                elapsed = clock(time.monotonic() - t_start)
        if self.reducer is not None and not self._film_complete:
            self.reducer.reduce_film(e, inverse_variance=(p["sampleCombination"] == "inversevar"))
        e.end_render()
        return e.read_film()
```

Baseline: 253.6 Msamples/s.

## Defer pass-stat readback and launch next iteration's first bounce early

Pass statistics are no longer read back synchronously at the end of each iteration. They are owed and resolved later, when the next iteration starts or when they are queried. The host also tells the context how many passes come next, so the first bounce of the next iteration (generate plus first trace) can be launched early, while the SD-tree build runs on the host. The runner checks that this early bounce exactly matches the parameters of the real launch before reusing it, and otherwise discards it. This removes host-device sync bubbles between iterations, at the cost of extra state, a second stats buffer and the chance of wasted work when the early bounce is discarded.

Result: no change. 254.2 Msamples/s (median of 3 runs) (+0.2%).

```diff
diff --git a/include/ppg.h b/include/ppg.h
--- a/include/ppg.h
+++ b/include/ppg.h
@@ -299,6 +299,11 @@
 int ppg_render_passes_nostat(ppg_ctx *ctx, int32_t n_passes);
 int ppg_finish_passes(ppg_ctx *ctx, ppg_pass_stats *stats);
 
+int ppg_finish_passes_deferred(ppg_ctx *ctx);
+int ppg_pass_stats_resolve(ppg_ctx *ctx, ppg_pass_stats *stats);
+
+int ppg_hint_next_passes(ppg_ctx *ctx, int32_t n_passes, int32_t is_final, int32_t do_nee);
+
 #define PPG_STOP_CANCELLED 2
 typedef int (*ppg_stop_hook)(void *user, int local_stop);
 int ppg_set_stop_hook(ppg_ctx *ctx, ppg_stop_hook hook, void *user);
diff --git a/include/ppg_testhooks.h b/include/ppg_testhooks.h
--- a/include/ppg_testhooks.h
+++ b/include/ppg_testhooks.h
@@ -29,6 +29,8 @@
 
 struct ppg_ctx;
 int ppg_debug_set_defer_depth(struct ppg_ctx *ctx, int32_t depth);
+
+int ppg_schedule_counters(struct ppg_ctx *ctx, uint64_t *out, uint32_t cap);
 
 struct ppg_debug_hit {
     int32_t prim;
diff --git a/practical-path-guiding_amd/csrc/ppg_batch_plan.h b/practical-path-guiding_amd/csrc/ppg_batch_plan.h
--- a/practical-path-guiding_amd/csrc/ppg_batch_plan.h
+++ b/practical-path-guiding_amd/csrc/ppg_batch_plan.h
@@ -134,6 +134,94 @@
     return {(int)std::max(1u, std::min(1024u, (n + laneLimit * (kBlock / 64u) - 1u) / (laneLimit * (kBlock / 64u)))), laneLimit};
 }
 
+struct FirstBounce {
+    bool launched = false;
+    unsigned int n_paths = 0, n_pix = 0;
+    const unsigned int *pixels = nullptr;
+    unsigned int pass_index_spp = 0, group_samples = 0, group_stride = 0;
+    unsigned long long seed = 0;
+    int grid = 0, gridAll = 0;
+    bool sorted = false;
+    bool do_nee = false;
+    bool small = false;
+};
+
+inline bool sameFirstBounce(const FirstBounce &early, const FirstBounce &own) {
+    return early.launched && early.n_paths == own.n_paths && early.n_pix == own.n_pix && early.pixels == own.pixels &&
+           early.pass_index_spp == own.pass_index_spp && early.group_samples == own.group_samples && early.group_stride == own.group_stride &&
+           early.seed == own.seed && early.grid == own.grid && early.gridAll == own.gridAll && early.sorted == own.sorted &&
+           early.do_nee == own.do_nee && early.small == own.small;
+}
+
+inline bool sortFirstBounce(bool fullMaterials, bool commonSplit, bool doNee, bool tuneNoSortFirst, bool haveSortBuffers) {
+    return fullMaterials && commonSplit && !doNee && !tuneNoSortFirst && haveSortBuffers;
+}
+
+struct NextPasses { bool set = false; int passes = 0; bool isFinal = false, doNee = false; };
+
+struct EarlyFacts {
+    bool tuneNoEarly = false;
+    int world = 1;
+    bool passHook = false, stopHook = false, footHook = false;
+    bool timerOn = false, tuneNoOverlap = false;
+    bool spp = true;
+    bool regionRounds = false;
+    bool cancelled = false;
+};
+inline bool earlyBounceAllowed(const NextPasses &hint, const EarlyFacts &f) {
+    return hint.set && hint.passes > 0 && !f.tuneNoEarly && f.world == 1 && !f.passHook && !f.stopHook && !f.footHook && f.spp &&
+           sideStreamsAllowed(f.timerOn, f.tuneNoOverlap) && !f.regionRounds && !f.cancelled;
+}
+
+struct FirstLaunch { int passes = 0; unsigned int firstPass = 0, groupPasses = 0, stridePasses = 0; };
+
+inline FirstLaunch firstLaunchOfBatches(int numPasses, int passesPerBatch, unsigned int passesRendered) {
+    FirstLaunch l;
+    l.passes = std::min(passesPerBatch, numPasses); l.firstPass = passesRendered;
+    return l;
+}
+inline FirstLaunch firstLaunchOfFinalGroups(int numPasses, unsigned int G, unsigned int launchPasses, unsigned int passesRendered) {
+    FirstLaunch l;
+    const unsigned int nGroups = ((unsigned int)numPasses + G - 1) / G;
+    l.firstPass = passesRendered;
+    if (G <= launchPasses) {
+        const unsigned int cnt = std::min(std::max(1u, launchPasses / G), nGroups);
+        unsigned int batch = 0;
+        for (unsigned int g = 0; g < cnt; ++g) batch += std::min(G, (unsigned int)numPasses - g * G);
+        l.passes = (int)batch; l.groupPasses = G; l.stridePasses = G;
+    } else {
+        const unsigned int batch = std::min(launchPasses, std::min(G, (unsigned int)numPasses));
+        l.passes = (int)batch; l.groupPasses = batch; l.stridePasses = batch;
+    }
+    return l;
+}
+
+struct FirstBounceFacts {
+    unsigned int nPix = 0;
+    const unsigned int *pixels = nullptr;
+    int sppPerPass = 1;
+    unsigned long long seed = 0;
+    int nBlocks = 0, tuneBlocksSmall = 0;
+    size_t tuneSmallPaths = 0;
+    unsigned int queueCap = 0;
+    bool fullMaterials = false, commonSplit = false, tuneNoSortFirst = false, haveSortBuffers = false, small = false;
+    bool doNee = false;
+};
+inline int gridOverPaths(size_t n) { return (int)std::max<size_t>(1, std::min<size_t>((n + kBlock - 1) / kBlock, (size_t)256 * 8)); }
+inline FirstBounce firstBounceOf(const FirstLaunch &l, const FirstBounceFacts &f) {
+    FirstBounce r;
+    r.n_pix = f.nPix; r.pixels = f.pixels;
+    r.n_paths = (unsigned int)((size_t)f.nPix * (size_t)f.sppPerPass * (size_t)l.passes);
+    r.pass_index_spp = l.firstPass * (unsigned int)f.sppPerPass;
+    r.group_samples = l.groupPasses * (unsigned int)f.sppPerPass; r.group_stride = l.stridePasses * (unsigned int)f.sppPerPass;
+    r.seed = f.seed;
+    r.grid = wavefrontGrid(f.nBlocks, f.tuneBlocksSmall, f.tuneSmallPaths, r.n_paths, f.queueCap);
+    r.gridAll = gridOverPaths(r.n_paths);
+    r.sorted = sortFirstBounce(f.fullMaterials, f.commonSplit, f.doNee, f.tuneNoSortFirst, f.haveSortBuffers);
+    r.do_nee = f.doNee; r.small = f.small;
+    return r;
+}
+
 struct RoundReadback {
     unsigned int live[64];
     unsigned int slowCount, slowOverflow;
diff --git a/practical-path-guiding_amd/csrc/ppg_hip.hip b/practical-path-guiding_amd/csrc/ppg_hip.hip
--- a/practical-path-guiding_amd/csrc/ppg_hip.hip
+++ b/practical-path-guiding_amd/csrc/ppg_hip.hip
@@ -214,6 +214,9 @@
 
 struct GroupLaunch { unsigned int firstPass, groupPasses, stridePasses, slot0, slotStride; bool wholeFilm; unsigned int addCount; bool groupsDone = true; bool exchange = false; };
 
+struct ppg_ctx;
+namespace { int resolvePassStats(ppg_ctx *ctx); }
+
 struct ppg_ctx {
     int nee = 0, sampleCombination = 1, spatialFilter = 0, directionalFilter = 0, loss = 0, budgetType = 1;
     int sdTreeMaxMemory = -1, sTreeThreshold = 12000, sppPerPass = 4, rrDepth = 5, maxDepth = -1;
@@ -240,6 +243,8 @@
         if (stream3) (void)hipStreamSynchronize(stream3);
         if (stream4) (void)hipStreamSynchronize(stream4);
         if (stream) (void)hipStreamSynchronize(stream);
+        (void)resolvePassStats(this);
+        early = FirstBounce{}; nextHint = NextPasses{};
         for (Stragglers &g : strag) { g.pending = false; g.aside = false; g.film = nullptr; }
     }
     hipStream_t stream4 = nullptr;
@@ -426,11 +431,32 @@
     bool isBuilt = false, isFinalIter = false, doNee = false;
     int iter = 0, passesRendered = 0, passesRenderedThisIter = 0, passesLocal = 0;
     std::chrono::steady_clock::time_point startTime, passStart;
+    bool passStartRecorded = false;
     std::atomic<bool> cancelled{false};
     bool cancelSeen = false;
     bool seesCancel() { if (!cancelled.load()) return false; cancelSeen = true; return true; }
     float lastVariance = 0;
     ppg_pass_stats lastStats{};
+    struct OwedStats {
+        bool owed = false;
+        int W = 0, H = 0, N = 0, nBlocks = 0, iter = 0;
+        unsigned int nTails = 0;
+        bool inverseVar = false, timed = false;
+        ppg_pass_stats s{};
+        std::chrono::steady_clock::time_point passStart;
+        hipEvent_t startEv = nullptr;
+    } owedStats;
+    hipEvent_t evStats = nullptr, evPassStart[2] = {nullptr, nullptr};
+    int passStartCur = 0;
+    unsigned int *h_tailLongest = nullptr;
+    bool tuneNoDeferredStats = false;
+    uint64_t statsDeferred = 0, statsResolvedBusy = 0;
+    NextPasses nextHint;
+    FirstBounce early;
+    DevBuf<BlockStats> d_statsEarly;
+    size_t pathCap = 0;
+    bool tuneNoEarlyBounce = false;
+    uint64_t earlyLaunched = 0, earlyUsed = 0, earlyDiscarded = 0;
     KernelTimer timer;
 #define PPG_TAIL_LOG 256
     DevBuf<unsigned int> d_tailLongest;
@@ -503,6 +529,8 @@
 }
 
 bool sideStreamsAllowed(const ppg_ctx *ctx) { return ppg_plan::sideStreamsAllowed(ctx->timer.enabled, ctx->tuneNoOverlap); }
+bool mayDeferStats(const ppg_ctx *ctx);
+int resolvePassStatsBusy(ppg_ctx *ctx);
 
 int gridFor(size_t n, int block = PPG_BLOCK, int maxBlocks = 256 * 8) {
     size_t b = (n + block - 1) / block;
@@ -723,6 +751,7 @@
     if (n > 0xfffffff0ull || nFinal > 0xfffffff0ull) { ctx->error = "too many paths per pass"; return PPG_ERR_INVALID; }
     const size_t nTrain = std::max<size_t>(1, n);
     size_t nn = std::max<size_t>(1, std::max(n, nFinal));
+    ctx->pathCap = nn;
     ctx->maxVertices = PPG_MAX_VERTICES;
     if (ctx->maxDepth > 0) ctx->maxVertices = std::max(1, std::min(PPG_MAX_VERTICES, ctx->maxDepth - 1));
     ctx->aosPaths = ctx->tunePathLayout ? ctx->tunePathLayout == 2 : (ctx->maxDepth < 0 && ctx->scene.n_tris > 64);
@@ -736,7 +765,7 @@
     const size_t chunks = (nn + PPG_DCHUNK - 1) / PPG_DCHUNK;
     const size_t cap = ((chunks + nb - 1) / nb) * PPG_DCHUNK;
     for (int k = 0; k < 2; ++k) { HIP_CHECK(ctx->d_queue[k].reserve(cap * nb)); HIP_CHECK(ctx->d_qcount[k].reserve(nb)); }
-    HIP_CHECK(ctx->d_stats.reserve(nb)); HIP_CHECK(ctx->d_qtotal.reserve(1));
+    HIP_CHECK(ctx->d_stats.reserve(nb)); HIP_CHECK(ctx->d_statsEarly.reserve(nb)); HIP_CHECK(ctx->d_qtotal.reserve(1));
     HIP_CHECK(ctx->d_offsets.reserve(nb)); HIP_CHECK(ctx->d_total.reserve(2));
     HIP_CHECK(ctx->d_bounceCounts.reserve(72)); HIP_CHECK(ctx->d_ticket.reserve(1));
     HIP_CHECK(ctx->d_adamCount.reserve(2));
@@ -1249,6 +1278,79 @@
     return PPG_OK;
 }
 
+size_t tailLdsBytes(const ppg_ctx *ctx, bool smallScene) { return smallScene ? (size_t)ctx->ldsTris * 48 : (size_t)PPG_LDS_STACK * PPG_BLOCK * 4; }
+size_t traceLdsBytes(const ppg_ctx *ctx, bool smallScene) {
+    return smallScene ? tailLdsBytes(ctx, true) : (size_t)PPG_TRACE_STACK * PPG_BLOCK * 4 + (PPG_BLOCK / 64) * sizeof(PairLds);
+}
+void launchGenerate(ppg_ctx *ctx, const PathState &P, const DevScene &S, const RenderParams &R, const Queues &Q, int gridAll) {
+    hipLaunchKernelGGL(k_generate, dim3(gridAll), dim3(PPG_BLOCK), 0, ctx->stream, P, S, R, Q);
+}
+void launchTrace(ppg_ctx *ctx, const PathState &P, const DevScene &S, const Queues &Q, int grid, int qin, bool sortSlices, bool smallScene, size_t traceLds) {
+    unsigned int *const trSorted = sortSlices ? ctx->d_queueSorted.p : nullptr;
+    unsigned char *const trKeys = sortSlices ? ctx->d_sortKeys.p : nullptr;
+    TraceLaunch a{grid, traceLds, ctx->stream, P, S, Q, qin, smallScene ? 0 : ctx->ldsNodes, ctx->ldsTris, trSorted, trKeys, smallScene, ctx->timer.enabled};
+    launcher(ppg_path_kernels[sceneFamily(S)].trace)(a);
+}
+
+unsigned int finalLaunchPasses(const ppg_ctx *ctx, unsigned int G, unsigned int minePasses, size_t pixels) {
+    unsigned int launchPasses = (unsigned int)ctx->maxBatchFinal;
+    if (ctx->tuneFinalHalves && ctx->maxDepth < 0 && ctx->tuneSplitDepth > 0 && sideStreamsAllowed(ctx) && minePasses >= 2 && minePasses <= launchPasses &&
+        pixels * (size_t)ctx->sppPerPass * (size_t)(minePasses / 2) >= ((size_t)1 << 21)) {
+        launchPasses = (minePasses + 1) / 2;
+        if (G < launchPasses) launchPasses = std::max(G, launchPasses / G * G);
+    }
+    return launchPasses;
+}
+
+int launchEarlyBounce(ppg_ctx *ctx, const NextPasses &hint) {
+    ctx->early = FirstBounce{};
+    const bool rounds = ctx->loss != LOSS_NONE && !hint.isFinal;
+    EarlyFacts ef;
+    ef.tuneNoEarly = ctx->tuneNoEarlyBounce; ef.world = ctx->shardWorld;
+    ef.passHook = ctx->passHook != nullptr; ef.stopHook = ctx->stopHook != nullptr; ef.footHook = ctx->footHook != nullptr;
+    ef.timerOn = ctx->timer.enabled; ef.tuneNoOverlap = ctx->tuneNoOverlap; ef.spp = ctx->budgetType == 0;
+    ef.regionRounds = rounds && ctx->adamRegions > 1 && hint.passes <= PPG_ADAM_REGION_MAX_PASSES;
+    ef.cancelled = ctx->cancelled.load();
+    if (!earlyBounceAllowed(hint, ef)) return PPG_OK;
+    const PathState &base = ctx->paths;
+    FirstLaunch l;
+    if (hint.isFinal) {
+        const unsigned int G = (unsigned int)ppg_final_group_passes(hint.passes);
+        l = firstLaunchOfFinalGroups(hint.passes, G, finalLaunchPasses(ctx, G, (unsigned int)hint.passes, (size_t)ctx->nPixAll), (unsigned int)ctx->passesRendered);
+    } else {
+        const int perBatch = rounds ? (int)ppg_adam_round_passes(ctx->sppPerPass, ctx->W, ctx->H, hint.passes) : ctx->maxBatch;
+        l = firstLaunchOfBatches(hint.passes, perBatch, (unsigned int)ctx->passesRendered);
+    }
+    const bool smallScene = isSmallScene(ctx);
+    FirstBounceFacts bf;
+    bf.nPix = base.n_pix; bf.pixels = base.pixels; bf.sppPerPass = ctx->sppPerPass; bf.seed = ctx->seed;
+    bf.nBlocks = ctx->nBlocks; bf.tuneBlocksSmall = ctx->tuneBlocksSmall; bf.tuneSmallPaths = ctx->tuneSmallPaths; bf.queueCap = ctx->queues.cap;
+    bf.fullMaterials = ctx->fullMaterials; bf.commonSplit = ctx->queues.n_common != nullptr; bf.tuneNoSortFirst = ctx->tuneNoSortFirst;
+    bf.haveSortBuffers = ctx->d_queueSorted.p != nullptr; bf.small = smallScene; bf.doNee = hint.doNee;
+    FirstBounce r = firstBounceOf(l, bf);
+    if (r.n_paths == 0 || (size_t)r.n_paths > ctx->pathCap || (ctx->maxDepth >= 0 && ctx->maxDepth < 1)) return PPG_OK;
+    hipStream_t s = ctx->stream;
+    PathState P = base;
+    P.n_paths = r.n_paths;
+    RenderParams R = ctx->params();
+    R.spp = ctx->sppPerPass * l.passes; R.is_final_iter = hint.isFinal; R.do_nee = hint.doNee;
+    R.pass_index_spp = r.pass_index_spp; R.group_samples = r.group_samples; R.group_stride = r.group_stride;
+    Queues Q = ctx->queues;
+    unsigned int *counts = ctx->d_bounceCounts.p;
+    Q.stop = counts + 64;
+    Q.dense_n = ctx->d_total.p;
+    Q.stats = ctx->d_statsEarly.p;
+    HIP_CHECK(hipMemsetAsync(ctx->d_statsEarly.p, 0, sizeof(BlockStats) * (size_t)ctx->nBlocks, s));
+    launchGenerate(ctx, P, ctx->scene, R, Q, r.gridAll);
+    HIP_CHECK(hipMemsetAsync(counts, 0, 72 * 4, s));
+    launchTrace(ctx, P, ctx->scene, Q, r.grid, QIN_FIRST, r.sorted, smallScene, traceLdsBytes(ctx, smallScene));
+    HIP_CHECK(hipGetLastError());
+    r.launched = true;
+    ctx->early = r;
+    ++ctx->earlyLaunched;
+    return PPG_OK;
+}
+
 int runWavefront(ppg_ctx *ctx, Batch &B) {
     const PathState &P = B.P;
     const DevScene &S = B.S;
@@ -1259,24 +1361,32 @@
     const bool neeOn = ctx->doNee;
     const bool fullMats = ctx->fullMaterials;
     const size_t triBytes = (size_t)ctx->scene.n_tris * 48;
-    const size_t traceLds = smallScene ? B.ldsBytes : (size_t)PPG_TRACE_STACK * PPG_BLOCK * 4 + (PPG_BLOCK / 64) * sizeof(PairLds);
+    const size_t traceLds = traceLdsBytes(ctx, smallScene);
     const unsigned int stopBelow = B.plan.stopBelow;
     int qin = QIN_FIRST;
-    timedLaunch(ctx, "k_generate", P.n_paths, [&] { hipLaunchKernelGGL(k_generate, dim3(B.gridAll), dim3(PPG_BLOCK), 0, s, P, S, B.R, Q); });
+    FirstBounce own;
+    own.n_paths = P.n_paths; own.n_pix = P.n_pix; own.pixels = P.pixels;
+    own.pass_index_spp = B.R.pass_index_spp; own.group_samples = B.R.group_samples; own.group_stride = B.R.group_stride; own.seed = B.R.seed;
+    own.grid = grid; own.gridAll = B.gridAll;
+    own.sorted = sortFirstBounce(fullMats, Q.n_common != nullptr, neeOn, ctx->tuneNoSortFirst, ctx->d_queueSorted.p != nullptr);
+    own.do_nee = neeOn; own.small = smallScene;
+    const bool early = !ctx->timer.enabled && sameFirstBounce(ctx->early, own);
+    if (ctx->early.launched) ++(early ? ctx->earlyUsed : ctx->earlyDiscarded);
+    ctx->early = FirstBounce{};
+    unsigned int *counts = ctx->d_bounceCounts.p;
+    Q.stop = counts + 64;
+    Q.dense_n = ctx->d_total.p;
+    if (!early) {
+        timedLaunch(ctx, "k_generate", P.n_paths, [&] { launchGenerate(ctx, P, S, B.R, Q, B.gridAll); });
+        HIP_CHECK(hipMemsetAsync(counts, 0, 72 * 4, s));
+    }
     const int maxBounces = planBounces(ctx->survival, P.n_paths, stopBelow, ctx->maxDepth, ctx->tuneBulkBounces, ctx->bounceMargin, B.plan.adamFast, ctx->deferDepthAdam);
     const bool liveCount = ctx->timer.enabled;
-    unsigned int *counts = ctx->d_bounceCounts.p;
-    HIP_CHECK(hipMemsetAsync(counts, 0, 72 * 4, s));
-    Q.stop = counts + 64;
-    Q.dense_n = ctx->d_total.p;
     for (int b = 0; b < maxBounces; ++b) {
-        const bool sortSlices = fullMats && (qin == QIN_DENSE || (Q.n_common && !neeOn && !ctx->tuneNoSortFirst)) && ctx->d_queueSorted.p;
-        unsigned int *const trSorted = sortSlices ? ctx->d_queueSorted.p : nullptr;
-        unsigned char *const trKeys = sortSlices ? ctx->d_sortKeys.p : nullptr;
-        timedLaunch(ctx, "k_trace", B.hostCount, [&] {
-            TraceLaunch a{grid, traceLds, s, P, S, Q, qin, smallScene ? 0 : ctx->ldsNodes, ctx->ldsTris, trSorted, trKeys, smallScene, ctx->timer.enabled};
-            launcher(ppg_path_kernels[sceneFamily(S)].trace)(a);
-        });
+        const bool sortSlices = qin == QIN_DENSE ? (fullMats && ctx->d_queueSorted.p) : own.sorted;
+        if (early && b == 0)
+            hipLaunchKernelGGL(k_add_block_stats, dim3((grid + 255) / 256), dim3(256), 0, s, Q.stats, ctx->d_statsEarly.p, (unsigned int)grid);
+        else timedLaunch(ctx, "k_trace", B.hostCount, [&] { launchTrace(ctx, P, S, Q, grid, qin, sortSlices, smallScene, traceLds); });
         int shadeIn = sortSlices ? QIN_SORTED : qin;
         ctx->joinTree();
         const bool split = shadeIn == QIN_SORTED && Q.n_common && !neeOn;
@@ -1391,6 +1501,7 @@
     if (plan.tail || plan.fastRound) {
         if (plan.tail) HIP_CHECK(hipMemcpyAsync(h->live, ctx->d_bounceCounts.p, sizeof h->live, hipMemcpyDeviceToHost, s));
         if (plan.splitTail) HIP_CHECK(hipMemcpyAsync(&h->handed, ctx->d_total.p, 8, hipMemcpyDeviceToHost, s));
+        { int rc = resolvePassStatsBusy(ctx); if (rc) return rc; }
         HIP_CHECK(hipStreamSynchronize(s));
         if (plan.tail) {
             const int ran = observeBounces(ctx->survival, h->live, B.bouncesRun, P.n_paths, plan.stopBelow);
@@ -1419,6 +1530,16 @@
         HIP_CHECK(G.count.reserve(2)); HIP_CHECK(G.ticket.reserve(1));
         HIP_CHECK(hipMemsetAsync(G.count.p, 0, 16, s));
         { int rc = launchTailAndEndedCommit(ctx, B, plan.deferDepth, handed); if (rc) return rc; }
+        bool listAside = false;
+        if (plan.overlap) {
+            if (plan.beside) {
+                HIP_CHECK(hipEventRecord(ctx->evFork, s));
+                HIP_CHECK(hipStreamWaitEvent(ctx->stream2, ctx->evFork, 0));
+                launchCommit(ctx, B, ctx->stream2, CommitSet::List);
+                HIP_CHECK(hipEventRecord(ctx->evJoin, ctx->stream2));
+                listAside = true;
+            } else launchCommitTimed(ctx, B, CommitSet::List, 0);
+        }
         HIP_CHECK(hipMemcpyAsync(&h->stragglers, G.count.p, 8, hipMemcpyDeviceToHost, s));
         HIP_CHECK(hipStreamSynchronize(s));
         B.nStrag = (unsigned int)h->stragglers;
@@ -1428,7 +1549,7 @@
             if (!rc) rc = launchStragglers(ctx, B);
             if (rc) return rc;
         }
-        if (plan.overlap) launchCommitTimed(ctx, B, CommitSet::List, 0);
+        if (listAside) HIP_CHECK(hipStreamWaitEvent(s, ctx->evJoin, 0));
     } else if (plan.overlap) {
         int rc = launchTailAndEndedCommit(ctx, B, 0u, 0);
         if (rc) return rc;
@@ -1524,17 +1645,9 @@
     std::vector<unsigned int> mine;
     for (unsigned int g = byRank ? rank : 0u; g < nGroups; g += byRank ? world : 1u) mine.push_back(g);
     auto passesOf = [&](unsigned int g) { return std::min(G, (unsigned int)numPasses - g * G); };
-    unsigned int launchPasses = (unsigned int)ctx->maxBatchFinal;
-    {
-        unsigned int minePasses = 0;
-        for (unsigned int g : mine) minePasses += passesOf(g);
-        const size_t pixels = byRank || world == 1 ? n : (size_t)ctx->nPix;
-        if (ctx->tuneFinalHalves && ctx->maxDepth < 0 && ctx->tuneSplitDepth > 0 && sideStreamsAllowed(ctx) && minePasses >= 2 && minePasses <= launchPasses &&
-            pixels * (size_t)ctx->sppPerPass * (size_t)(minePasses / 2) >= ((size_t)1 << 21)) {
-            launchPasses = (minePasses + 1) / 2;
-            if (G < launchPasses) launchPasses = std::max(G, launchPasses / G * G);
-        }
-    }
+    unsigned int minePasses = 0;
+    for (unsigned int g : mine) minePasses += passesOf(g);
+    const unsigned int launchPasses = finalLaunchPasses(ctx, G, minePasses, byRank || world == 1 ? n : (size_t)ctx->nPix);
     const bool exch = ctx->exchangesFootprints() && !byRank;
     auto exchangeGroup = [&](unsigned int g) -> int {
         int rc = flushStragglers(ctx, false);
@@ -1618,6 +1731,8 @@
 
 int renderPassesBody(ppg_ctx *ctx, int numPasses) {
     size_t n = (size_t)ctx->W * ctx->H;
+    const NextPasses hint = ctx->nextHint;
+    ctx->nextHint = NextPasses{};
     HIP_CHECK(hipMemsetAsync(ctx->d_image.p, 0, 3 * n * 4, ctx->stream));
     HIP_CHECK(hipMemsetAsync(ctx->d_sq.p, 0, 3 * n * 4, ctx->stream));
     HIP_CHECK(hipMemsetAsync(ctx->d_imageW.p, 0, n * 4, ctx->stream));
@@ -1625,6 +1740,12 @@
     HIP_CHECK(ctx->d_tailLongest.reserve(PPG_TAIL_LOG + 1));
     HIP_CHECK(hipMemsetAsync(ctx->d_tailLongest.p, 0, (PPG_TAIL_LOG + 1) * 4, ctx->stream));
     ctx->tailLaunches = 0;
+    ctx->passStartRecorded = false;
+    if (mayDeferStats(ctx)) {
+        ctx->passStartCur ^= 1;
+        HIP_CHECK(hipEventRecord(ctx->evPassStart[ctx->passStartCur], ctx->stream));
+        ctx->passStartRecorded = true;
+    }
     ctx->passStart = std::chrono::steady_clock::now();
     ctx->passesLocal = 0;
     const bool rounds = ctx->loss != LOSS_NONE && ctx->isBuilt && !ctx->isFinalIter;
@@ -1669,6 +1790,7 @@
             HIP_CHECK(hipStreamSynchronize(ctx->stream));
         }
     }
+    if (!drain) { int rc = launchEarlyBounce(ctx, hint); if (rc) return rc; }
     {
         const bool deferRounds = rounds && ctx->maxDepth < 0 && recordPositionsKnown(ctx->spatialFilter, ctx->doNee, ctx->nee);
         int rc = flushStragglers(ctx, deferRounds && ctx->passHook != nullptr);
@@ -1705,8 +1827,13 @@
     return rc;
 }
 
-int finishPasses(ppg_ctx *ctx, ppg_pass_stats *st) {
+bool mayDeferStats(const ppg_ctx *ctx) {
+    return ctx->sampleCombination != 1 && ctx->budgetType == 0 && !ctx->stopHook && ctx->shardWorld == 1 && !ctx->timer.enabled && !ctx->tuneNoDeferredStats;
+}
+
+int enqueuePassStats(ppg_ctx *ctx, bool timed) {
     if (ctx->partialsPending) { ctx->error = "the groups of this final iteration were not exchanged: ppg_final_partials / ppg_final_partials_commit before ppg_finish_passes"; return PPG_ERR_STATE; }
+    { int rc = resolvePassStats(ctx); if (rc) return rc; }
     const int n = ctx->W * ctx->H;
     const int N = ctx->passesLocal * ctx->sppPerPass;
     if (ctx->sampleCombination == 2) {
@@ -1715,39 +1842,77 @@
         hipLaunchKernelGGL(k_normalise, dim3((n + 255) / 256), dim3(256), 0, ctx->stream, n, ctx->d_image.p, ctx->d_imageW.p, ctx->images.back().p);
     }
     hipLaunchKernelGGL(k_variance, dim3((n + 255) / 256), dim3(256), 0, ctx->stream, n, ctx->W, N, ctx->d_image.p, ctx->d_sq.p, ctx->d_imageW.p, ctx->d_var.p, ctx->d_lum.p);
-    float *lum = ctx->h_lum;
     if (ctx->h_statsCap < (size_t)ctx->nBlocks) {
         if (ctx->h_stats) (void)hipHostFree(ctx->h_stats);
         ctx->h_stats = nullptr; ctx->h_statsCap = 0;
         HIP_CHECK(hipHostMalloc((void **)&ctx->h_stats, (size_t)ctx->nBlocks * sizeof(BlockStats), hipHostMallocDefault));
         ctx->h_statsCap = (size_t)ctx->nBlocks;
     }
-    BlockStats *bs = ctx->h_stats;
-    HIP_CHECK(hipMemcpyAsync(lum, ctx->d_lum.p, (size_t)n * 4, hipMemcpyDeviceToHost, ctx->stream));
-    HIP_CHECK(hipMemcpyAsync(bs, ctx->d_stats.p, (size_t)ctx->nBlocks * sizeof(BlockStats), hipMemcpyDeviceToHost, ctx->stream));
-    unsigned int tailLongest[PPG_TAIL_LOG];
+    if (!ctx->h_tailLongest) HIP_CHECK(hipHostMalloc((void **)&ctx->h_tailLongest, PPG_TAIL_LOG * sizeof(unsigned int), hipHostMallocDefault));
+    HIP_CHECK(hipMemcpyAsync(ctx->h_lum, ctx->d_lum.p, (size_t)n * 4, hipMemcpyDeviceToHost, ctx->stream));
+    HIP_CHECK(hipMemcpyAsync(ctx->h_stats, ctx->d_stats.p, (size_t)ctx->nBlocks * sizeof(BlockStats), hipMemcpyDeviceToHost, ctx->stream));
     const unsigned int nTails = std::min<unsigned int>(ctx->tailLaunches, PPG_TAIL_LOG);
-    if (nTails) HIP_CHECK(hipMemcpyAsync(tailLongest, ctx->d_tailLongest.p, nTails * 4, hipMemcpyDeviceToHost, ctx->stream));
-    HIP_CHECK(hipStreamSynchronize(ctx->stream));
+    if (nTails) HIP_CHECK(hipMemcpyAsync(ctx->h_tailLongest, ctx->d_tailLongest.p, nTails * 4, hipMemcpyDeviceToHost, ctx->stream));
+    HIP_CHECK(hipEventRecord(ctx->evStats, ctx->stream));
+    ppg_ctx::OwedStats &o = ctx->owedStats;
+    o.owed = true; o.W = ctx->W; o.H = ctx->H; o.N = N; o.nBlocks = ctx->nBlocks; o.nTails = nTails; o.iter = ctx->iter;
+    o.inverseVar = ctx->sampleCombination == 2; o.timed = timed && ctx->passStartRecorded;
+    o.passStart = ctx->passStart; o.startEv = ctx->evPassStart[ctx->passStartCur];
+    o.s = ppg_pass_stats{};
+    o.s.passes_rendered_total = ctx->passesRendered; o.s.passes_rendered_local = ctx->passesLocal; o.s.samples = ctx->samplesLocal;
+    return PPG_OK;
+}
+
+int resolvePassStats(ppg_ctx *ctx) {
+    ppg_ctx::OwedStats &o = ctx->owedStats;
+    if (!o.owed) return PPG_OK;
+    o.owed = false;
+    HIP_CHECK(hipEventSynchronize(ctx->evStats));
+    const float secondsHost = elapsedSeconds(o.passStart);
+    const BlockStats *bs = ctx->h_stats;
+    const float *lum = ctx->h_lum;
+    const int n = o.W * o.H;
     BlockStats c{};
-    for (int k = 0; k < ctx->nBlocks; ++k) { const BlockStats &x = bs[k]; c.rays += x.rays; c.path_len += x.path_len; c.committed += x.committed; c.bvh_nodes += x.bvh_nodes; c.bvh_tris += x.bvh_tris; c.max_len = std::max(c.max_len, x.max_len); c.shade_common += x.shade_common; }
-    if (ctx->debugBatch) fprintf(stderr, "[ppg passes] iter %d passes %d rays %llu path_len_sum %llu longest path finished by k_tail %llu\n", ctx->iter, ctx->passesLocal, (unsigned long long)c.rays, (unsigned long long)c.path_len, (unsigned long long)c.max_len);
+    for (int k = 0; k < o.nBlocks; ++k) { const BlockStats &x = bs[k]; c.rays += x.rays; c.path_len += x.path_len; c.committed += x.committed; c.bvh_nodes += x.bvh_nodes; c.bvh_tris += x.bvh_tris; c.max_len = std::max(c.max_len, x.max_len); c.shade_common += x.shade_common; }
+    if (ctx->debugBatch) fprintf(stderr, "[ppg passes] iter %d passes %d rays %llu path_len_sum %llu longest path finished by k_tail %llu\n", o.iter, o.s.passes_rendered_local, (unsigned long long)c.rays, (unsigned long long)c.path_len, (unsigned long long)c.max_len);
     ctx->bvhNodesVisited += c.bvh_nodes; ctx->bvhTrisTested += c.bvh_tris; ctx->shadeCommonRays += c.shade_common;
-    for (unsigned int k = 0; k < nTails; ++k) ctx->tailLongestSum += tailLongest[k];
+    for (unsigned int k = 0; k < o.nTails; ++k) ctx->tailLongestSum += ctx->h_tailLongest[k];
     float variance = 0;
     for (int k = 0; k < n; ++k) variance += lum[k];
-    variance /= (float)ctx->W * ctx->H * (N - 1);
-    if (ctx->sampleCombination == 2) ctx->variances.push_back(variance);
+    variance /= (float)o.W * o.H * (o.N - 1);
+    if (o.inverseVar) ctx->variances.push_back(variance);
     ctx->lastVariance = variance;
-    ppg_pass_stats s{};
-    s.seconds = elapsedSeconds(ctx->passStart);
-    s.passes_rendered_total = ctx->passesRendered; s.passes_rendered_local = ctx->passesLocal; s.variance = variance;
-    s.samples = ctx->samplesLocal;
+    ppg_pass_stats s = o.s;
+    s.seconds = secondsHost;
+    if (o.timed) {
+        float ms = 0;
+        if (hipEventElapsedTime(&ms, o.startEv, ctx->evStats) == hipSuccess) s.seconds = ms * 1e-3f; else (void)hipGetLastError();
+    }
+    s.variance = variance;
     s.rays = c.rays; s.path_length_sum = c.path_len; s.vertices_committed = c.committed;
     ctx->lastStats = s;
-    if (st) *st = s;
     ctx->timer.resolve();
     return PPG_OK;
+}
+
+int resolvePassStatsBusy(ppg_ctx *ctx) {
+    if (ctx->owedStats.owed) ++ctx->statsResolvedBusy;
+    return resolvePassStats(ctx);
+}
+
+int finishPasses(ppg_ctx *ctx, ppg_pass_stats *st) {
+    int rc = enqueuePassStats(ctx, false);
+    if (!rc) rc = resolvePassStats(ctx);
+    if (!rc && st) *st = ctx->lastStats;
+    return rc;
+}
+
+int finishPassesDeferred(ppg_ctx *ctx) {
+    const bool defer = mayDeferStats(ctx);
+    int rc = enqueuePassStats(ctx, defer);
+    if (!rc && defer) ++ctx->statsDeferred;
+    if (!rc && !defer) rc = resolvePassStats(ctx);
+    return rc;
 }
 
 int allocFilm(ppg_ctx *ctx) {
@@ -1849,6 +2014,7 @@
 int endRender(ppg_ctx *ctx) {
     ctx->joinTree();
     ctx->renderOpen = false;
+    { int rc = resolvePassStats(ctx); if (rc) return rc; }
 #ifdef PPG_PROBE
     if (ctx->d_probe.p) {
         unsigned long long h[PPG_PROBE_SLOTS];
@@ -1897,8 +2063,17 @@
         int rc = beginIteration(ctx, passesThisIteration >= remainingPasses);
         if (rc) return rc;
         ppg_pass_stats st;
+        if (ctx->sampleCombination != 1 && remainingPasses > passesThisIteration) {
+            const int left = remainingPasses - passesThisIteration;
+            int next = std::min(left, 1 << (ctx->iter + 1));
+            if (left - next < 2 * next) next = left;
+            ctx->nextHint.set = true; ctx->nextHint.passes = next; ctx->nextHint.isFinal = next >= left;
+            ctx->nextHint.doNee = doNeeWithSpp(ctx, (ctx->passesRendered + passesThisIteration) * ctx->sppPerPass);
+        }
         if ((rc = renderPassesNoStat(ctx, passesThisIteration))) return rc;
-        if ((rc = finishPasses(ctx, &st))) return rc;
+        const bool defer = mayDeferStats(ctx);
+        st = ppg_pass_stats{};
+        if ((rc = defer ? finishPassesDeferred(ctx) : finishPasses(ctx, &st))) return rc;
         float variance = st.variance;
         const float lastVarAtEnd = currentVarAtEnd;
         currentVarAtEnd = passesThisIteration * variance / remainingPasses;
@@ -2147,6 +2322,8 @@
         if (const char *e = getenv("PPG_SPLIT_DEPTH")) c->tuneSplitDepth = std::max(0, atoi(e));
         c->tuneFinalHalves = getenv("PPG_FINAL_HALVES") != nullptr;
         c->tuneNoTopCut = getenv("PPG_NO_TOPCUT") != nullptr;
+        c->tuneNoDeferredStats = getenv("PPG_NO_DEFERRED_STATS") != nullptr;
+        c->tuneNoEarlyBounce = getenv("PPG_NO_EARLY_BOUNCE") != nullptr;
     }
     if (c->sppPerPass <= 0) { g_createError = "sppPerPass must be > 0"; return PPG_ERR_INVALID; }
     int ndev = 0;
@@ -2158,6 +2335,7 @@
         (e = hipStreamCreate(&c->stream3)) != hipSuccess || (e = hipEventCreateWithFlags(&c->evTreeFork, hipEventDisableTiming)) != hipSuccess ||
         (e = hipStreamCreate(&c->stream4)) != hipSuccess || (e = hipEventCreateWithFlags(&c->evStragFork, hipEventDisableTiming)) != hipSuccess ||
         (e = hipEventCreateWithFlags(&c->evStragDone, hipEventDisableTiming)) != hipSuccess ||
+        (e = hipEventCreate(&c->evStats)) != hipSuccess || (e = hipEventCreate(&c->evPassStart[0])) != hipSuccess || (e = hipEventCreate(&c->evPassStart[1])) != hipSuccess ||
         (e = hipEventCreateWithFlags(&c->evSplatDone, hipEventDisableTiming)) != hipSuccess || (e = hipEventCreateWithFlags(&c->evAdamDone, hipEventDisableTiming)) != hipSuccess) {
         g_createError = std::string("HIP init failed: ") + hipGetErrorString(e);
         return PPG_ERR_DEVICE;
@@ -2174,6 +2352,7 @@
     if (ctx->stream2) (void)hipStreamSynchronize(ctx->stream2);
     if (ctx->stream3) (void)hipStreamSynchronize(ctx->stream3);
     if (ctx->stream4) (void)hipStreamSynchronize(ctx->stream4);
+    (void)resolvePassStats(ctx);
     g_blockCache.settle();
     if (ctx->stream2) (void)hipStreamDestroy(ctx->stream2);
     if (ctx->stream3) (void)hipStreamDestroy(ctx->stream3);
@@ -2182,6 +2361,8 @@
     for (hipEvent_t ev : {ctx->evTreeFork, ctx->evSplatDone, ctx->evAdamDone}) if (ev) (void)hipEventDestroy(ev);
     if (ctx->evFork) (void)hipEventDestroy(ctx->evFork);
     if (ctx->evJoin) (void)hipEventDestroy(ctx->evJoin);
+    for (hipEvent_t ev : {ctx->evStats, ctx->evPassStart[0], ctx->evPassStart[1]}) if (ev) (void)hipEventDestroy(ev);
+    if (ctx->h_tailLongest) (void)hipHostFree(ctx->h_tailLongest);
     ctx->timer.resolve();
     for (auto e : ctx->timer.pool) (void)hipEventDestroy(e);
     if (ctx->h_lum) (void)hipHostFree(ctx->h_lum);
@@ -2233,6 +2414,22 @@
 int ppg_set_do_nee(ppg_ctx *ctx, int32_t do_nee) { ctx->doNee = do_nee != 0; return PPG_OK; }
 int ppg_render_passes_nostat(ppg_ctx *ctx, int32_t n) { NEED_TREE return renderPassesNoStat(ctx, n); }
 int ppg_finish_passes(ppg_ctx *ctx, ppg_pass_stats *st) { NEED_TREE return finishPasses(ctx, st); }
+int ppg_finish_passes_deferred(ppg_ctx *ctx) { NEED_TREE return finishPassesDeferred(ctx); }
+int ppg_pass_stats_resolve(ppg_ctx *ctx, ppg_pass_stats *st) {
+    (void)hipSetDevice(ctx->device);
+    const int rc = resolvePassStats(ctx);
+    if (!rc && st) *st = ctx->lastStats;
+    return rc;
+}
+int ppg_schedule_counters(ppg_ctx *ctx, uint64_t *out, uint32_t cap) {
+    const uint64_t v[5] = {ctx->statsDeferred, ctx->statsResolvedBusy, ctx->earlyLaunched, ctx->earlyUsed, ctx->earlyDiscarded};
+    for (uint32_t k = 0; k < cap; ++k) out[k] = k < 5 ? v[k] : 0;
+    return PPG_OK;
+}
+int ppg_hint_next_passes(ppg_ctx *ctx, int32_t n_passes, int32_t is_final, int32_t do_nee) {
+    ctx->nextHint.set = n_passes > 0; ctx->nextHint.passes = n_passes; ctx->nextHint.isFinal = is_final != 0; ctx->nextHint.doNee = do_nee != 0;
+    return PPG_OK;
+}
 int ppg_render_passes(ppg_ctx *ctx, int32_t n, ppg_pass_stats *st) {
     NEED_TREE
     int rc = renderPassesNoStat(ctx, n);
@@ -2692,6 +2889,7 @@
 int ppg_read_variance(ppg_ctx *ctx, float *rgb) {
     NEED_SCENE
     if (!ctx->d_var.p) { ctx->error = "nothing rendered"; return PPG_ERR_STATE; }
+    { int rc = resolvePassStats(ctx); if (rc) return rc; }
     HIP_CHECK(hipMemcpy(rgb, ctx->d_var.p, 3 * (size_t)ctx->W * ctx->H * 4, hipMemcpyDeviceToHost));
     return PPG_OK;
 }
@@ -2930,12 +3128,16 @@
 }
 
 int ppg_enable_kernel_timing(ppg_ctx *ctx, int32_t enable) {
+    (void)hipSetDevice(ctx->device);
+    (void)resolvePassStats(ctx);
     ctx->timer.reset();
     ctx->bvhNodesVisited = ctx->bvhTrisTested = 0; ctx->tailLongestSum = 0; ctx->shadeCommonRays = 0;
     ctx->timer.enabled = enable != 0;
     return PPG_OK;
 }
 int ppg_kernel_times(ppg_ctx *ctx, ppg_kernel_time *out, uint32_t cap, uint32_t *n) {
+    (void)hipSetDevice(ctx->device);
+    { int rc = resolvePassStats(ctx); if (rc) return rc; }
     ctx->timer.resolve();
     uint32_t k = 0;
     for (size_t i = 0; i < ctx->timer.names.size() && k < cap; ++i, ++k) {
diff --git a/practical-path-guiding_amd/csrc/ppg_host_kernels.h b/practical-path-guiding_amd/csrc/ppg_host_kernels.h
--- a/practical-path-guiding_amd/csrc/ppg_host_kernels.h
+++ b/practical-path-guiding_amd/csrc/ppg_host_kernels.h
@@ -93,6 +93,14 @@
         if (bounce_count) *bounce_count = (unsigned int)carry;
         if (stop && carry < (unsigned long long)stop_below) *stop = 1u;
     }
+}
+
+static __global__ void k_add_block_stats(BlockStats *dst, const BlockStats *src, unsigned int n) {
+    const unsigned int b = blockIdx.x * blockDim.x + threadIdx.x;
+    if (b >= n) return;
+    const BlockStats s = src[b];
+    if (s.rays) atomicAdd(&dst[b].rays, s.rays);
+    if (s.shade_common) atomicAdd(&dst[b].shade_common, s.shade_common);
 }
 
 static __global__ void k_fold_replicas(unsigned long long *compact, unsigned long long *rep, unsigned int n_nodes) {
diff --git a/practical-path-guiding_amd/host/guided_path_hip.h b/practical-path-guiding_amd/host/guided_path_hip.h
--- a/practical-path-guiding_amd/host/guided_path_hip.h
+++ b/practical-path-guiding_amd/host/guided_path_hip.h
@@ -196,6 +196,15 @@
     bool passes(int n, ppg_pass_stats &st, const LogFn &log, bool finalGroups = false) {
         say(log, fmt("Rendering %d render passes.", n));
         int rc;
+        if (m_deferStats) {
+            rc = ppg_render_passes_nostat(m_ctx, n);
+            check(rc, "ppg_render_passes_nostat");
+            if (rc != PPG_OK) return false;
+            check(ppg_finish_passes_deferred(m_ctx), "ppg_finish_passes_deferred");
+            st = ppg_pass_stats();
+            m_passesRendered += n;
+            return true;
+        }
         if (!m_reducer) {
             rc = ppg_render_passes(m_ctx, n, &st);
             check(rc, "ppg_render_passes");
@@ -246,12 +255,19 @@
         const bool automatic = std::string(m_cfg.sampleCombination) == "automatic";
         int iter = 0;
         m_passesRendered = 0;
+        m_deferStats = !automatic && !m_reducer && !log;
         while (m_passesRendered < nPasses) {
             const int sppRendered = m_passesRendered * m_cfg.sppPerPass;
             ppg_set_do_nee(m_ctx, doNeeWithSpp(sppRendered));
             int remainingPasses = nPasses - m_passesRendered;
             int passesThisIteration = std::min(remainingPasses, 1 << iter);
             if (remainingPasses - passesThisIteration < 2 * passesThisIteration) passesThisIteration = remainingPasses;
+            if (!automatic && !m_reducer && remainingPasses > passesThisIteration) {
+                const int left = remainingPasses - passesThisIteration;
+                int next = std::min(left, 1 << (iter + 1));
+                if (left - next < 2 * next) next = left;
+                ppg_hint_next_passes(m_ctx, next, next >= left, doNeeWithSpp((m_passesRendered + passesThisIteration) * m_cfg.sppPerPass));
+            }
             say(log, fmt("ITERATION %d, %d passes", iter, passesThisIteration));
             say(log, "Resetting distributions for sampling.");
             bool isFinal = passesThisIteration >= remainingPasses;
@@ -289,6 +305,7 @@
         float elapsedSeconds = 0;
         int iter = 0;
         m_passesRendered = 0;
+        m_deferStats = false;
         while (elapsedSeconds < nSeconds) {
             const int sppRendered = m_passesRendered * m_cfg.sppPerPass;
             ppg_set_do_nee(m_ctx, doNeeWithSpp(sppRendered));
@@ -338,6 +355,7 @@
     void rethrowHookError() { if (m_hookError) { std::exception_ptr e = m_hookError; m_hookError = nullptr; std::rethrow_exception(e); } }
 
     Reducer *m_reducer = nullptr;
+    bool m_deferStats = false;
     std::atomic<bool> m_cancelled{false};
     bool m_filmComplete = false;
     std::exception_ptr m_hookError;
diff --git a/practical-path-guiding_amd/ppg_host/bindings.py b/practical-path-guiding_amd/ppg_host/bindings.py
--- a/practical-path-guiding_amd/ppg_host/bindings.py
+++ b/practical-path-guiding_amd/ppg_host/bindings.py
@@ -777,6 +777,25 @@
         self._call("finish_passes", C.byref(st))
         return st
 
+    def can_defer_stats(self):
+        return self.prefix == "ppg_"
+
+    def finish_passes_deferred(self):
+        self._call("finish_passes_deferred")
+
+    def pass_stats_resolve(self):
+        st = PassStats()
+        self._call("pass_stats_resolve", C.byref(st))
+        return st
+
+    def hint_next_passes(self, n_passes, is_final, do_nee):
+        self._call("hint_next_passes", C.c_int32(int(n_passes)), C.c_int32(int(is_final)), C.c_int32(int(do_nee)))
+
+    def schedule_counters(self):
+        out = (C.c_uint64 * 5)()
+        self._call("schedule_counters", out, C.c_uint32(5))
+        return dict(zip(("stats_deferred", "stats_resolved_busy", "early_launched", "early_used", "early_discarded"), (int(v) for v in out)))
+
     def build_sdtree(self):
         st = TreeStats()
         self._call("build_sdtree", C.byref(st))
diff --git a/practical-path-guiding_amd/ppg_host/integrator.py b/practical-path-guiding_amd/ppg_host/integrator.py
--- a/practical-path-guiding_amd/ppg_host/integrator.py
+++ b/practical-path-guiding_amd/ppg_host/integrator.py
@@ -57,7 +57,24 @@
         nee = self.props["nee"]
         return False if nee == "never" else (spp < 128 if nee == "kickstart" else True)
 
+    def _settle_stats(self, quiet=False):
+        rec, self._owed = getattr(self, "_owed", None), None
+        if rec is None:
+            return
+        try:
+            rec["stats"][0] = self.engine.pass_stats_resolve().as_dict()
+        except Exception:
+            if not quiet:
+                raise
+
     def render(self, scene=None):
+        try:
+            return self._render(scene)
+        except BaseException:
+            self._settle_stats(quiet=True)
+            raise
+
+    def _render(self, scene):
         e, p = self.engine, self.props
         if scene is not None:
             if self.reducer is not None:
@@ -96,6 +113,9 @@
         self._film_complete = False
         spp = p["sppPerPass"]
         automatic = p["sampleCombination"] == "automatic"
+        defer = not automatic and self.reducer is None and self.log is None and e.can_defer_stats()
+        self._owed = None
+        hint = not automatic and self.reducer is None and e.can_defer_stats()
         it, passes_rendered = 0, 0
         current_var_at_end = float("inf")
         t_start = time.monotonic()
@@ -112,6 +132,25 @@
                 self._recorded = not self._final
                 self._film_complete = False
                 e.begin_iteration(self._final)
+                if hint and remaining > this_iter:
+                    left = remaining - this_iter
+                    nxt = min(left, 1 << (it + 1))
+                    if left - nxt < 2 * nxt:
+                        nxt = left
+                    e.hint_next_passes(nxt, nxt >= left, self._do_nee((passes_rendered + this_iter) * spp))
+                if defer:
+                    e.render_passes_nostat(this_iter)
+                    self._settle_stats()
+                    e.finish_passes_deferred()
+                    rec = dict(iter=it, passes=this_iter, stats=[None])
+                    self._owed = rec
+                    passes_rendered += this_iter
+                    remaining -= this_iter
+                    rec["tree"] = self._build().as_dict()
+                    e.end_iteration()
+                    self.iterations.append(rec)
+                    it += 1
+                    continue
                 st = self._passes(this_iter)
                 rec = dict(iter=it, passes=this_iter, stats=[st.as_dict()])
                 passes_rendered += st.passes_rendered_local
@@ -167,6 +206,7 @@
                     self.log(rec)
                 it += 1
                 elapsed = clock(time.monotonic() - t_start)
+        self._settle_stats()
         if self.reducer is not None and not self._film_complete:
             self.reducer.reduce_film(e, inverse_variance=(p["sampleCombination"] == "inversevar"))
         e.end_render()
```
